# tud-amr/semantic_dsp_map

Hardware: AMD Instinct MI355X
Metric: Mvoxels updated/sec (256^3 grid, 2M particles, VKITTI2 camera; whole hot-path frame) (higher is better)
Workload: dtype f32

## Files before the change

### include/sdm.h

```cpp
#ifndef SDM_H_
#define SDM_H_

#include <stddef.h>
#include <stdint.h>

#ifdef __cplusplus
extern "C" {
#endif

typedef struct sdm_map sdm_map;

typedef enum {
  SDM_OK = 0,
  SDM_ERR_INVALID_ARGUMENT = 1,
  SDM_ERR_NO_DEVICE = 2,
  SDM_ERR_HIP = 3,
  SDM_ERR_CAPACITY = 4,
  SDM_ERR_NOT_CONVERGED = 5,
  SDM_ERR_COMM = 6
} sdm_status;

typedef struct {
  int32_t x_n, y_n, z_n;
  int32_t p_n;
// ... 305 lines not shown
  uint64_t cell_sum[3];
  float    box_min[3];
  float    box_max[3];
  float    centroid[3];
  uint32_t pad1;
} sdm_frontier_cluster;
sdm_status sdm_frontiers_update(sdm_map *m, uint32_t flags, int32_t min_cells, int64_t max_cells);
sdm_status sdm_get_frontier_clusters(sdm_map *m, sdm_frontier_cluster *out, int32_t cap, int32_t *n_out, float origin[3]);
sdm_status sdm_get_frontier_cells(sdm_map *m, uint32_t *cell, uint32_t *cluster, uint8_t *unknown_faces,
                                  int64_t cap, int64_t *n_out);

#define SDM_VIEW_MAX_RAYS 65536
typedef struct {
  float pos[3];
  float q[4];
  float range;
} sdm_view;
typedef struct {
  uint32_t n_unknown;
  uint32_t n_free;
  uint32_t n_occupied;
  uint32_t rays_hit;
  uint32_t rays_in_map;
  uint32_t pad;
  uint64_t ray_cells;
  uint64_t ray_unknown;
} sdm_view_gain;
sdm_status sdm_query_views(sdm_map *m, const sdm_view *views, int64_t n_views, const float *dirs, int32_t n_rays,
                           sdm_view_gain *out, sdm_segment_hit *rays_out, int32_t *ray_unknown_out, uint32_t flags);

#define SDM_REACH_FACE_CONNECTED  0x1u
#define SDM_REACH_THROUGH_UNKNOWN 0x2u
#define SDM_REACH_COST_PER_CELL   10
typedef struct {
  uint32_t n_starts_used;
  uint32_t n_traversable, n_reached, max_cost_reached;
  uint32_t rounds;
  uint32_t flags, min_d2, max_cost;
} sdm_reach_info;
typedef struct {
  uint32_t cost;
  float    metres;
  uint32_t cell;
  uint8_t  next;
  uint8_t  status;
  uint16_t pad;
} sdm_reach_result;
sdm_status sdm_reach_update(sdm_map *m, const float *start_xyz, const uint32_t *start_cells, int64_t n_starts,
                            uint32_t min_d2, uint32_t max_cost, uint32_t flags);
sdm_status sdm_get_reach(sdm_map *m, uint32_t *cost, sdm_reach_info *info, float origin[3]);
sdm_status sdm_query_reach(sdm_map *m, const float *xyz, const uint32_t *cells, int64_t n, sdm_reach_result *out, uint32_t flags);
sdm_status sdm_reach_paths(sdm_map *m, const float *xyz, const uint32_t *cells, int64_t n, int32_t max_len,
                           uint32_t *cells_out, int32_t *len_out, uint32_t flags);

sdm_status sdm_object_particle_count(sdm_map *m, int32_t track_id, int64_t *count);
sdm_status sdm_tracks_with_particles(sdm_map *m, int32_t *out, int32_t cap, int32_t *n_out);

sdm_status sdm_get_stats(sdm_map *m, sdm_stats *out, int32_t count_live);
sdm_status sdm_set_profiling(sdm_map *m, int32_t on);
sdm_status sdm_debug_force_generic_flood(sdm_map *m, int32_t on);
sdm_status sdm_get_ring_state(sdm_map *m, sdm_ring_state *out);
sdm_status sdm_set_ring_state(sdm_map *m, const sdm_ring_state *in);
sdm_status sdm_get_stamps(sdm_map *m, uint32_t *sx, uint32_t *sy, uint32_t *sz);
sdm_status sdm_set_stamps(sdm_map *m, const uint32_t *sx, const uint32_t *sy, const uint32_t *sz);
sdm_status sdm_dump_state(sdm_map *m, float *px, float *py, float *pz, float *w, uint16_t *ts,
                          uint16_t *track, uint8_t *label, uint8_t *status, uint8_t *forget,
                          uint16_t *owner);
sdm_status sdm_load_state(sdm_map *m, const float *px, const float *py, const float *pz,
                          const float *w, const uint16_t *ts, const uint16_t *track,
                          const uint8_t *label, const uint8_t *status, const uint8_t *forget,
                          const uint16_t *owner);
sdm_status sdm_get_ck_kappa(sdm_map *m, float *out);
sdm_status sdm_get_bin_counts(sdm_map *m, uint32_t *out);
sdm_status sdm_get_bins(sdm_map *m, uint32_t *out, int64_t cap, int64_t *n_out);
sdm_status sdm_get_extrinsic(sdm_map *m, float *out16);

sdm_status sdm_time_occupancy_sweep(sdm_map *m, int32_t iters, float *avg_ms);
sdm_status sdm_debug_fill_dense(sdm_map *m);
sdm_status sdm_debug_fill_dense_ex(sdm_map *m, int32_t mode);
sdm_status sdm_debug_hinted_groups(sdm_map *m, int64_t *n_out);
sdm_status sdm_debug_sweep_lists(sdm_map *m, int32_t mode);
sdm_status sdm_debug_sweep_mode(sdm_map *m, int32_t *mode_out);
sdm_status sdm_debug_alias_cap(sdm_map *m, int32_t cap);
sdm_status sdm_debug_reach_tiles(sdm_map *m, int64_t *tiles_out);
sdm_status sdm_debug_view_batch(sdm_map *m, int32_t max_views_in_flight);

sdm_status sdm_test_scan(const uint32_t *in, uint32_t *out, int64_t n);
sdm_status sdm_test_sort_pairs(const uint32_t *keys_in, const uint32_t *vals_in, uint32_t *keys_out,
                               uint32_t *vals_out, int64_t n, int32_t nbits);
#define SDM_TEST_IN_PLACE 1u
#define SDM_TEST_COUNT_ON_DEVICE 2u
#define SDM_TEST_GUARD_WORDS 64
sdm_status sdm_test_scratch_elems(int32_t sort, int64_t n, int64_t *elems);
sdm_status sdm_test_scan_seq(int32_t n_calls, const int64_t *capacity, const int64_t *count, uint32_t flags,
                             const uint32_t *in, uint32_t *out, int32_t *guard_ok, uint32_t *scratch_out);
sdm_status sdm_test_sort_pairs_seq(int32_t n_calls, const int64_t *capacity, const int64_t *count, const int32_t *nbits,
                                   uint32_t flags, const uint32_t *keys_in, const uint32_t *vals_in, uint32_t *keys_out,
                                   uint32_t *vals_out, int32_t *which, int32_t *guard_ok, uint32_t *scratch_out);

const char *sdm_last_error(void);
const char *sdm_version(void);

#ifdef __cplusplus
}
#endif
#endif
```

### semantic_dsp_map_amd/binding.py

```python
import ctypes as C
import os

import numpy as np

_HERE = os.path.dirname(os.path.abspath(__file__))
LIB_PATH = os.environ.get("SDM_LIB_PATH") or os.path.join(_HERE, "csrc", "libsdm_hip.so")

LABELED_POINT = np.dtype([("x", "<f4"), ("y", "<f4"), ("z", "<f4"), ("sigma", "<f4"),
                          ("track_id", "<u2"), ("label_id", "u1"), ("is_valid", "u1")])
OBJECT_MOVE = np.dtype([("track_id", "<i4"), ("T", "<f4", (16,))])
VOXEL_RESULT = np.dtype([("wsum", "<f4"), ("track", "<u2"), ("label", "u1"), ("occ", "i1")])
POINT = np.dtype([("x", "<f4"), ("y", "<f4"), ("z", "<f4"), ("track", "<u2"), ("label", "u1"), ("occ", "i1")])
POINT_XYZRGB = np.dtype([("x", "<f4"), ("y", "<f4"), ("z", "<f4"), ("one", "<f4"), ("b", "u1"), ("g", "u1"), ("r", "u1"), ("a", "u1"),
                         ("pad", "<u4", (3,))])
assert LABELED_POINT.itemsize == 20 and OBJECT_MOVE.itemsize == 68 and VOXEL_RESULT.itemsize == 8 and POINT.itemsize == 16
SEGMENT_HIT = np.dtype([("t", "<f4"), ("voxel", "<u4"), ("cells", "<i4"), ("track", "<u2"), ("label", "u1"), ("occ", "i1")])
BOX_RESULT = np.dtype([("n_occupied", "<i4"), ("n_free", "<i4"), ("n_unknown", "<i4"), ("first_occupied", "<u4"), ("clipped", "<i4")])
assert SEGMENT_HIT.itemsize == 16 and BOX_RESULT.itemsize == 20
QUERY_ON_DEVICE = 0x1
QUERY_UNKNOWN_BLOCKS = 0x2
DISTANCE_RESULT = np.dtype([("distance", "<f4"), ("gradient", "<f4", (3,)), ("nearest", "<f4", (3,)), ("d2", "<u4"), ("track", "<u2"),
                            ("label", "u1"), ("occ", "i1")])
assert DISTANCE_RESULT.itemsize == 36
ESDF_UNKNOWN_IS_OBSTACLE = 0x1
# ... 123 lines not shown
        "sdm_update": [vp, vp, vp, vp, vp, vp, i32, vp, i32, u32, i32],
        "sdm_update_raw": [vp, vp, vp, vp, vp, i32, vp, vp, vp, i32, vp, i32, u32, i32],
        "sdm_update_raw_ex": [vp, vp, vp, vp, vp, i32, vp, vp, vp, i32, vp, i32, u32, i32, vp],
        "sdm_get_labeled_cloud": [vp, vp],
        "sdm_host_alloc": [C.c_size_t, C.POINTER(vp)],
        "sdm_host_free": [vp],
        "sdm_update_begin": [vp, vp, vp, vp, vp, vp, i32, vp, i32, u32, i32, C.POINTER(vp)],
        "sdm_update_finish": [vp, vp, i32, u32, i32],
        "sdm_frame_start": [vp, vp, vp, vp, vp, vp, i32, vp, i32, u32, i32],
        "sdm_frame_moves": [vp],
        "sdm_frame_moves_pending": [vp, C.POINTER(C.c_int32)],
        "sdm_frame_predict": [vp, C.POINTER(vp)],
        "sdm_set_halo_buffers": [vp, vp, vp, vp, vp, i32],
        "sdm_comm_unique_id": [vp],
        "sdm_comm_init": [vp, vp, i32],
        "sdm_ipc_create": [vp, i32, vp],
        "sdm_ipc_connect": [vp, vp],
        "sdm_update_sharded": [vp, vp, vp, vp, vp, vp, i32, vp, i32, u32],
        "sdm_ck_chunk_elems": [vp, C.POINTER(i64)],
        "sdm_ck_reduce": [vp, vp, vp],
        "sdm_comm_timing": [vp, i32],
        "sdm_get_comm_times": [vp, vp],
        "sdm_device_alloc": [vp, C.c_size_t, C.POINTER(vp)],
        "sdm_device_free": [vp, vp],
        "sdm_device_upload": [vp, vp, vp, C.c_size_t],
        "sdm_device_download": [vp, vp, vp, C.c_size_t],
        "sdm_device_synchronize": [vp],
        "sdm_stream": [vp, C.POINTER(vp)],
        "sdm_set_stream": [vp, vp],
        "sdm_set_ck_buffer": [vp, vp],
        "sdm_synchronize": [vp],
        "sdm_get_voxels": [vp, vp],
        "sdm_get_occupied": [vp, vp, C.c_size_t, C.POINTER(C.c_size_t), i32],
        "sdm_get_occupied_rgb": [vp, vp, C.c_size_t, C.POINTER(C.c_size_t), i32],
        "sdm_get_freespace_rgb": [vp, vp, C.c_size_t, C.POINTER(C.c_size_t), i32],
        "sdm_set_colours": [vp, vp],
        "sdm_get_freespace": [vp, vp, C.c_size_t, C.POINTER(C.c_size_t), i32],
        "sdm_voxels_device_ptr": [vp, C.POINTER(vp)],
        "sdm_query_points": [vp, vp, i64, vp, vp, u32],
        "sdm_query_segments": [vp, vp, i64, vp, u32],
        "sdm_query_boxes": [vp, vp, i64, vp, u32],
        "sdm_esdf_update": [vp, u32],
        "sdm_get_esdf": [vp, vp, vp, vp],
        "sdm_query_distance": [vp, vp, i64, vp, u32],
        "sdm_instances_update": [vp, u32],
        "sdm_get_instances": [vp, vp, i32, C.POINTER(i32), vp],
        "sdm_get_label_cells": [vp, vp],
        "sdm_frontiers_update": [vp, u32, i32, i64],
        "sdm_get_frontier_clusters": [vp, vp, i32, C.POINTER(i32), vp],
        "sdm_get_frontier_cells": [vp, vp, vp, vp, i64, C.POINTER(i64)],
        "sdm_query_views": [vp, vp, i64, vp, i32, vp, vp, vp, u32],
        "sdm_debug_view_batch": [vp, i32],
        "sdm_reach_update": [vp, vp, vp, i64, u32, u32, u32],
        "sdm_get_reach": [vp, vp, vp, vp],
        "sdm_query_reach": [vp, vp, vp, i64, vp, u32],
        "sdm_reach_paths": [vp, vp, vp, i64, i32, vp, vp, u32],
        "sdm_debug_reach_tiles": [vp, C.POINTER(i64)],
        "sdm_object_particle_count": [vp, i32, C.POINTER(i64)],
        "sdm_tracks_with_particles": [vp, vp, i32, C.POINTER(i32)],
        "sdm_comm_set_options": [vp, i32, i32],
        "sdm_get_stats": [vp, C.POINTER(Stats), i32],
        "sdm_set_profiling": [vp, i32],
        "sdm_debug_force_generic_flood": [vp, i32],
        "sdm_get_ring_state": [vp, C.POINTER(RingState)],
        "sdm_set_ring_state": [vp, C.POINTER(RingState)],
        "sdm_get_stamps": [vp, vp, vp, vp],
        "sdm_set_stamps": [vp, vp, vp, vp],
        "sdm_dump_state": [vp] + [vp] * 10,
        "sdm_load_state": [vp] + [vp] * 10,
        "sdm_get_ck_kappa": [vp, vp],
        "sdm_get_bin_counts": [vp, vp],
        "sdm_get_bins": [vp, vp, i64, C.POINTER(i64)],
        "sdm_get_extrinsic": [vp, vp],
        "sdm_time_occupancy_sweep": [vp, i32, C.POINTER(C.c_float)],
        "sdm_set_issue_mode": [vp, i32],
        "sdm_bind_host_thread": [i32],
        "sdm_host_numa_node_early": [i32],
        "sdm_debug_fill_dense": [vp],
        "sdm_debug_fill_dense_ex": [vp, i32],
        "sdm_debug_hinted_groups": [vp, C.POINTER(C.c_int64)],
        "sdm_debug_sweep_lists": [vp, i32],
        "sdm_debug_sweep_mode": [vp, C.POINTER(i32)],
        "sdm_debug_alias_cap": [vp, i32],
        "sdm_test_scan": [vp, vp, i64],
        "sdm_test_sort_pairs": [vp, vp, vp, vp, i64, i32],
        "sdm_test_scratch_elems": [i32, i64, C.POINTER(i64)],
        "sdm_test_scan_seq": [i32, vp, vp, u32, vp, vp, C.POINTER(i32), vp],
        "sdm_test_sort_pairs_seq": [i32, vp, vp, vp, u32, vp, vp, vp, vp, vp, C.POINTER(i32), vp],
    }
    for name, argtypes in sig.items():
        fn = getattr(L, name)
        fn.argtypes = argtypes
        fn.restype = C.c_int
    L.sdm_last_error.restype = C.c_char_p
    L.sdm_version.restype = C.c_char_p
    global HOST_NUMA_NODE
    HOST_NUMA_NODE = L.sdm_bind_host_thread(int(os.environ.get("LOCAL_RANK", "0")))
    _lib = L
    return L


def _ptr(a):
    if a is None:
        return None
    if isinstance(a, int):
        return C.c_void_p(a)
    return a.ctypes.data_as(C.c_void_p)


def _check(L, rc, what):
    if rc != 0:
        raise SdmError("%s failed: %s (%s)" % (what, STATUS_NAMES.get(rc, rc), L.sdm_last_error().decode()))


class SdmMap:

    def __init__(self, cfg, params=None, noise_table=None, device=0, shard_rank=0, shard_count=1, max_visible=0):
        self.L = load_library()
        c = Config()
        for k, _ in Config._fields_:
            if k in cfg:
                setattr(c, k, cfg[k])
        c.device, c.shard_rank, c.shard_count, c.max_visible = device, shard_rank, shard_count, max_visible
        self.cfg = c
        h = C.c_void_p()
        _check(self.L, self.L.sdm_create(C.byref(c), C.byref(h)), "sdm_create")
        self.h = h
        self.V = 1 << (c.x_n + c.y_n + c.z_n)
        self.S = 1 << c.p_n
        self.v_count = self.V // shard_count
        self.W, self.H = c.width, c.height
        if params is not None:
            self.set_params(params)
        if noise_table is not None:
            self.upload_noise_table(noise_table)

    def close(self):
        if getattr(self, "h", None):
            self.L.sdm_destroy(self.h)
            self.h = None

    def __del__(self):
        try:
            self.close()
        except Exception:
            pass

    def clear(self):
        _check(self.L, self.L.sdm_clear(self.h), "sdm_clear")

    def set_params(self, params):
        p = Params()
        for k, _ in Params._fields_:
            setattr(p, k, params[k])
        _check(self.L, self.L.sdm_set_params(self.h, C.byref(p)), "sdm_set_params")

    def generate_noise_table(self, seed=20250217, n=1000000, stddev=0.05):
        _check(self.L, self.L.sdm_generate_noise_table(self.h, seed, n, stddev), "sdm_generate_noise_table")

    def upload_noise_table(self, table):
        t = np.ascontiguousarray(table, dtype=np.float32)
        _check(self.L, self.L.sdm_upload_noise_table(self.h, _ptr(t), t.size), "sdm_upload_noise_table")

    def download_noise_table(self, n=1000000):
        t = np.empty(n, np.float32)
        _check(self.L, self.L.sdm_download_noise_table(self.h, _ptr(t), n), "sdm_download_noise_table")
# ... 398 lines not shown

    def ring_state(self):
        r = RingState()
        _check(self.L, self.L.sdm_get_ring_state(self.h, C.byref(r)), "sdm_get_ring_state")
        return {"global_time_stamp": r.global_time_stamp, "moved_steps": list(r.moved_steps),
                "eq_steps": list(r.eq_steps), "map_center": list(r.map_center), "last_pos": list(r.last_pos),
                "birth_cursor": r.birth_cursor, "move_cursor": r.move_cursor}

    def set_ring_state(self, d):
        r = RingState()
        r.global_time_stamp = d["global_time_stamp"]
        for i in range(3):
            r.moved_steps[i] = d["moved_steps"][i]
            r.eq_steps[i] = d["eq_steps"][i]
            r.map_center[i] = d["map_center"][i]
            r.last_pos[i] = d["last_pos"][i]
        r.birth_cursor = d["birth_cursor"]
        r.move_cursor = d["move_cursor"]
        _check(self.L, self.L.sdm_set_ring_state(self.h, C.byref(r)), "sdm_set_ring_state")

    def stamps(self):
        c = self.cfg
        sx = np.empty(1 << c.x_n, np.uint32)
        sy = np.empty(1 << c.y_n, np.uint32)
        sz = np.empty(1 << c.z_n, np.uint32)
        _check(self.L, self.L.sdm_get_stamps(self.h, _ptr(sx), _ptr(sy), _ptr(sz)), "sdm_get_stamps")
        return sx, sy, sz

    def set_stamps(self, sx, sy, sz):
        sx, sy, sz = (np.ascontiguousarray(a, dtype=np.uint32) for a in (sx, sy, sz))
        _check(self.L, self.L.sdm_set_stamps(self.h, _ptr(sx), _ptr(sy), _ptr(sz)), "sdm_set_stamps")

    def dump_state(self):
        n = self.v_count * self.S
        st = {k: np.empty(n, dt) for k, dt in STATE_FIELDS}
        _check(self.L, self.L.sdm_dump_state(self.h, *[_ptr(st[k]) for k, _ in STATE_FIELDS]), "sdm_dump_state")
        return st

    def load_state(self, st):
        arrs = [np.ascontiguousarray(st[k], dtype=dt) for k, dt in STATE_FIELDS]
        _check(self.L, self.L.sdm_load_state(self.h, *[_ptr(a) for a in arrs]), "sdm_load_state")

    def ck_kappa(self):
        out = np.empty(self.W * self.H, np.float32)
        _check(self.L, self.L.sdm_get_ck_kappa(self.h, _ptr(out)), "sdm_get_ck_kappa")
        return out.reshape(self.H, self.W)

    def bin_counts(self):
        out = np.empty(self.W * self.H, np.uint32)
        _check(self.L, self.L.sdm_get_bin_counts(self.h, _ptr(out)), "sdm_get_bin_counts")
        return out.reshape(self.H, self.W)

    def bins(self):
        n = C.c_int64()
        _check(self.L, self.L.sdm_get_bins(self.h, None, 0, C.byref(n)), "sdm_get_bins")
        out = np.empty(max(n.value, 1), np.uint32)
        _check(self.L, self.L.sdm_get_bins(self.h, _ptr(out), n.value, C.byref(n)), "sdm_get_bins")
        return out[:n.value]

    def extrinsic(self):
        out = np.empty(16, np.float32)
        _check(self.L, self.L.sdm_get_extrinsic(self.h, _ptr(out)), "sdm_get_extrinsic")
        return out.reshape(4, 4)

    def fill_dense_ex(self, mode):
        _check(self.L, self.L.sdm_debug_fill_dense_ex(self.h, mode), "sdm_debug_fill_dense_ex")

    def hinted_groups(self):
        n = C.c_int64()
        _check(self.L, self.L.sdm_debug_hinted_groups(self.h, C.byref(n)), "sdm_debug_hinted_groups")
        return n.value

    def force_sweep_lists(self, mode):
        _check(self.L, self.L.sdm_debug_sweep_lists(self.h, int(mode)), "sdm_debug_sweep_lists")

    def sweep_mode(self):
        v = C.c_int32(0)
        _check(self.L, self.L.sdm_debug_sweep_mode(self.h, C.byref(v)), "sdm_debug_sweep_mode")
        return v.value

    def set_alias_cap(self, cap):
        _check(self.L, self.L.sdm_debug_alias_cap(self.h, int(cap)), "sdm_debug_alias_cap")

    def fill_dense(self):
        _check(self.L, self.L.sdm_debug_fill_dense(self.h), "sdm_debug_fill_dense")

    def time_occupancy_sweep(self, iters=20):
        ms = C.c_float()
        _check(self.L, self.L.sdm_time_occupancy_sweep(self.h, iters, C.byref(ms)), "sdm_time_occupancy_sweep")
        return ms.value


def pinhole_rays(cfg, stride=1):
    get = (lambda k: cfg[k]) if isinstance(cfg, dict) else (lambda k: getattr(cfg, k))
    u = np.arange(0, int(get("width")), int(stride), dtype=np.float32)
    v = np.arange(0, int(get("height")), int(stride), dtype=np.float32)
    x = (u - np.float32(get("cx"))) / np.float32(get("fx"))
    y = (v - np.float32(get("cy"))) / np.float32(get("fy"))
    out = np.empty((len(v), len(u), 3), np.float32)
    out[..., 0], out[..., 1], out[..., 2] = x[None, :], y[:, None], 1.0
    return out


def comm_unique_id():
    L = load_library()
    buf = np.zeros(128, np.uint8)
    _check(L, L.sdm_comm_unique_id(_ptr(buf)), "sdm_comm_unique_id")
    return buf.tobytes()


def test_scan(a):
    L = load_library()
    a = np.ascontiguousarray(a, dtype=np.uint32)
    out = np.empty_like(a)
    _check(L, L.sdm_test_scan(_ptr(a), _ptr(out), a.size), "sdm_test_scan")
    return out


def test_sort_pairs(keys, vals, nbits):
    L = load_library()
    keys = np.ascontiguousarray(keys, dtype=np.uint32)
    vals = np.ascontiguousarray(vals, dtype=np.uint32)
    ko, vo = np.empty_like(keys), np.empty_like(vals)
    _check(L, L.sdm_test_sort_pairs(_ptr(keys), _ptr(vals), _ptr(ko), _ptr(vo), keys.size, nbits), "sdm_test_sort_pairs")
    return ko, vo


TEST_IN_PLACE, TEST_COUNT_ON_DEVICE, TEST_GUARD_WORDS = 1, 2, 64


def test_scratch_elems(sort, n):
    L = load_library()
    v = C.c_int64(0)
    _check(L, L.sdm_test_scratch_elems(int(bool(sort)), int(n), C.byref(v)), "sdm_test_scratch_elems")
    return v.value


def _seq_args(capacity, count, arrays):
    capacity = np.ascontiguousarray(capacity, dtype=np.int64)
    count = capacity.copy() if count is None else np.ascontiguousarray(count, dtype=np.int64)
    if capacity.ndim != 1 or capacity.size == 0 or count.shape != capacity.shape:
        raise ValueError("one capacity and one count per call")
    arrays = [np.ascontiguousarray(a, dtype=np.uint32) for a in arrays]
    if any(a.shape != (int(capacity.sum()),) for a in arrays):
        raise ValueError("the arrays hold one slice of `capacity` words per call")
    return capacity, count, arrays


def test_scan_seq(capacity, a, out, count=None, in_place=False, count_on_device=False, want_scratch=False):
    L = load_library()
    capacity, count, (a, out) = _seq_args(capacity, count, [a, out])
    out = out.copy()
    flags = (TEST_IN_PLACE if in_place else 0) | (TEST_COUNT_ON_DEVICE if count_on_device else 0)
    scratch = np.empty(test_scratch_elems(False, capacity.max()), np.uint32) if want_scratch else None
    ok = C.c_int32(0)
    _check(L, L.sdm_test_scan_seq(capacity.size, _ptr(capacity), _ptr(count), flags, _ptr(a), _ptr(out), C.byref(ok), _ptr(scratch)),
           "sdm_test_scan_seq")
    return out, bool(ok.value), scratch


def test_sort_pairs_seq(capacity, nbits, keys, vals, keys_out, vals_out, count=None, count_on_device=False, want_scratch=False):
    L = load_library()
    capacity, count, (keys, vals, keys_out, vals_out) = _seq_args(capacity, count, [keys, vals, keys_out, vals_out])
    nbits = np.ascontiguousarray(np.broadcast_to(np.asarray(nbits, np.int32), capacity.shape))
    keys_out, vals_out = keys_out.copy(), vals_out.copy()
    which = np.zeros(capacity.size, np.int32)
# ... 7 lines not shown
```

### semantic_dsp_map_amd/csrc/frame.hip

```cpp
#include <chrono>

#include "sdm_map.h"

#pragma clang fp contract(off)

void sdm::drop_graphs(sdm_map *m) {
  if (m->graph_exec) (void)hipGraphExecDestroy(m->graph_exec);
  if (m->graph) (void)hipGraphDestroy(m->graph);
  m->graph_exec = nullptr;
  m->graph = nullptr;
  m->graph_set_node = nullptr;
  for (hipGraphExec_t &g : m->piece) {
    if (g) (void)hipGraphExecDestroy(g);
    g = nullptr;
  }
}

namespace {

inline void stage_mark(sdm_map *m, int stage) {
  if (m->profiling && !m->capturing) {
    (void)hipEventRecord(m->ev[stage], m->stream);
    m->stage_ran[stage] = true;
  }
}

sdm_status frame_host_prepare(sdm_map *m, const float cam_pos[3], const float cam_q[4], const sdm_object_move *moves, int32_t n_moves,
                              const int32_t *remove_tracks, int32_t n_remove, uint32_t flags, int32_t stop_after) {
  if ((n_moves > MAX_MOVE_OBJECTS || n_remove > MAX_REMOVE_TRACKS) && m->capturing) {
    set_error("sdm_update", __FILE__, __LINE__, "object lists beyond one frame block inside a graph capture");
    return SDM_ERR_INVALID_ARGUMENT;
  }
  m->moves_all.clear();
  m->removes_all.clear();
  m->mv_batch_next = n_moves > MAX_MOVE_OBJECTS ? (size_t)MAX_MOVE_OBJECTS : 0;
  m->mv_batch_ready = false;
  if (n_moves > MAX_MOVE_OBJECTS) m->moves_all.assign(moves, moves + n_moves);
  if (n_remove > MAX_REMOVE_TRACKS) m->removes_all.assign(remove_tracks, remove_tracks + n_remove);
  m->stop_after = stop_after;
  m->frame_flags = flags;
  for (int i = 0; i < 9; ++i) m->stage_ran[i] = false;
  m->global_time_stamp += 1;
  FrameArgs &fa = m->fa;
  fa.su.n = 0;
  fa.su.value = m->global_time_stamp;
  m->restamped[0] = m->restamped[1] = m->restamped[2] = 0;
  update_ego_center(m, cam_pos);
  sync_frame_scalars(m);
  if (m->stamps_dirty) {
    m->sweep_all = true;
    fa.su.n = 0;
  }
  refresh_filter(m);
  m->forgetting_initialized = true;
  compute_extrinsic(m, cam_pos, cam_q);
  compute_frustum_box(m);
  fa.f = m->f;
  memset(&fa.ms, 0, sizeof(fa.ms));
  const int n_first = n_moves < MAX_MOVE_OBJECTS ? n_moves : MAX_MOVE_OBJECTS;
  fa.ms.n = n_first;
  for (int k = 0; k < n_first; ++k) {
    fa.ms.track[k] = (uint16_t)moves[k].track_id;
    memcpy(fa.ms.T[k], moves[k].T, 12 * sizeof(float));
  }
  fa.n_obj = n_first;
  fa.mv_batch = 0;
  if (n_moves > 0 && !stage_done(stop_after, 1)) m->mv_seq++;
  fa.mv_seq = m->mv_seq;
  fa.n_remove = n_remove < MAX_REMOVE_TRACKS ? n_remove : MAX_REMOVE_TRACKS;
  for (int k = 0; k < fa.n_remove; ++k) fa.remove[k] = (uint16_t)remove_tracks[k];
  fa.force_generic = m->force_generic_flood;
  m->n_moves = n_moves;
  m->n_remove = n_remove;
  return SDM_OK;
}

sdm_status frame_enqueue_start(sdm_map *m) {
  hipStream_t s = m->stream;
  const Dims &d = m->d;
  const int32_t stop_after = m->stop_after;
  const bool whole = d.v_count == d.V;
  stage_mark(m, 0);
  if (m->stamps_dirty) SDM_TRY(upload_stamps(m));
  m->cur_depth = m->fa.depth;
  m->cur_cloud = m->fa.cloud;
  if (m->capturing) {
    m->fb.set(d, m->st, m->sc, m->fa, true, whole);
    launch_frame_begin(m->fb, s);
    HIP_TRY(hipEventRecord(m->cap_begin, s));
    HIP_TRY(hipStreamWaitEvent(m->s_frustum, m->cap_begin, 0));
    HIP_TRY(hipStreamWaitEvent(m->s_birth, m->cap_begin, 0));
  } else {
    const bool side_chain_now = m->n_moves > 0 && (!whole || ((m->comm || m->ipc) && m->sharded_frame));
    if (!m->state_event_valid && (!m->vis_event_valid || side_chain_now)) {
      HIP_TRY(hipEventRecord(m->ev_state, s));
      m->state_event_valid = true;
    }
    HIP_TRY(hipStreamWaitEvent(m->s_frustum, m->vis_event_valid ? m->ev_vis : m->ev_state, 0));
    launch_set_frame(m->d_fa[1], m->fa, m->s_frustum);
    HIP_TRY(hipEventRecord(m->ev_fa, m->s_frustum));
    if (whole && m->mv_pending) HIP_TRY(hipMemsetAsync(m->sc.mv_tot, 0, move_total_elems() * sizeof(uint32_t), s));
    m->fb.set(d, m->st, m->sc, m->fa, false, whole);
    launch_frame_begin(m->fb, s, !stage_done(stop_after, 5) ? m->ev_begin : nullptr);
    if (whole && m->n_moves > 0) m->mv_pending = true;
  }
  stage_mark(m, 1);
  if (stage_done(stop_after, 1)) return SDM_OK;

  const bool side_chain = !m->capturing && m->n_moves > 0 && (!whole || ((m->comm || m->ipc) && m->sharded_frame));
  if (m->capturing) {
    if (!whole) launch_moves_count(d, m->st, m->sc, m->d_counts_local, s);
  } else if (side_chain) {
    HIP_TRY(lazy_stream(m->device, &m->s_moves));
    HIP_TRY(hipStreamWaitEvent(m->s_moves, m->ev_state, 0));
    if (!whole) {
      if (m->mv_pending) HIP_TRY(hipMemsetAsync(m->sc.mv_tot, 0, move_total_elems() * sizeof(uint32_t), m->s_moves));
      launch_moves_count(d, m->st, m->sc, m->counts_local_user ? m->counts_local_user : m->d_counts_local, m->s_moves, &m->fa);
      m->mv_pending = true;
    }
    if ((m->comm || m->ipc) && m->sharded_frame) {
      if (m->comm_timing) HIP_TRY(hipEventRecord(m->ev_comm[0], m->s_moves));
      SDM_TRY(exchange_counts(m, m->s_moves));
      if (m->comm_timing) {
        HIP_TRY(hipEventRecord(m->ev_comm[1], m->s_moves));
        m->comm_timed[0] = true;
      }
    }
    HIP_TRY(hipEventRecord(m->ev_counts, m->s_moves));
  }
  if (!stage_done(stop_after, 3)) {
    launch_frustum(d, m->sc, m->s_frustum);
    HIP_TRY(hipGetLastError());
    HIP_TRY(hipEventRecord(m->capturing ? m->cap_frustum : m->ev_frustum, m->s_frustum));
  } else if (!m->capturing) {
    HIP_TRY(hipStreamWaitEvent(s, m->ev_fa, 0));
  }
  if (!stage_done(stop_after, 5)) {
    if (!m->capturing) HIP_TRY(hipStreamWaitEvent(m->s_birth, m->ev_begin, 0));
    m->birth_which = launch_birth_prepare(d, m->flt, m->bo, m->st, m->sc, m->s_birth);
    HIP_TRY(hipEventRecord(m->capturing ? m->cap_birth : m->ev_birth, m->s_birth));
  }
  if (side_chain) HIP_TRY(hipStreamWaitEvent(s, m->ev_counts, 0));
  m->state_event_valid = false;
  m->vis_event_valid = false;
  return SDM_OK;
}

sdm_status check_frame_args(sdm_map *m, const float *depth, const sdm_labeled_point *cloud, const float cam_pos[3], const float cam_q[4],
                            const sdm_object_move *moves, int32_t n_moves, const int32_t *remove_tracks, int32_t n_remove) {
  if (!m || !depth || !cloud || !cam_pos || !cam_q || n_moves < 0 || n_remove < 0 || (n_moves && !moves) || (n_remove && !remove_tracks)) {
    set_error("sdm_update", __FILE__, __LINE__, "null pointer or negative count");
    return SDM_ERR_INVALID_ARGUMENT;
  }
  return SDM_OK;
}

sdm_status stage_inputs(sdm_map *m, const float *depth, const sdm_labeled_point *cloud, uint32_t flags) {
  const size_t hw = (size_t)m->d.W * m->d.H;
  if (flags & SDM_INPUT_ON_DEVICE) {
    m->fa.depth = depth;
    m->fa.cloud = cloud;
  } else {
    HIP_TRY(hipMemcpyAsync(m->d_depth, depth, hw * sizeof(float), hipMemcpyHostToDevice, m->stream));
    HIP_TRY(hipMemcpyAsync(m->d_cloud, cloud, hw * sizeof(sdm_labeled_point), hipMemcpyHostToDevice, m->stream));
    m->fa.depth = m->d_depth;
    m->fa.cloud = m->d_cloud;
  }
  return SDM_OK;
}

}

extern "C" {

sdm_status sdm_frame_start(sdm_map *m, const float *depth, const sdm_labeled_point *cloud, const float cam_pos[3],
                           const float cam_q[4], const sdm_object_move *moves, int32_t n_moves,
                           const int32_t *remove_tracks, int32_t n_remove, uint32_t flags, int32_t stop_after) {
  sdm_status rc = check_frame_args(m, depth, cloud, cam_pos, cam_q, moves, n_moves, remove_tracks, n_remove);
  if (rc != SDM_OK) return rc;
  HIP_TRY(hipSetDevice(m->device));
  if ((rc = frame_host_prepare(m, cam_pos, cam_q, moves, n_moves, remove_tracks, n_remove, flags, stop_after)) != SDM_OK) return rc;
  if ((rc = stage_inputs(m, depth, cloud, flags)) != SDM_OK) return rc;
  m->n_direct_frames++;
  return frame_enqueue_start(m);
}

sdm_status sdm_frame_moves(sdm_map *m) {
  if (!m) return SDM_ERR_INVALID_ARGUMENT;
  if (stage_done(m->stop_after, SDM_STAGE_EGO)) return SDM_OK;
  if (!m->capturing) HIP_TRY(hipSetDevice(m->device));
  const int world = m->cfg.shard_count, rank = m->cfg.shard_rank;
  const int32_t *counts_all = m->counts_all_user;
  int w = world, r = rank;
  if (!counts_all) {
    counts_all = m->counts_local_user ? m->counts_local_user : m->d_counts_local;
    w = 1;
    r = 0;
  }
  if (m->capturing || m->n_moves > 0) {
    launch_moves_transform(m->d, m->flt, m->st, m->sc, counts_all, w, r, m->stream);
    m->mv_pending = false;
    m->mv_batch_ready = false;
    const bool shard = m->d.v_count != m->d.V;
    while (m->mv_batch_next && m->mv_batch_next < m->moves_all.size()) {
      const size_t k0 = m->mv_batch_next;
      const int nb = (int)std::min<size_t>(MAX_MOVE_OBJECTS, m->moves_all.size() - k0);
      FrameArgs &fa = m->fa;
      memset(&fa.ms, 0, sizeof(fa.ms));
      fa.ms.n = nb;
      for (int k = 0; k < nb; ++k) {
        fa.ms.track[k] = (uint16_t)m->moves_all[k0 + k].track_id;
        memcpy(fa.ms.T[k], m->moves_all[k0 + k].T, 12 * sizeof(float));
      }
      fa.n_obj = nb;
      fa.mv_seq = ++m->mv_seq;
      fa.mv_batch += 1;
      m->mv_batch_next = k0 + MAX_MOVE_OBJECTS;
      launch_moves_batch(m->d, m->st, m->sc, fa, m->counts_local_user ? m->counts_local_user : m->d_counts_local, m->stream);
      if (shard) {
        m->mv_batch_ready = true;
        return SDM_OK;
      }
      launch_moves_transform(m->d, m->flt, m->st, m->sc, counts_all, w, r, m->stream);
    }
    m->mv_batch_next = 0;
  }
  return SDM_OK;
}

sdm_status sdm_frame_moves_pending(sdm_map *m, int32_t *pending) {
  if (!m || !pending) return SDM_ERR_INVALID_ARGUMENT;
  *pending = m->mv_batch_ready ? 1 : 0;
  return SDM_OK;
}

sdm_status sdm_frame_predict(sdm_map *m, const float **ck_part_dev) {
  if (!m) return SDM_ERR_INVALID_ARGUMENT;
  if (m->mv_batch_ready) {
    set_error("sdm_frame_predict", __FILE__, __LINE__, "a batch of the frame's object list is still waiting for its counts: sdm_frame_moves_pending");
    return SDM_ERR_INVALID_ARGUMENT;
  }
  const int stop_after = m->stop_after;
  if (stage_done(stop_after, SDM_STAGE_EGO)) return SDM_OK;
  if (!m->capturing) HIP_TRY(hipSetDevice(m->device));
  hipStream_t s = m->stream;
  const Dims &d = m->d;
  if (m->capturing || m->n_moves > 0)
    launch_moves_finish(d, m->flt, m->st, m->sc, m->counts_all_user ? m->cfg.shard_count : 1, m->cfg.shard_rank, s);
  stage_mark(m, 2);
  if (stage_done(stop_after, 2)) return SDM_OK;

  if (m->capturing || m->n_remove > 0) launch_remove(d, m->st, m->sc, s);
  for (size_t k0 = MAX_REMOVE_TRACKS; k0 < m->removes_all.size(); k0 += MAX_REMOVE_TRACKS) {
    FrameArgs &fa = m->fa;
    fa.n_remove = (int)std::min<size_t>(MAX_REMOVE_TRACKS, m->removes_all.size() - k0);
    for (int k = 0; k < fa.n_remove; ++k) fa.remove[k] = (uint16_t)m->removes_all[k0 + k];
    launch_set_frame(m->d_fa[0], fa, s);
    launch_remove(d, m->st, m->sc, s);
  }
  stage_mark(m, 3);
  if (stage_done(stop_after, 3)) return SDM_OK;

  HIP_TRY(hipStreamWaitEvent(s, m->capturing ? m->cap_frustum : m->ev_frustum, 0));
  float *ck_dst = m->ck_user ? m->ck_user : m->d_ck_part;
  launch_visibility(d, m->flt, m->st, m->sc, ck_dst, m->fused_ck ? 1 : 0, s, m->capturing ? nullptr : m->ev_vis);
  if (!m->capturing) m->vis_event_valid = true;
  stage_mark(m, 4);
  if (stage_done(stop_after, 4)) return SDM_OK;

  launch_ck(d, m->flt, m->st, m->sc, ck_dst, m->fused_ck ? 1 : 0, s);
  if (ck_part_dev) *ck_part_dev = ck_dst;
  return SDM_OK;
}

sdm_status sdm_update_begin(sdm_map *m, const float *depth, const sdm_labeled_point *cloud, const float cam_pos[3],
                            const float cam_q[4], const sdm_object_move *moves, int32_t n_moves,
                            const int32_t *remove_tracks, int32_t n_remove, uint32_t flags, int32_t stop_after,
                            const float **ck_part_dev) {
  sdm_status rc = sdm_frame_start(m, depth, cloud, cam_pos, cam_q, moves, n_moves, remove_tracks, n_remove, flags, stop_after);
  if (rc != SDM_OK) return rc;
  const int32_t *keep_all = m->counts_all_user;
  m->counts_all_user = nullptr;
  rc = sdm_frame_moves(m);
  while (rc == SDM_OK && m->mv_batch_ready) rc = sdm_frame_moves(m);
  if (rc == SDM_OK) rc = sdm_frame_predict(m, ck_part_dev);
  m->counts_all_user = keep_all;
  return rc;
}

sdm_status sdm_set_halo_buffers(sdm_map *m, int32_t *counts_local, const int32_t *counts_all, void *send, const void *recv_all,
                                int32_t cap_records) {
  if (!m || cap_records < 0) return SDM_ERR_INVALID_ARGUMENT;
  m->counts_local_user = counts_local;
  m->counts_all_user = counts_all;
  m->sc.halo_send = (unsigned char *)send;
  m->sc.halo_recv = (const unsigned char *)recv_all;
  m->sc.halo_cap = (uint32_t)cap_records;
  m->sc.halo_world = (uint32_t)m->cfg.shard_count;
  return SDM_OK;
}

sdm_status sdm_update_finish(sdm_map *m, const float *ck_parts_dev, int32_t n_parts, uint32_t flags, int32_t stop_after) {
  if (!m || n_parts < 1) return SDM_ERR_INVALID_ARGUMENT;
  if (stage_done(stop_after, SDM_STAGE_VISIBILITY)) return SDM_OK;
  if (!m->capturing) HIP_TRY(hipSetDevice(m->device));
  hipStream_t s = m->stream;
  const Dims &d = m->d;
  const float *own = m->ck_user ? m->ck_user : m->d_ck_part;
  const float *ck_raw = nullptr;
  if (!m->fused_ck) {
    if (!ck_parts_dev || n_parts == 1) ck_raw = ck_parts_dev ? ck_parts_dev : own;
    else launch_ck_finish(d, m->flt, m->sc, ck_parts_dev, n_parts, m->ck_part_stride, s);
  }
  m->ck_raw_last = ck_raw;
  m->ck_part_stride = 0;
  launch_weight(d, m->flt, m->st, m->sc, s, ck_raw);
  stage_mark(m, 5);
  if (stage_done(stop_after, 5)) return SDM_OK;
  HIP_TRY(hipStreamWaitEvent(s, m->capturing ? m->cap_birth : m->ev_birth, 0));
  launch_birth_replay(d, m->flt, m->st, m->sc, m->birth_which, m->global_time_stamp > 65535u, s);
  if (!m->capturing) {
    if (d.v_count != d.V || m->comm || m->ipc) {
      HIP_TRY(hipEventRecord(m->ev_state, s));
      m->state_event_valid = true;
    } else {
      m->state_event_valid = false;
    }
  }
  stage_mark(m, 6);
  if (stage_done(stop_after, 6)) return SDM_OK;
  if (!(flags & SDM_SKIP_OCCUPANCY)) {
    launch_occupancy(d, m->flt, m->st, m->sc.cnt, m->sweep_all ? 1 : 0, m->sc.fa, next_epoch(m->f.epoch), s, sweep_mode(m));
    if (m->sweep_all) m->sweep_rec_pending = true;
    m->sweep_all = false;
    if (!m->capturing) m->sweep_epoch = next_epoch(m->f.epoch);
  }
  stage_mark(m, 7);
  return SDM_OK;
}

namespace {

sdm_status issue_frame(sdm_map *m, uint32_t flags, int32_t stop_after) {
  sdm_status rc = frame_enqueue_start(m);
  if (rc == SDM_OK) rc = sdm_frame_moves(m);
  if (rc == SDM_OK) rc = sdm_frame_predict(m, nullptr);
  if (rc == SDM_OK) rc = sdm_update_finish(m, nullptr, 1, flags, stop_after);
  return rc;
// ... 18 lines not shown
  sdm_status rc = SDM_OK;
  if (e == hipSuccess) {
    rc = issue_frame(m, m->frame_flags, 0);
    hipGraph_t g = nullptr;
    e = hipStreamEndCapture(m->stream, &g);
    m->graph = g;
  }
  m->s_frustum = side[0];
  m->s_birth = side[1];
  m->s_moves = side[2];
  m->capturing = false;
  if (e != hipSuccess || rc != SDM_OK || !m->graph) {
    set_error("hipStreamCapture", __FILE__, __LINE__, e != hipSuccess ? hipGetErrorString(e) : "frame enqueue failed under capture");
    (void)hipGetLastError();
    return rc != SDM_OK ? rc : SDM_ERR_HIP;
  }
  size_t n_nodes = 0;
  HIP_TRY(hipGraphGetNodes(m->graph, nullptr, &n_nodes));
  std::vector<hipGraphNode_t> nodes(n_nodes);
  HIP_TRY(hipGraphGetNodes(m->graph, nodes.data(), &n_nodes));
  for (hipGraphNode_t nd : nodes) {
    hipGraphNodeType t;
    if (hipGraphNodeGetType(nd, &t) != hipSuccess || t != hipGraphNodeTypeKernel) continue;
    hipKernelNodeParams kp;
    if (hipGraphKernelNodeGetParams(nd, &kp) == hipSuccess && kp.func == FrameBeginLaunch::kernel()) m->graph_set_node = nd;
  }
  if (!m->graph_set_node) {
    set_error("graph_capture", __FILE__, __LINE__, "frame-block node not found in the captured graph");
    return SDM_ERR_HIP;
  }
  HIP_TRY(hipGraphInstantiate(&m->graph_exec, m->graph, nullptr, nullptr, 0));
  m->graph_flt = m->flt;
  return SDM_OK;
}

sdm_status graph_launch(sdm_map *m) {
  m->fb.set(m->d, m->st, m->sc, m->fa, true, m->d.v_count == m->d.V);
  hipKernelNodeParams kp;
  memset(&kp, 0, sizeof(kp));
  kp.func = const_cast<void *>(FrameBeginLaunch::kernel());
  kp.gridDim = dim3(FrameBeginLaunch::GRID);
  kp.blockDim = dim3(FrameBeginLaunch::BLOCK);
  kp.sharedMemBytes = 0;
  kp.kernelParams = m->fb.argv;
  kp.extra = nullptr;
  const auto t0 = std::chrono::steady_clock::now();
  HIP_TRY(hipGraphExecKernelNodeSetParams(m->graph_exec, m->graph_set_node, &kp));
  const auto t1 = std::chrono::steady_clock::now();
  HIP_TRY(hipGraphLaunch(m->graph_exec, m->stream));
  if (m->host_timing) {
    m->t_setparams_us += std::chrono::duration<double, std::micro>(t1 - t0).count();
    m->t_launch_us += std::chrono::duration<double, std::micro>(std::chrono::steady_clock::now() - t1).count();
  }
  return SDM_OK;
}

sdm_status pieces_capture(sdm_map *m) {
  SDM_TRY(capture_prepare(m));
  const Dims &d = m->d;
  auto capture = [&](hipStream_t st, int which, auto &&body) -> sdm_status {
    HIP_TRY(hipStreamBeginCapture(st, hipStreamCaptureModeThreadLocal));
    body(st);
    hipGraph_t g = nullptr;
    hipError_t e = hipStreamEndCapture(st, &g);
    if (e != hipSuccess || !g) {
      set_error("hipStreamEndCapture", __FILE__, __LINE__, e != hipSuccess ? hipGetErrorString(e) : "no graph");
      (void)hipGetLastError();
      return SDM_ERR_HIP;
    }
    e = hipGraphInstantiate(&m->piece[which], g, nullptr, nullptr, 0);
    (void)hipGraphDestroy(g);
    if (e != hipSuccess) {
      set_error("hipGraphInstantiate", __FILE__, __LINE__, hipGetErrorString(e));
      return SDM_ERR_HIP;
    }
    return SDM_OK;
  };
  sdm_status rc = capture(m->s_frustum, 0, [&](hipStream_t st) { launch_frustum(d, m->sc, st); });
  if (rc == SDM_OK)
    rc = capture(m->s_birth, 1, [&](hipStream_t st) { m->birth_which = launch_birth_prepare(d, m->flt, m->bo, m->st, m->sc, st); });
  if (rc == SDM_OK)
    rc = capture(m->stream, 2, [&](hipStream_t st) {
      if (d.v_count != d.V) launch_moves_count(d, m->st, m->sc, m->d_counts_local, st);
      launch_moves_transform(d, m->flt, m->st, m->sc, m->d_counts_local, 1, 0, st);
      launch_moves_finish(d, m->flt, m->st, m->sc, 1, m->cfg.shard_rank, st);
      launch_remove(d, m->st, m->sc, st);
    });
  if (rc == SDM_OK)
    rc = capture(m->stream, 3, [&](hipStream_t st) {
      launch_visibility(d, m->flt, m->st, m->sc, m->d_ck_part, 1, st);
      launch_ck(d, m->flt, m->st, m->sc, m->d_ck_part, 1, st);
      launch_weight(d, m->flt, m->st, m->sc, st);
    });
  if (rc == SDM_OK)
    rc = capture(m->stream, 4, [&](hipStream_t st) {
      launch_birth_replay(d, m->flt, m->st, m->sc, m->birth_which, false, st);
      launch_occupancy(d, m->flt, m->st, m->sc.cnt, 0, m->sc.fa, 0, st);
    });
  m->graph_flt = m->flt;
  return rc;
}

sdm_status pieces_launch(sdm_map *m) {
  hipStream_t s = m->stream;
  const auto t0 = std::chrono::steady_clock::now();
  m->fb.set(m->d, m->st, m->sc, m->fa, true, m->d.v_count == m->d.V);
  launch_frame_begin(m->fb, s);
  HIP_TRY(hipEventRecord(m->ev_begin, s));
  HIP_TRY(hipStreamWaitEvent(m->s_frustum, m->ev_begin, 0));
  HIP_TRY(hipGraphLaunch(m->piece[0], m->s_frustum));
  HIP_TRY(hipEventRecord(m->ev_frustum, m->s_frustum));
  HIP_TRY(hipStreamWaitEvent(m->s_birth, m->ev_begin, 0));
  HIP_TRY(hipGraphLaunch(m->piece[1], m->s_birth));
  HIP_TRY(hipEventRecord(m->ev_birth, m->s_birth));
  HIP_TRY(hipGraphLaunch(m->piece[2], s));
  HIP_TRY(hipStreamWaitEvent(s, m->ev_frustum, 0));
  HIP_TRY(hipGraphLaunch(m->piece[3], s));
  HIP_TRY(hipStreamWaitEvent(s, m->ev_birth, 0));
  HIP_TRY(hipGraphLaunch(m->piece[4], s));
  if (m->host_timing) m->t_launch_us += std::chrono::duration<double, std::micro>(std::chrono::steady_clock::now() - t0).count();
  return SDM_OK;
}

}

sdm_status sdm_set_issue_mode(sdm_map *m, int32_t mode) {
  if (!m || mode < 0 || mode > 4) return SDM_ERR_INVALID_ARGUMENT;
  HIP_TRY(hipSetDevice(m->device));
  bool use;
  int shape;
  issue_mode_for(m, mode, &use, &shape);
  if (shape != m->graph_shape) {
    HIP_TRY(hipStreamSynchronize(m->stream));
    drop_graphs(m);
  }
  m->graph_mode = mode;
  m->use_graph = use;
  m->graph_shape = shape;
  return SDM_OK;
}

sdm_status sdm_update(sdm_map *m, const float *depth, const sdm_labeled_point *cloud, const float cam_pos[3],
                      const float cam_q[4], const sdm_object_move *moves, int32_t n_moves, const int32_t *remove_tracks,
                      int32_t n_remove, uint32_t flags, int32_t stop_after) {
  sdm_status rc = check_frame_args(m, depth, cloud, cam_pos, cam_q, moves, n_moves, remove_tracks, n_remove);
  if (rc != SDM_OK) return rc;
  HIP_TRY(hipSetDevice(m->device));
  m->fused_ck = true;
  const auto tp0 = std::chrono::steady_clock::now();
  rc = frame_host_prepare(m, cam_pos, cam_q, moves, n_moves, remove_tracks, n_remove, flags, stop_after);
  if (rc == SDM_OK) rc = stage_inputs(m, depth, cloud, flags);
  if (m->host_timing) m->t_prepare_us += std::chrono::duration<double, std::micro>(std::chrono::steady_clock::now() - tp0).count();
  if (rc != SDM_OK) {
    m->fused_ck = false;
    return rc;
  }
  const bool would_be_plain = stop_after == 0 && (flags & ~(uint32_t)SDM_INPUT_ON_DEVICE) == 0 && !m->profiling &&
                              m->cfg.shard_count == 1 && !m->comm && !m->ck_user && !m->counts_local_user &&
                              m->stream == m->own_stream && !m->sweep_all && !m->stamps_dirty &&
                              n_moves <= MAX_MOVE_OBJECTS && n_remove <= MAX_REMOVE_TRACKS &&
                              m->global_time_stamp <= 65535u;
  const bool plain = m->use_graph && would_be_plain;
  if (plain) {
    const bool pieces = m->graph_shape == GRAPH_PIECES;
    bool have = pieces ? m->piece[4] != nullptr : m->graph_exec != nullptr;
    if (have && memcmp(&m->graph_flt, &m->flt, sizeof(Filter)) != 0) have = false;
    if (!have) {
      const auto tc = std::chrono::steady_clock::now();
      rc = pieces ? pieces_capture(m) : graph_capture(m);
      if (m->host_timing)
        fprintf(stderr, "sdm host timing: graph capture + instantiate %.0f us (%s)\n",
                std::chrono::duration<double, std::micro>(std::chrono::steady_clock::now() - tc).count(),
                pieces ? "pieces" : (m->graph_shape == GRAPH_CHAIN ? "chain" : "branched"));
    }
    bool direct = false;
    if (rc != SDM_OK) {
      m->use_graph = false;
      direct = true;
      rc = SDM_OK;
    } else {
      rc = pieces ? pieces_launch(m) : graph_launch(m);
      if (rc != SDM_OK) {
        m->use_graph = false;
        m->stamps_dirty = true;
        m->sweep_all = true;
      } else {
        m->cur_depth = m->fa.depth;
        m->cur_cloud = m->fa.cloud;
        m->state_event_valid = false;
        m->vis_event_valid = false;
// ... 191 lines not shown
```

### semantic_dsp_map_amd/csrc/kernels.hip

```cpp
#include <algorithm>

#include <type_traits>

#include <hip/hip_ext.h>
#include "sdm_internal.h"
#include "sdm_scratch.h"

#pragma clang fp contract(off)

namespace sdm {

namespace {

constexpr int TPB = 256;

#ifdef SDM_AB_TIMERS
}
__device__ unsigned long long g_dbg[6][8192 * 4];
namespace {
#define DBG_T() wall_clock64()
#define DBG_PUTK(k, i, v) do { if (blockIdx.x < 8192) g_dbg[k][blockIdx.x * 4 + (i)] = (unsigned long long)(v); } while (0)
#define DBG_PUT(i, v) DBG_PUTK(0, i, v)
#define DBG_LANE0(k, i) do { if (threadIdx.x == 0 && threadIdx.y == 0) DBG_PUTK(k, i, DBG_T()); } while (0)
#else
#define DBG_T() 0ull
#define DBG_PUT(i, v)
#define DBG_LANE0(k, i)
#endif

typedef uint32_t v4u __attribute__((ext_vector_type(4)));
typedef uint32_t v2u __attribute__((ext_vector_type(2)));
template <typename T>
using gptr = const __attribute__((address_space(1))) T *;
template <typename T>
__device__ __forceinline__ gptr<T> as_global(const T *p) {
  return (gptr<T>)p;
}
__device__ __forceinline__ sdm_labeled_point load_point(const sdm_labeled_point *cloud, size_t i) {
  static_assert(sizeof(sdm_labeled_point) == 20, "five words");
  gptr<uint32_t> w = (gptr<uint32_t>)(cloud + i);
  uint32_t t[5];
#pragma unroll
  for (int k = 0; k < 5; ++k) t[k] = w[k];
  sdm_labeled_point o;
  __builtin_memcpy(&o, t, sizeof(o));
  return o;
}
template <int A = 16, typename T, int N>
__device__ __forceinline__ void load_vec(T (&dst)[N], const T *src) {
  constexpr int B = (int)sizeof(T) * N;
  if constexpr (A < (B > 16 ? 16 : B)) {
    __builtin_memcpy(dst, __builtin_assume_aligned(src, A), B);
  } else if constexpr (B >= 16) {
    const v4u *p = reinterpret_cast<const v4u *>(src);
    v4u tmp[B / 16];
#pragma unroll
    for (int i = 0; i < B / 16; ++i) tmp[i] = __builtin_nontemporal_load(p + i);
    __builtin_memcpy(dst, tmp, B);
  } else if constexpr (B == 8) {
    v2u tmp = __builtin_nontemporal_load(reinterpret_cast<const v2u *>(src));
    __builtin_memcpy(dst, &tmp, 8);
  } else if constexpr (B == 4) {
    uint32_t tmp = __builtin_nontemporal_load(reinterpret_cast<const uint32_t *>(src));
    __builtin_memcpy(dst, &tmp, 4);
  } else {
    uint16_t tmp = __builtin_nontemporal_load(reinterpret_cast<const uint16_t *>(src));
    __builtin_memcpy(dst, &tmp, 2);
  }
}
template <int A = 16, typename T, int N>
__device__ __forceinline__ void store_vec(T *dst, const T (&src)[N]) {
  constexpr int B = (int)sizeof(T) * N;
  constexpr int AL = A < (B > 16 ? 16 : B) ? A : (B > 16 ? 16 : B);
  __builtin_memcpy(__builtin_assume_aligned(dst, AL), src, B);
}

template <int S>
struct RecRaw {
  static constexpr int L = S - 1, BYTES = 10 * L, N8 = (BYTES + 7) / 8;
  uint32_t d[2 * N8];
};
template <int S, bool NT = true>
__device__ __forceinline__ void rec_fetch(RecRaw<S> &raw, const unsigned char *r) {
  constexpr int N8 = RecRaw<S>::N8;
#pragma unroll
  for (int j = 0; j < N8 / 2; ++j) {
    const rec_v4u *q = reinterpret_cast<const rec_v4u *>(r + 16 * j);
    const rec_v4u t = NT ? __builtin_nontemporal_load(q) : *q;
    raw.d[4 * j + 0] = t.x;
    raw.d[4 * j + 1] = t.y;
    raw.d[4 * j + 2] = t.z;
    raw.d[4 * j + 3] = t.w;
  }
  if constexpr (N8 & 1) {
    const rec_v2u *q = reinterpret_cast<const rec_v2u *>(r + 16 * (N8 / 2));
    const rec_v2u t = NT ? __builtin_nontemporal_load(q) : *q;
    raw.d[2 * N8 - 2] = t.x;
    raw.d[2 * N8 - 1] = t.y;
  }
}
__device__ __forceinline__ uint32_t raw_u16(const uint32_t *d, int off) { return (d[off >> 2] >> ((off & 3) * 8)) & 0xffffu; }
__device__ __forceinline__ uint32_t raw_u8(const uint32_t *d, int off) { return (d[off >> 2] >> ((off & 3) * 8)) & 0xffu; }
template <int S>
__device__ __forceinline__ void rec_unpack(const RecRaw<S> &raw, float (&wv)[S], uint16_t (&ts)[S], uint16_t (&trk)[S], uint8_t (&lab)[S],
                                           uint8_t (&stv)[S]) {
  constexpr int L = S - 1;
  wv[0] = 0.f;
  ts[0] = 0;
  trk[0] = 0;
  lab[0] = 0;
// ... 1375 lines not shown
  for (int i = 1; i < S; ++i) {
    live[i] = false;
    if (stv[i] == ST_INVALID) continue;
    if ((uint32_t)tsv[i] < smax) {
      stv[i] = ST_INVALID;
      dirty = true;
      continue;
    }
    valid_n++;
    live[i] = true;
  }
  int pixv[S], rowv[S];
  float camz[S], dptv[S];
#pragma unroll
  for (int i = 1; i < S; ++i) {
    pixv[i] = -1;
    rowv[i] = 0;
    if (!live[i]) continue;
    int row, col;
    if (project_to_image(d, f, pos[i].x, pos[i].y, pos[i].z, row, col, camz[i])) {
      pixv[i] = row * d.W + col;
      rowv[i] = row;
      dptv[i] = depth_img[pixv[i]];
    }
  }
  bool vis[S];
  uint32_t pib[S];
#pragma unroll
  for (int i = 1; i < S; ++i) {
    vis[i] = false;
    if (!live[i] || pixv[i] < 0) continue;
    const float dpt = dptv[i];
    if (dpt > d.dmax) {
      SlotRef{rec, S - 1, (uint32_t)i - 1u}.set_w(SDM_OCC_INIT_WEIGHT);
      wrote_free = true;
      observed = true;
      continue;
    }
    if (camz[i] > dpt * d.occl_coeff) continue;
    observed = true;
    vis[i] = true;
  }
  const uint32_t sub = (shard + (threadIdx.x & 63u)) & (ROW_SUBS - 1);
  uint32_t rq[S];
#pragma unroll
  for (int i = 1; i < S; ++i)
    if (vis[i]) {
      pib[i] = atomicAdd(&sc.bin_count[pixv[i]], 1u);
      rq[i] = atomicAdd(&sc.row_cnt[(size_t)(rowv[i] * ROW_SUBS + sub) * ROW_CNT_STRIDE], 1u);
    }
#pragma unroll
  for (int i = 1; i < S; ++i)
    if (vis[i]) {
      if (rq[i] < sc.row_cap && pib[i] < (1u << ROW_PIB_BITS)) {
        const uint32_t col = (uint32_t)(pixv[i] - rowv[i] * d.W);
        sc.row_list[(size_t)(rowv[i] * ROW_SUBS + sub) * sc.row_cap + rq[i]] =
            make_uint2((uint32_t)(((size_t)v << d.p_n) + i), col | pib[i] << ROW_COL_BITS);
      } else {
        sc.cnt->overflow = 1;
      }
    }
  if (dirty) rec_store_status<S>(rec, stv);
  if (dirty || wrote_free) st.vflag[lv] = VF_DIRTY;
  bool stamped = observed;
  if (!observed && valid_n == 0) stamped = im_ok && im_z <= im_depth;
  if (stamped) st.vts[lv] = (uint16_t)f.gts;
  if (dirty || wrote_free || stamped) mark_tile(st, lv, f.epoch);
}

constexpr int VIS_WORDS = 32;
constexpr int VIS_J = VIS_WORDS * 64 / TPB;

template <int S>
__global__ __launch_bounds__(TPB) void k_visibility(Dims d, State st, Scratch sc) {
  __shared__ unsigned long long wmask[VIS_WORDS];
  __shared__ uint32_t woff[VIS_WORDS + 1];
  __shared__ uint16_t full_list[VIS_WORDS * 64];
  __shared__ uint32_t n_full;
  DBG_LANE0(1, 0);
  const Frame f = sc.fa->f;
  const gptr<float> depth_img = as_global(sc.fa->depth);
  const uint32_t fgen = (uint32_t)sc.fa->force_generic, fcx = (uint32_t)sc.cnt->flood_complex;
  const bool generic = (fgen | fcx) != 0;
  if (blockIdx.x == 0 && threadIdx.x == 0) {
    sc.cnt->vis_flood_complex = fcx;
    sc.cnt->vis_flood_rounds = sc.cnt->flood_rounds;
    sc.cnt->vis_start_in_frustum = sc.cnt->start_in_frustum;
  }
  const int bx = f.bb1[0] - f.bb0[0], by = f.bb1[1] - f.bb0[1], bz = f.bb1[2] - f.bb0[2];
  if (bx <= 0 || by <= 0 || bz <= 0) return;
  const int wlo = f.bb0[0] >> 6, nwx = ((f.bb1[0] - 1) >> 6) - wlo + 1;
  const uint32_t n_words = (uint32_t)nwx * by * bz;
  for (uint32_t g0 = blockIdx.x * VIS_WORDS; g0 < n_words; g0 += gridDim.x * VIS_WORDS) {
  __syncthreads();
  if (threadIdx.x == 0) n_full = 0;
  if (threadIdx.x < VIS_WORDS) {
    const uint32_t g = g0 + threadIdx.x;
    unsigned long long m = 0;
    if (g < n_words) {
      const int wi = wlo + (int)(g % nwx);
      const int ay = f.bb0[1] + (int)((g / nwx) % by);
      const int az = f.bb0[2] + (int)(g / ((uint32_t)nwx * by));
      const uint32_t rz = axis_correct(az + f.eq[2], d.NZ);
      if (rz >= d.rz_begin && rz < d.rz_begin + d.rz_count) {
        const uint64_t *__restrict__ bits = generic ? sc.reach : sc.vmask;
        const int VY = d.NY + 1;
        unsigned long long w0[4], w1[4], lr[4];
        const int wi1 = wi + 1 < (int)sc.wpl ? wi + 1 : wi;
#pragma unroll
        for (int c = 0; c < 4; ++c) {
          const int y = ay + (c & 1), z = az + (c >> 1);
          const size_t lb = ((size_t)z * VY + y) * sc.wpl;
          lr[c] = sc.line_reach[(size_t)z * sc.wy + (y >> 6)];
          w0[c] = bits[lb + wi];
          w1[c] = bits[lb + wi1];
        }
        __builtin_amdgcn_sched_barrier(0);
#pragma unroll
        for (int c = 0; c < 4; ++c) {
          const int y = ay + (c & 1);
          const bool line_ok = generic || ((lr[c] >> (y & 63)) & 1ull);
          const unsigned long long w1m = wi + 1 < (int)sc.wpl ? w1[c] : 0ull;
          if (line_ok) m |= w0[c] | (w0[c] >> 1) | (w1m << 63);
        }
        const int x0 = wi << 6;
        const int lo = f.bb0[0] > x0 ? f.bb0[0] - x0 : 0;
        const int hi = f.bb1[0] - x0 < 64 ? f.bb1[0] - x0 : 64;
        unsigned long long keep = hi >= 64 ? ~0ull : ((1ull << hi) - 1ull);
        keep &= ~((1ull << lo) - 1ull);
        m &= keep;
      }
    }
    wmask[threadIdx.x] = m;
    const uint32_t c = (uint32_t)__popcll(m);
    uint32_t inc = c;
#pragma unroll
    for (int off = 1; off < VIS_WORDS; off <<= 1) {
      const uint32_t t = __shfl_up(inc, off, 64);
      if ((int)threadIdx.x >= off) inc += t;
    }
    woff[threadIdx.x] = inc - c;
    if (threadIdx.x == VIS_WORDS - 1) woff[VIS_WORDS] = inc;
  }
  __syncthreads();
  const uint32_t nl = woff[VIS_WORDS];
  DBG_LANE0(1, 1);
  if (threadIdx.x == 0 && nl) atomicAdd(&sc.cnt->shard[blockIdx.x & (VIS_SHARDS - 1)].fv, nl);
  if (nl == 0) continue;
  uint32_t code[VIS_J], lvv[VIS_J], flg[VIS_J];
#pragma unroll
  for (int j = 0; j < VIS_J; ++j) {
    const uint32_t li = threadIdx.x + (uint32_t)j * TPB;
    code[j] = 0xffffffffu;
    lvv[j] = 0;
    flg[j] = 0;
    if ((uint32_t)j * TPB >= nl) continue;
    const bool have = li < nl;
    int w = 0;
#pragma unroll
    for (int k = 1; k < VIS_WORDS; ++k) w += woff[k] <= li ? 1 : 0;
    const int bit = nth_set_bit(wmask[w], li - woff[w]) & 63;
    const uint32_t g = g0 + (uint32_t)w;
    const int ax = ((wlo + (int)(g % nwx)) << 6) + bit;
    const int ay = f.bb0[1] + (int)((g / nwx) % by);
    const int az = f.bb0[2] + (int)(g / ((uint32_t)nwx * by));
    const uint32_t rx = axis_correct(ax + f.eq[0], d.NX), ry = axis_correct(ay + f.eq[1], d.NY), rz = axis_correct(az + f.eq[2], d.NZ);
    code[j] = have ? (uint32_t)(w << 6 | bit) : 0xffffffffu;
    lvv[j] = have ? ring_to_voxel(d, rx, ry, rz) - d.v_begin : 0u;
    flg[j] = st.vflag[lvv[j]];
  }
  __builtin_amdgcn_sched_barrier(0);
#pragma unroll
  for (int j = 0; j < VIS_J; ++j) flg[j] = code[j] != 0xffffffffu ? flg[j] & VF_STATE : 0u;
  float imz[VIS_J], imd[VIS_J];
#pragma unroll
  for (int j = 0; j < VIS_J; ++j) {
    imz[j] = 1.f;
    imd[j] = 0.f;
    if (code[j] == 0xffffffffu) continue;
    if (flg[j]) {
      full_list[atomicAdd(&n_full, 1u)] = (uint16_t)code[j];
      continue;
    }
    const uint32_t g = g0 + (code[j] >> 6);
    const int ax = ((wlo + (int)(g % nwx)) << 6) + (int)(code[j] & 63u);
    const int ay = f.bb0[1] + (int)((g / nwx) % by);
    const int az = f.bb0[2] + (int)(g / ((uint32_t)nwx * by));
    const float ix = (float)(uint32_t)ax * d.voxel_size + d.pmin[0] + f.center[0];
    const float iy = (float)(uint32_t)ay * d.voxel_size + d.pmin[1] + f.center[1];
    const float iz = (float)(uint32_t)az * d.voxel_size + d.pmin[2] + f.center[2];
    int row, col;
    float z;
    if (project_to_image(d, f, ix, iy, iz, row, col, z)) {
      imz[j] = z;
      imd[j] = depth_img[(size_t)row * d.W + col];
    }
  }
#pragma unroll
  for (int j = 0; j < VIS_J; ++j) {
    if (code[j] == 0xffffffffu || flg[j]) continue;
    if (imz[j] <= imd[j]) {
      st.vts[lvv[j]] = (uint16_t)f.gts;
      mark_tile(st, lvv[j], f.epoch);
    }
  }
  __syncthreads();
  DBG_LANE0(1, 2);
  const uint32_t nf = n_full;
  for (uint32_t k = threadIdx.x; k < nf; k += TPB) {
    const uint32_t c = full_list[k];
    const uint32_t g = g0 + (c >> 6);
    const int ax = ((wlo + (int)(g % nwx)) << 6) + (int)(c & 63u);
    const int ay = f.bb0[1] + (int)((g / nwx) % by);
    const int az = f.bb0[2] + (int)(g / ((uint32_t)nwx * by));
    visibility_voxel<S>(d, f, st, sc, depth_img, ax, ay, az);
  }
  DBG_LANE0(1, 3);
  }
}

__device__ __forceinline__ void sift_down(uint32_t *a, uint32_t start, uint32_t end) {
  uint32_t root = start;
  while (2 * root + 1 <= end) {
    uint32_t child = 2 * root + 1, sw = root;
    if (a[sw] < a[child]) sw = child;
    if (child + 1 <= end && a[sw] < a[child + 1]) sw = child + 1;
    if (sw == root) return;
    uint32_t t = a[root];
    a[root] = a[sw];
    a[sw] = t;
    root = sw;
  }
}

constexpr int A7_ROWS = 16;
constexpr int A7_ITEMS = 16;
constexpr uint32_t CK_LIGHT_MAX = 4;
enum : uint8_t { CK_DONE = 0, CK_LIGHT = 1, CK_HEAVY = 2 };

__device__ __forceinline__ void ck_store(const Filter &flt, const Scratch &sc, float *__restrict__ ck_out, int finish, int p,
                                         const sdm_labeled_point &o, float ck) {
  if (finish) {
    const float ckk = ck * flt.p_detect + flt.noise_number;
    sc.ck_kappa[p] = ckk;
    sc.pix4[p] = make_float4(o.x, o.y, o.z, ckk);
    sc.pixt[p] = (uint32_t)o.track_id | (1u << 16);
  } else {
    ck_out[p] = ck;
  }
}

constexpr int BR_TPB = 640;
constexpr int BR_WAVES = BR_TPB / 64;
constexpr int BR_MAXW = 1 << ROW_COL_BITS;
template <int PPT>
__global__ __launch_bounds__(BR_TPB) __attribute__((amdgpu_waves_per_eu(PPT <= 4 ? 5 : 4, PPT <= 4 ? 5 : 4))) void k_bin_rows(Dims d, State st, Scratch sc) {
  static_assert(PPT == 2 || PPT == 4 || PPT * BR_TPB >= BR_MAXW, "eight pixels per thread cover the widest image");
  __shared__ uint32_t pre[BR_MAXW + 1];
  __shared__ uint32_t wave_tot[BR_WAVES];
  __shared__ uint32_t s_base;
  const int r = blockIdx.x;
  DBG_LANE0(2, 0);
  if (r == (int)gridDim.x - 1 && threadIdx.x < 64) alias_compact_wave(st);
  const bool overflow = sc.cnt->overflow != 0;
  const int lane = threadIdx.x & 63, wid = threadIdx.x >> 6;
  const int W = d.W;
  uint32_t c[PPT];
  const int j0 = PPT * (int)threadIdx.x;
#pragma unroll
  for (int u = 0; u < PPT; ++u) c[u] = (!overflow && j0 + u < W) ? sc.bin_count[r * W + j0 + u] : 0u;
  uint32_t sub_n = 0;
  if (threadIdx.x < ROW_SUBS && !overflow) {
    sub_n = sc.row_cnt[(size_t)(r * ROW_SUBS + threadIdx.x) * ROW_CNT_STRIDE];
    if (sub_n > sc.row_cap) sub_n = sc.row_cap;
  }
  uint32_t inc = 0;
#pragma unroll
  for (int u = 0; u < PPT; ++u) inc += c[u];
  const uint32_t mine = inc;
#pragma unroll
  for (int off = 1; off < 64; off <<= 1) {
    const uint32_t t = __shfl_up(inc, off, 64);
    if (lane >= off) inc += t;
  }
  if (lane == 63) wave_tot[wid] = inc;
  __syncthreads();
  uint32_t before = 0, total = 0;
#pragma unroll
  for (int w = 0; w < BR_WAVES; ++w) {
    if (w < wid) before += wave_tot[w];
    total += wave_tot[w];
  }
  {
    uint32_t run = before + inc - mine;
#pragma unroll
    for (int u = 0; u < PPT; ++u) {
      if (j0 + u < W) pre[j0 + u] = run;
      run += c[u];
    }
  }
  if (threadIdx.x == 0) {
// ... 1422 lines not shown
}

void launch_clear(const Dims &d, const State &st, hipStream_t s, bool fresh) {
  size_t n = (size_t)d.v_count * d.S;
  if (fresh) {
    hipMemsetAsync(st.pos4, 0, n * sizeof(float4), s);
    hipMemsetAsync(st.forget, 0, n, s);
    hipMemsetAsync(st.rec, 0, (size_t)d.v_count * rec_bytes(d.S), s);
    hipMemsetAsync(st.vts, 0, (size_t)d.v_count * sizeof(uint16_t), s);
    hipMemsetAsync(st.vflag, 0, (size_t)d.v_count, s);
    hipMemsetAsync(st.owner, 0xFF, n * sizeof(uint16_t), s);
    hipMemsetAsync(st.res, 0, (size_t)d.v_count * sizeof(sdm_voxel_result), s);
  } else {
    if (d.S == 8) hipLaunchKernelGGL(k_clear_map<8>, dim3(blocks_for(d.v_count, CLR_VOX)), dim3(TPB), 0, s, d, st);
    else if (d.S == 16) hipLaunchKernelGGL(k_clear_map<16>, dim3(blocks_for(d.v_count, CLR_VOX)), dim3(TPB), 0, s, d, st);
    else
      hipLaunchKernelGGL(k_clear_slots, dim3(blocks_for(n)), dim3(TPB), 0, s, d, st, n);
  }
  hipMemsetAsync(st.grp_hint, 0, grp_hint_bytes(d.v_count), s);
  hipMemsetAsync(st.alias, 0, 8, s);
  hipMemsetAsync(st.alias_filter, 0, ALIAS_FILTER_WORDS * 4, s);
  hipMemsetAsync(st.owner_flag, 0, owner_flag_bytes(n), s);
  hipMemsetAsync(st.owner_flag2, 0, owner_flag2_bytes(n), s);
}

#define SDM_DISPATCH_S(kernel, grid, s, ...)                                                      \
  switch (d.p_n) {                                                                                 \
    case 1: hipLaunchKernelGGL(kernel<2>, grid, dim3(TPB), 0, s, __VA_ARGS__); break;              \
    case 2: hipLaunchKernelGGL(kernel<4>, grid, dim3(TPB), 0, s, __VA_ARGS__); break;              \
    case 3: hipLaunchKernelGGL(kernel<8>, grid, dim3(TPB), 0, s, __VA_ARGS__); break;              \
    default: hipLaunchKernelGGL(kernel<16>, grid, dim3(TPB), 0, s, __VA_ARGS__); break;            \
  }

size_t tile_mark_bytes(const Dims &d) {
  const size_t n_tiles = blocks_for(d.v_count, OCC_TILE);
  return (std::max<size_t>(n_tiles, (size_t)TPB * OCC_SEG_MAX) + 16 + 15) / 16 * 16;
}
void launch_occupancy(const Dims &d, const Filter &flt, const State &st, Counters *cnt, int all_dirty, const FrameArgs *fa, uint32_t remark,
                      hipStream_t s, int mode) {
  dim3 grid(blocks_for(d.v_count, OCC_TILE));
  const int lists = mode & OCC_LISTS;
  if (all_dirty && (mode & OCC_SKIP_SCAN)) {
    SDM_DISPATCH_S(k_occupancy_dense, grid, s, d, flt.occ_threshold, st, cnt, st.occ_need, remark, grid.x | 0x80000000u);
  } else if (all_dirty) {
    const dim3 sgrid = grid;
    if (lists) {
      SDM_DISPATCH_S(k_occupancy_scan_lists, sgrid, s, d, flt.occ_threshold, st, cnt, st.occ_need, grid.x, remark);
      SDM_DISPATCH_S(k_occupancy_listed, dim3(OCC_LISTED_GRID), s, d, flt.occ_threshold, st, remark);
    } else {
      SDM_DISPATCH_S(k_occupancy_scan, sgrid, s, d, flt.occ_threshold, st, cnt, st.occ_need, grid.x, remark);
    }
    SDM_DISPATCH_S(k_occupancy_dense, grid, s, d, flt.occ_threshold, st, cnt, st.occ_need, remark, grid.x);
  } else {
    const uint32_t n_tiles = grid.x;
    const uint32_t seg = n_tiles <= TPB * OCC_SEG_MAX ? ((n_tiles + TPB - 1) / TPB + 15u) / 16u * 16u : 0u;
    if (seg) grid = dim3(std::min<uint32_t>(OCC_GRID, n_tiles));
    SDM_DISPATCH_S(k_occupancy, grid, s, d, flt.occ_threshold, st, cnt, fa, n_tiles, seg);
  }
}


void launch_set_frame(FrameArgs *fa_dev, const FrameArgs &fa, hipStream_t s) {
  hipLaunchKernelGGL(k_set_frame, dim3(1), dim3(TPB), 0, s, fa_dev, fa);
}
const void *set_frame_kernel() { return reinterpret_cast<const void *>(k_set_frame); }

void launch_frustum(const Dims &d, const Scratch &sc, hipStream_t s) {
  static bool lds_attr_set = false;
  if (!lds_attr_set) {
    (void)hipFuncSetAttribute(reinterpret_cast<const void *>(k_flood2d), hipFuncAttributeMaxDynamicSharedMemorySize, 152 * 1024);
    lds_attr_set = true;
  }
  const size_t max_words = (size_t)(d.NY + 1) * (d.NZ + 1) * sc.wpl;
  const unsigned g_mask = (unsigned)std::min<size_t>(blocks_for(max_words * 64), 4096);
  const unsigned g_line = (unsigned)std::min<size_t>(blocks_for((size_t)sc.wy * (d.NZ + 1) * 64), 256);
  hipLaunchKernelGGL(k_vertex_mask, dim3(g_mask), dim3(TPB), 0, s, d, sc.fa_side, sc.vmask, sc.wpl, sc.cnt);
  hipLaunchKernelGGL(k_line_info, dim3(g_line), dim3(TPB), 0, s, d, sc.fa_side, sc.vmask, sc.wpl, sc.wy, sc.line_ne, sc.line_ey, sc.line_ez,
                     sc.cnt);
  hipLaunchKernelGGL(k_flood2d, dim3(1), dim3(TPB), (size_t)(d.NZ + 1) * sc.wy * 8 * 4, s, d, sc.fa_side, sc.vmask, sc.wpl, sc.wy, sc.line_ey,
                     sc.line_ez, sc.line_reach, sc.cnt);
  hipLaunchKernelGGL(k_flood_generic, dim3(1), dim3(1024), 0, s, d, sc.fa_side, sc.vmask, sc.reach, sc.wpl, sc.cnt);
}

void launch_visibility(const Dims &d, const Filter &flt, const State &st, const Scratch &sc, float *ck_out, int finish, hipStream_t s,
                       hipEvent_t vis_done) {
  {
    const size_t max_words = (size_t)((d.NX + 63) / 64 + 1) * d.NY * d.NZ;
    dim3 grid((unsigned)std::min<size_t>(blocks_for(max_words, VIS_WORDS), 2048));
    if (vis_done) {
      switch (d.p_n) {
        case 1: hipExtLaunchKernelGGL(k_visibility<2>, grid, dim3(TPB), 0, s, nullptr, vis_done, 0, d, st, sc); break;
        case 2: hipExtLaunchKernelGGL(k_visibility<4>, grid, dim3(TPB), 0, s, nullptr, vis_done, 0, d, st, sc); break;
        case 3: hipExtLaunchKernelGGL(k_visibility<8>, grid, dim3(TPB), 0, s, nullptr, vis_done, 0, d, st, sc); break;
        default: hipExtLaunchKernelGGL(k_visibility<16>, grid, dim3(TPB), 0, s, nullptr, vis_done, 0, d, st, sc); break;
      }
    } else {
      SDM_DISPATCH_S(k_visibility, grid, s, d, st, sc);
    }
  }
  if (d.W <= 2 * BR_TPB) hipLaunchKernelGGL(k_bin_rows<2>, dim3((unsigned)d.H), dim3(BR_TPB), 0, s, d, st, sc);
  else if (d.W <= 4 * BR_TPB) hipLaunchKernelGGL(k_bin_rows<4>, dim3((unsigned)d.H), dim3(BR_TPB), 0, s, d, st, sc);
  else hipLaunchKernelGGL(k_bin_rows<8>, dim3((unsigned)d.H), dim3(BR_TPB), 0, s, d, st, sc);
  hipLaunchKernelGGL(k_ck_classify, dim3(blocks_for((size_t)d.W * d.H)), dim3(TPB), 0, s, d, flt, sc, ck_out, finish);
}

void launch_ck(const Dims &d, const Filter &flt, const State &st, const Scratch &sc, float *ck_out, int finish, hipStream_t s) {
  hipLaunchKernelGGL(k_ck, dim3(CK_HEAVY_BLOCKS + blocks_for((size_t)d.W * d.H, A7_ROWS * A7_ITEMS)), dim3(A7_ROWS, A7_ITEMS), 0, s, d, flt, st, sc,
                     ck_out, finish);
}
void launch_ck_finish(const Dims &d, const Filter &flt, const Scratch &sc, const float *parts, int n_parts, size_t part_stride, hipStream_t s) {
  hipLaunchKernelGGL(k_ck_finish, dim3(blocks_for((size_t)d.W * d.H)), dim3(TPB), 0, s, d, flt, sc, parts, n_parts,
                     part_stride ? part_stride : (size_t)d.W * d.H);
}
void launch_ck_reduce_chunk(const float *stage, const float *own_part, float *full, uint32_t chunk, int world, int rank, hipStream_t s) {
  hipLaunchKernelGGL(k_ck_reduce_chunk, dim3((chunk + TPB - 1) / TPB), dim3(TPB), 0, s, stage, own_part, full, chunk, world, rank);
}
void launch_weight(const Dims &d, const Filter &flt, const State &st, const Scratch &sc, hipStream_t s, const float *ck_raw) {
  const int side = 2 * d.window_half + 1;
#define SDM_WEIGHT(UU, RR)                                                                                              \
  if (ck_raw) hipLaunchKernelGGL((k_weight<UU, RR, true>), dim3(WT_GRID), dim3(64 * WT_WAVES), 0, s, d, flt, st, sc, ck_raw); \
  else hipLaunchKernelGGL((k_weight<UU, RR, false>), dim3(WT_GRID), dim3(64 * WT_WAVES), 0, s, d, flt, st, sc, ck_raw);
  if (side * side <= 64) {
    SDM_WEIGHT(4, 1)
  } else if (side * side <= 128) {
    SDM_WEIGHT(4, 2)
  } else {
    SDM_WEIGHT(2, 4)
  }
#undef SDM_WEIGHT
}

int launch_birth_prepare(const Dims &d, const Filter &flt, const BirthOrder &bo, const State &st,
                         const Scratch &sc, hipStream_t s) {
  const size_t hw = (size_t)d.W * d.H;
  const size_t total = hw * flt.nb;
  if (flt.use_rng) {
    hipLaunchKernelGGL(k_birth_flags, dim3(blocks_for(hw)), dim3(TPB), 0, s, d, bo, sc);
    exclusive_scan_u32(sc.b_valid, sc.b_rank, hw, sc.scan_scratch_b, s);
  }
  hipLaunchKernelGGL(k_birth_candidates, dim3(blocks_for(total)), dim3(TPB), 0, s, d, flt, bo, st, sc);
  if (flt.use_rng) hipLaunchKernelGGL(k_birth_cursor, dim3(1), dim3(64), 0, s, d, flt, sc);
  int nbits = d.x_n + d.y_n + d.z_n + 1;
  return radix_sort_pairs(sc.bkey_a, sc.bval_a, sc.bkey_b, sc.bval_b, total, nbits, sc.sort_scratch, s);
}

void launch_birth_replay(const Dims &d, const Filter &flt, const State &st, const Scratch &sc, int which, bool literal,
                         hipStream_t s) {
  const size_t total = (size_t)d.W * d.H * flt.nb;
  const uint32_t *skey = which ? sc.bkey_b : sc.bkey_a;
  const uint32_t *sval = which ? sc.bval_b : sc.bval_a;
  dim3 grid(blocks_for(total));
#define SDM_BIRTH(SS)                                                                                                  \
  if (literal) hipLaunchKernelGGL((k_birth_replay<SS, true>), grid, dim3(TPB), 0, s, d, flt, st, sc, skey, sval, (uint32_t)total); \
  else hipLaunchKernelGGL((k_birth_replay<SS, false>), grid, dim3(TPB), 0, s, d, flt, st, sc, skey, sval, (uint32_t)total);
  switch (d.p_n) {
    case 1: SDM_BIRTH(2) break;
    case 2: SDM_BIRTH(4) break;
    case 3: SDM_BIRTH(8) break;
    default: SDM_BIRTH(16) break;
  }
#undef SDM_BIRTH
}

void launch_labeled_cloud(const Dims &d, const CloudArgsHost &h, const float *depth, const uint8_t *static_mask,
                          const uint16_t *label_to_inst, const uint8_t *obj_masks, const double *bbox,
                          sdm_labeled_point *cloud, hipStream_t s) {
  CloudArgs a;
  static_assert(sizeof(CloudArgs) == sizeof(CloudArgsHost), "CloudArgs layout");
  __builtin_memcpy(&a, &h, sizeof(a));
  hipLaunchKernelGGL(k_labeled_cloud, dim3(blocks_for((size_t)d.W * d.H)), dim3(TPB), 0, s, d, a, depth, static_mask, label_to_inst,
                     obj_masks, bbox, cloud);
}

void launch_manual_resize(const Dims &d, const void *src, void *dst, int src_w, int src_h, float scale, int elem_bytes,
                          hipStream_t s) {
  const float scale_inv = 1.f / scale;
  dim3 grid(blocks_for((size_t)d.W * d.H));
  if (elem_bytes == 4)
    hipLaunchKernelGGL(k_manual_resize<float>, grid, dim3(TPB), 0, s, (const float *)src, (float *)dst, src_w, src_h, d.W, d.H, scale_inv);
  else
    hipLaunchKernelGGL(k_manual_resize<uint8_t>, grid, dim3(TPB), 0, s, (const uint8_t *)src, (uint8_t *)dst, src_w, src_h, d.W, d.H,
                       scale_inv);
// ... 143 lines not shown
```

### semantic_dsp_map_amd/csrc/lifecycle.hip

```cpp
#include <rocrand/rocrand.h>

#include <chrono>
#include <cmath>
#include <cstdlib>
#include <mutex>

#include "sdm_map.h"

#pragma clang fp contract(off)

namespace {

thread_local std::string g_last_error;

__attribute__((constructor(101))) void sdm_runtime_defaults() {
  setenv("HIP_FORCE_DEV_KERNARG", "1", 0);
}

constexpr double GRAPH_PIECES_US = 110.0, GRAPH_CHAIN_US = 170.0;
constexpr int LAUNCHES_PER_FRAME = 50;

__global__ void k_noop() {}

}
// ... 300 lines not shown
  }
  if (c.overflow && c.n_moved > m->sc.cap_move) {
    char buf[160];
    snprintf(buf, sizeof(buf), "moved-copy list overflowed: %u particles of moving objects in one frame, more than %u", c.n_moved,
             m->sc.cap_move);
    set_error("capacity", __FILE__, __LINE__, buf);
    return SDM_ERR_CAPACITY;
  }
  if (c.overflow) {
    set_error("capacity", __FILE__, __LINE__, "visible-particle or move list overflowed: more visible particles than sdm_config.max_visible, more in ONE image row than "
              "max(2 max_visible / height, 2 width slots) - raise max_visible -, or more than 2^20 in one pixel's bin");
    return SDM_ERR_CAPACITY;
  }
  if (c.vis_flood_rounds >= 256 && !c.vis_flood_complex) {
    set_error("flood", __FILE__, __LINE__, "frustum flood fill did not converge");
    return SDM_ERR_NOT_CONVERGED;
  }
  return SDM_OK;
}

}

extern "C" {

const char *sdm_last_error(void) { return g_last_error.c_str(); }
const char *sdm_version(void) { return "libsdm_hip 0.1 (gfx950)"; }

static sdm_status map_init(sdm_map *m, const sdm_config *cfg, int shard_count) {
  m->cfg = *cfg;
  m->cfg.shard_count = shard_count;
  m->device = cfg->device;
  Dims &d = m->d;
  d.x_n = cfg->x_n;
  d.y_n = cfg->y_n;
  d.z_n = cfg->z_n;
  d.p_n = cfg->p_n;
  d.NX = 1u << d.x_n;
  d.NY = 1u << d.y_n;
  d.NZ = 1u << d.z_n;
  d.S = 1u << d.p_n;
  d.V = d.NX * d.NY * d.NZ;
  d.rz_count = d.NZ / shard_count;
  d.rz_begin = d.rz_count * cfg->shard_rank;
  d.v_count = d.V / shard_count;
  d.v_begin = d.v_count * cfg->shard_rank;
  d.voxel_size = cfg->voxel_size;
  d.recip = 1.f / cfg->voxel_size;
  d.pmax[0] = (d.NX >> 1) * cfg->voxel_size;
  d.pmax[1] = (d.NY >> 1) * cfg->voxel_size;
  d.pmax[2] = (d.NZ >> 1) * cfg->voxel_size;
  for (int a = 0; a < 3; ++a) d.pmin[a] = -d.pmax[a];
  d.W = cfg->width;
  d.H = cfg->height;
  d.fx = cfg->fx;
  d.fy = cfg->fy;
  d.cx = cfg->cx;
  d.cy = cfg->cy;
  d.dmin = cfg->depth_min;
  d.dmax = cfg->depth_max;
  d.tanx = (float)tan(atan2(cfg->width / 2.0, (double)cfg->fx));
  d.tany = (float)tan(atan2(cfg->height / 2.0, (double)cfg->fy));
  d.occl_coeff = 0.1f + 1.f;
  d.window_half = cfg->window_half;
  d.max_movable = cfg->max_movable_track;
  m->stamps_x.assign(d.NX, 0);
  m->stamps_y.assign(d.NY, 0);
  m->stamps_z.assign(d.NZ, 0);
  m->prm.detection_probability = 0.95f;
  m->prm.noise_number = 0.1f;
  m->prm.nb_ptc_num_per_point = 3;
  m->prm.occupancy_threshold = 0.2f;
  m->prm.max_obersevation_lost_time = 5;
  m->prm.forgetting_rate = 1.0f;
  m->prm.max_forget_count = 5;
  m->prm.match_score_threshold = 0.3f;
  m->prm.id_transition_probability = 0.1f;
  m->prm.if_consider_depth_noise = 0;
  m->prm.if_use_independent_filter = 0;
  m->prm.depth_noise_first_order = 0.f;
  m->prm.depth_noise_zero_order = 0.1f;

  for (hipStream_t *s : {&m->own_stream, &m->s_frustum, &m->s_birth}) HIP_TRY(new_stream(cfg->device, s));
  m->stream = m->own_stream;
  for (hipEvent_t *e : {&m->ev_state, &m->ev_counts, &m->ev_begin, &m->ev_frustum, &m->ev_birth, &m->ev_fa, &m->ev_vis, &m->cap_begin,
                        &m->cap_frustum, &m->cap_birth, &m->ev_copy, &m->raw[0].ev_free, &m->raw[1].ev_free})
    SDM_TRY(new_event(m, e, hipEventDisableTiming));
  const size_t n_slots = (size_t)d.v_count * d.S;
  const size_t hw = (size_t)d.W * d.H;
#define A(ptr, n) SDM_TRY(alloc_tracked(m, &(ptr), (n)))
  A(m->st.pos4, n_slots);
  A(m->st.forget, n_slots);
  HIP_TRY(hipMemsetAsync(m->st.forget, 0, n_slots, m->stream));
  A(m->st.rec, rec_array_bytes(d.v_count, d.S));
  const size_t v_groups = ((size_t)d.v_count + 511) / 512 * 512;
  A(m->st.vts, v_groups + 64);
  A(m->st.vflag, v_groups + 64);
  m->st.tile_stride = (uint32_t)tile_mark_bytes(d);
  A(m->st.tile_dirty, 2 * (size_t)m->st.tile_stride);
  A(m->st.occ_need, ((size_t)d.v_count + 63) / 64 + 32);
  A(m->st.occ_list, occ_list_tiles(d.v_count) * OCC_LIST_CAP);
  A(m->st.occ_list_n, occ_list_tiles(d.v_count) + 64);
  m->st.occ_unit_cap = (uint32_t)((occ_list_tiles(d.v_count) + OCC_LIST_SHARDS - 1) / OCC_LIST_SHARDS * (OCC_LIST_CAP / OCC_LIST_UNIT));
  A(m->st.occ_unit, (size_t)OCC_LIST_SHARDS * m->st.occ_unit_cap);
  A(m->st.occ_shard, OCC_LIST_SHARDS + 1);
  HIP_TRY(hipMemsetAsync(m->st.occ_shard, 0, (OCC_LIST_SHARDS + 1) * sizeof(State::OccListShard), m->stream));
  A(m->st.grp_hint, grp_hint_bytes(d.v_count));
  HIP_TRY(hipMemsetAsync(m->st.grp_hint, 0, grp_hint_bytes(d.v_count), m->stream));
  A(m->st.owner, n_slots);
  A(m->st.owner_flag, owner_flag_bytes(n_slots));
  A(m->st.owner_flag2, owner_flag2_bytes(n_slots));
  A(m->st.alias, 2 + 2 * ALIAS_CAP);
  m->st.alias_cap = ALIAS_CAP;
  HIP_TRY(hipMemsetAsync(m->st.alias, 0, 8, m->stream));
  A(m->st.alias_filter, ALIAS_FILTER_WORDS);
  HIP_TRY(hipMemsetAsync(m->st.alias_filter, 0, ALIAS_FILTER_WORDS * 4, m->stream));
  A(m->st.res, d.v_count);
  A(m->st.stamps_x, d.NX);
  A(m->st.stamps_y, d.NY);
  A(m->st.stamps_z, d.NZ);
  A(m->st.pdf, PDF_NUM);
  m->noise_n = 1000000;
  A(m->st.noise, m->noise_n);
  HIP_TRY(hipMemsetAsync(m->st.noise, 0, (size_t)m->noise_n * 4, m->stream));
  {
    std::vector<float> pdf;
    build_pdf_table(pdf);
    HIP_TRY(hipMemcpyAsync(m->st.pdf, pdf.data(), PDF_NUM * 4, hipMemcpyHostToDevice, m->stream));
    HIP_TRY(hipStreamSynchronize(m->stream));
  }
  Scratch &sc = m->sc;
  sc.wpl = (int)((d.NX + 1 + 63) / 64);
  const size_t n_words = (size_t)(d.NZ + 1) * (d.NY + 1) * sc.wpl;
  A(sc.vmask, n_words);
  A(sc.reach, n_words);
  sc.wy = (int)((d.NY + 1 + 63) / 64);
  const size_t n_line_words = (size_t)(d.NZ + 1) * sc.wy;
  A(sc.line_ne, n_line_words);
  A(sc.line_ey, n_line_words);
  A(sc.line_ez, n_line_words);
  A(sc.line_reach, n_line_words);
  A(m->d_depth, hw);
  A(m->d_cloud, hw);
  A(sc.bin_count, hw + 1 + (size_t)d.H * ROW_SUBS * ROW_CNT_STRIDE);
  A(sc.row_win, hw);
  sc.row_cnt = sc.bin_count + hw + 1;
  A(sc.bin_start, (size_t)d.H * (d.W + 1));
  size_t cap_vis = cfg->max_visible > 0 ? (size_t)cfg->max_visible
                                        : std::min<size_t>(n_slots + (size_t)VIS_SHARDS * 256 * d.S, (size_t)16 << 20);
  cap_vis = (cap_vis + VIS_SHARDS - 1) / VIS_SHARDS * VIS_SHARDS;
  cap_vis = std::min<size_t>(cap_vis, 0xffffff00u);
  sc.cap_vis = (uint32_t)cap_vis;
  {
    const size_t row_total = std::min<size_t>(cap_vis, std::max<size_t>(2 * cap_vis / (size_t)d.H, (size_t)2 * d.W * d.S));
    sc.row_cap = (uint32_t)std::max<size_t>(64, (row_total + row_total / 4) / ROW_SUBS + 64);
  }
  A(sc.row_list, (size_t)d.H * ROW_SUBS * sc.row_cap);
  A(sc.bin_idx, cap_vis);
  A(sc.vpix, cap_vis);
  A(sc.vp4, cap_vis);
  A(sc.vtf, cap_vis);
  A(sc.pix4, hw);
  A(sc.pixt, hw);
  A(sc.ck_kappa, hw);
  sc.cap_heavy = (uint32_t)(((hw + 255) / 256 + VIS_SHARDS - 1) / VIS_SHARDS * 256);
  A(sc.ck_heavy, (size_t)sc.cap_heavy * VIS_SHARDS);
  A(sc.ck_class, hw);
  m->ck_chunk = (uint32_t)(((hw + shard_count - 1) / shard_count + 63) / 64 * 64);
  A(m->d_ck_part, (size_t)m->ck_chunk * shard_count);
  for (auto &r : m->raw) {
    A(r.depth, hw);
    A(r.static_mask, hw);
    A(r.label_to_inst, 256);
    A(r.bbox, 6 * MAX_CLOUD_OBJECTS);
  }
  A(sc.b_valid, hw + 1);
  A(sc.b_rank, hw + 1);
  sc.cap_move = (uint32_t)std::min<size_t>((size_t)d.V * d.S, (size_t)1 << 18);
  A(m->d_counts_local, HALO_OBJ);
  const size_t mv_cnt_n = move_count_elems();
  A(sc.mv_cnt, mv_cnt_n);
  A(sc.mv_list, 8192);
  A(sc.mv_nlist, 4);
  HIP_TRY(hipMemsetAsync(sc.mv_nlist, 0, 4 * sizeof(uint32_t), m->stream));
  A(sc.mv_nmem, 8192);
  A(sc.mv_mem, move_member_elems(n_slots));
  A(sc.mv_tot, move_total_elems());
  HIP_TRY(hipMemsetAsync(sc.mv_tot, 0, move_total_elems() * sizeof(uint32_t), m->stream));
  A(m->d_track_bits, 2048);
  A(sc.mv_copy, sc.cap_move);
  A(sc.track_to_obj, 65536);
  HIP_TRY(hipMemsetAsync(sc.track_to_obj, 0xFF, 65536, m->stream));
  size_t scan_need = scan_scratch_elems(hw + 1);
  A(sc.scan_scratch, scan_need + 16);
  A(sc.scan_scratch_b, scan_scratch_elems(hw + 1) + 16);
  HIP_TRY(hipMemsetAsync(sc.scan_scratch, 0, (scan_need + 16) * 4, m->stream));
  HIP_TRY(hipMemsetAsync(sc.scan_scratch_b, 0, (scan_scratch_elems(hw + 1) + 16) * 4, m->stream));
  A(sc.mv_row, (size_t)d.v_count * MV_ROW);
  HIP_TRY(hipMemsetAsync(sc.mv_row, 0xff, (size_t)d.v_count * MV_ROW * sizeof(uint32_t), m->stream));
  A(sc.mv_next, sc.cap_move);
  A(sc.cnt, 1);
  A(sc.cur, 1);
  HIP_TRY(hipMemsetAsync(sc.cnt, 0, sizeof(Counters), m->stream));
  HIP_TRY(hipMemsetAsync(sc.cur, 0, sizeof(Cursors), m->stream));
  A(m->d_fa[0], 1);
  A(m->d_fa[1], 1);
  A(m->d_fa[2], 1);
  for (FrameArgs *p : m->d_fa) HIP_TRY(hipMemsetAsync(p, 0, sizeof(FrameArgs), m->stream));
  m->sc.fa = m->d_fa[0];
  m->sc.fa_side = m->d_fa[1];
  m->sc.fa_moves = m->d_fa[2];
  A(m->d_u64, 1);
  A(m->emit.mask, emit_mask_bytes(d));
  A(m->emit.blk_cnt, emit_block_elems(d));
  A(m->emit.total, 4);
#undef A
  m->cur_depth = m->d_depth;
  m->cur_cloud = m->d_cloud;
  {
    const char *e = getenv("SDM_GRAPH");
    if (e && e[0] >= '0' && e[0] <= '4') m->graph_mode = e[0] - '0';
    if (const char *k = getenv("SDM_SWEEP_SKIP_SCAN")) m->sweep_skip_allowed = atoi(k) != 0;
    m->host_timing = getenv("SDM_HOST_TIMING") != nullptr;
  }
  {
    int lds_max = 0;
    if (hipDeviceGetAttribute(&lds_max, hipDeviceAttributeSharedMemPerBlockOptin, cfg->device) != hipSuccess || lds_max <= 0)
      (void)hipDeviceGetAttribute(&lds_max, hipDeviceAttributeMaxSharedMemoryPerBlock, cfg->device);
    (void)hipGetLastError();
    if ((size_t)(d.NZ + 1) * sc.wy * 32 > (size_t)std::min(lds_max, 152 * 1024)) m->force_generic_flood = 1;
  }
  refresh_filter(m);
  build_birth_order(m);
  SDM_TRY(ensure_birth_buffers(m));
  for (hipEvent_t &e : m->ev) SDM_TRY(new_event(m, &e, hipEventDefault));
  host_initialize(m);
  launch_clear(d, m->st, m->stream, true);
  SDM_TRY(upload_stamps(m));
  HIP_TRY(hipStreamSynchronize(m->stream));
  {
    hipLaunchKernelGGL(k_noop, dim3(1), dim3(1), 0, m->stream);
    HIP_TRY(hipStreamSynchronize(m->stream));
    double burst[5];
    for (int rep = 0; rep < 5; ++rep) {
      const auto t0 = std::chrono::steady_clock::now();
      for (int i = 0; i < 16; ++i) hipLaunchKernelGGL(k_noop, dim3(1), dim3(1), 0, m->stream);
      burst[rep] = std::chrono::duration<double, std::micro>(std::chrono::steady_clock::now() - t0).count();
      HIP_TRY(hipStreamSynchronize(m->stream));
    }
    std::sort(burst, burst + 5);
    static std::mutex best_mu;
    static double best_seen = 0.0;
    double best = burst[0];
    {
      std::lock_guard<std::mutex> g(best_mu);
      if (best_seen == 0.0 || best < best_seen) best_seen = best;
      best = best_seen;
    }
    m->enqueue_us = best / 16.0 * LAUNCHES_PER_FRAME;
    issue_mode_for(m, m->graph_mode, &m->use_graph, &m->graph_shape);
  }
  return SDM_OK;
}

sdm_status sdm_create(const sdm_config *cfg, sdm_map **out) {
  if (!cfg || !out) return SDM_ERR_INVALID_ARGUMENT;
  *out = nullptr;
  if (cfg->x_n + cfg->y_n + cfg->z_n + cfg->p_n > 31 || cfg->x_n < 2 || cfg->y_n < 2 || cfg->z_n < 2 || cfg->p_n < 1 ||
      cfg->p_n > 4 || cfg->x_n > 9 || cfg->y_n > 9 || cfg->z_n > 9 || cfg->width <= 0 || cfg->height <= 0 || !(cfg->voxel_size > 0.f) ||
      cfg->window_half < 0 || cfg->window_half > 7) {
    set_error("sdm_create", __FILE__, __LINE__, "invalid configuration");
    return SDM_ERR_INVALID_ARGUMENT;
  }
  int shard_count = cfg->shard_count > 0 ? cfg->shard_count : 1;
  if (cfg->shard_rank < 0 || cfg->shard_rank >= shard_count || ((1u << cfg->z_n) % (uint32_t)shard_count) != 0) {
    set_error("sdm_create", __FILE__, __LINE__, "invalid shard rank/count (count must divide the z axis)");
    return SDM_ERR_INVALID_ARGUMENT;
  }
  if (cfg->width >= (1 << ROW_COL_BITS)) {
    set_error("sdm_create", __FILE__, __LINE__, "image width above 4095 (the row kernel of the pixel bins holds one image row in LDS)");
    return SDM_ERR_INVALID_ARGUMENT;
  }
  int ndev = 0;
  if (hipGetDeviceCount(&ndev) != hipSuccess || ndev <= 0 || cfg->device < 0 || cfg->device >= ndev) {
    set_error("sdm_create", __FILE__, __LINE__, "no HIP device / bad device ordinal: libsdm_hip has no CPU path");
    return SDM_ERR_NO_DEVICE;
  }
  HIP_TRY(hipSetDevice(cfg->device));
  {
    const char *e = getenv("SDM_NUMA_BIND");
    if (!(e && e[0] == '0')) (void)bind_host_thread_to(cfg->device);
  }
  sdm_map *m = new sdm_map();
  const sdm_status rc = map_init(m, cfg, shard_count);
  if (rc == SDM_OK) *out = m;
  else (void)sdm_destroy(m);
  return rc;
}

sdm_status sdm_destroy(sdm_map *m) {
  if (!m) return SDM_ERR_INVALID_ARGUMENT;
  if (m->host_timing) {
    const double ng = m->n_graph_frames ? (double)m->n_graph_frames : 1.0, nd = m->n_direct_frames ? (double)m->n_direct_frames : 1.0;
    fprintf(stderr, "sdm host timing: prepare+inputs %.1f us/frame; graph frames %llu: set-params %.1f us, hipGraphLaunch %.1f us; direct frames %llu: %.1f us\n",
            m->t_prepare_us / (ng + nd - ((m->n_graph_frames && m->n_direct_frames) ? 0.0 : 1.0)), (unsigned long long)m->n_graph_frames,
// ... 96 lines not shown
```

### semantic_dsp_map_amd/csrc/moves.hip

```cpp
#include <hip/hip_ext.h>
#include "sdm_internal.h"
#include "sdm_scratch.h"

#pragma clang fp contract(off)

namespace sdm {

#ifdef SDM_AB_TIMERS
__device__ unsigned long long g_dbg_m[4][4096 * 4];
void debug_timers_moves(unsigned long long *out, int reset) {
  (void)hipMemcpyFromSymbol(out, HIP_SYMBOL(g_dbg_m), sizeof(g_dbg_m));
  if (reset) {
    static unsigned long long z[4][4096 * 4];
    (void)hipMemcpyToSymbol(HIP_SYMBOL(g_dbg_m), z, sizeof(z));
  }
}
#define DBGM(k, i, v) do { if (blockIdx.x < 4096 && threadIdx.x == 0) g_dbg_m[k][blockIdx.x * 4 + (i)] = (unsigned long long)(v); } while (0)
#define DBGM_T() wall_clock64()
#define DBGM_MAX(i, v) atomicMax(&g_dbg_m[1][2048 * 4 + (i)], (unsigned long long)(v))
#define DBGM_ADD(i, v) atomicAdd(&g_dbg_m[1][2048 * 4 + (i)], (unsigned long long)(v))
#else
#define DBGM(k, i, v)
#define DBGM_T() 0ull
#define DBGM_MAX(i, v)
// ... 209 lines not shown
    }
    __syncthreads();
    {
      uint32_t *mem = sc.mv_mem + (size_t)pos * MV_CHUNK;
#pragma unroll
      for (int r = 0; r < MV_ITEMS; ++r) {
        if (ent[r] == MV_COMPLEX) continue;
        const uint32_t o = (ent[r] >> 12) & 63u;
        const uint32_t rank = (ent[r] >> 18) + rank_cnt[r][wid][o];
        mem[all_cnt[r][wid] + pre[r]] = ((uint32_t)r * TPB + threadIdx.x) | o << 12 | rank << 18;
      }
    }
    DBGM(2, 2, DBGM_T());
  }
  DBGM(2, 3, DBGM_T());
}
__global__ __launch_bounds__(TPB) void k_move_members(State st, MembersArgs ma, const FrameArgs *__restrict__ fa) {
  const int n_obj = fa->n_obj;
  if (n_obj <= 0) return;
  move_members_body(st, ma, ma.n_flags, ma.n_slots, n_obj, fa->ms.track, fa->mv_seq);
}
__global__ __launch_bounds__(TPB) void k_move_members_v(State st, MembersArgs ma, const FrameArgs src, FrameArgs *__restrict__ dst) {
  if (blockIdx.x == 0) {
    const uint32_t *s4 = reinterpret_cast<const uint32_t *>(&src);
    uint32_t *d4 = reinterpret_cast<uint32_t *>(dst);
    for (uint32_t i = threadIdx.x; i < sizeof(FrameArgs) / 4; i += blockDim.x) d4[i] = s4[i];
  }
  if (src.n_obj <= 0) return;
  move_members_body(st, ma, ma.n_flags, ma.n_slots, src.n_obj, src.ms.track, src.mv_seq);
}

__global__ __launch_bounds__(TPB) void k_frame_begin(Counters *cnt, uint32_t *__restrict__ bin_count, uint32_t n_bins,
                                                      State st, const FrameArgs src, FrameArgs *__restrict__ dst_main,
                                                      FrameArgs *__restrict__ dst_side, Dims d, uint32_t slab_max, MembersArgs ma,
                                                      int with_members) {
  const StampUpdates &su = src.su;
  DBGM(3, 0, DBGM_T());
  if (blockIdx.x == gridDim.x - 1) {
    const uint32_t *s4 = reinterpret_cast<const uint32_t *>(&src);
    uint32_t *m4 = reinterpret_cast<uint32_t *>(dst_main), *e4 = reinterpret_cast<uint32_t *>(dst_side);
    for (uint32_t k = threadIdx.x; k < sizeof(FrameArgs) / 4; k += blockDim.x) {
      m4[k] = s4[k];
      if (e4) e4[k] = s4[k];
    }
  }
  uint32_t i = blockIdx.x * blockDim.x + threadIdx.x;
  for (uint32_t t = i; t < slab_max * (uint32_t)su.n; t += gridDim.x * blockDim.x) mark_slab_voxel_dirty(d, st, su, slab_max, t);
  if (i < offsetof(Counters, flood_complex) / 4) reinterpret_cast<uint32_t *>(cnt)[i] = 0;
  if (i < (uint32_t)su.n) {
    const uint32_t e = su.entry[i], axis = e >> 12, idx = e & 0xfffu;
    uint32_t *arr = axis == 0 ? st.stamps_x : (axis == 1 ? st.stamps_y : st.stamps_z);
    arr[idx] = su.value;
  }
  for (; i < n_bins; i += gridDim.x * blockDim.x) bin_count[i] = 0;
  DBGM(3, 1, DBGM_T());
  if (with_members && src.n_obj > 0) move_members_body(st, ma, ma.n_flags, ma.n_slots, src.n_obj, src.ms.track, src.mv_seq);
}

struct HaloRecord {
  float x, y, z;
  uint32_t forget_bits;
  float w;
  uint32_t voxel;
  uint32_t e;
  uint32_t ts_track;
  uint32_t owner_label_status;
};
static_assert(sizeof(HaloRecord) == HALO_RECORD_BYTES, "halo record layout");

__global__ void k_move_local_counts(int32_t *counts_local, Scratch sc, const FrameArgs *__restrict__ fa, int reset_export) {
  const int k = threadIdx.x;
  const int n_obj = fa->n_obj;
  const uint32_t world = sc.halo_world;
  if (sc.halo_send && reset_export)
    for (uint32_t dst = (uint32_t)k; dst < world; dst += blockDim.x)
      *reinterpret_cast<uint32_t *>(sc.halo_send + (size_t)dst * halo_segment_bytes(sc.halo_cap)) = 0;
  if (k >= HALO_OBJ) return;
  const uint32_t *tot = sc.mv_tot + (size_t)(fa->mv_seq & 1u) * MAX_MOVE_OBJECTS * MV_TOT_STRIDE;
  counts_local[k] = k < n_obj ? (int32_t)tot[k * MV_TOT_STRIDE] : 0;
}

constexpr uint32_t MV_NIL = 0xffffffffu;

__device__ __forceinline__ void move_link(const Dims &d, const Scratch &sc, uint32_t v, uint32_t e, uint32_t forget_bits) {
  const uint32_t lv = v - d.v_begin;
  uint32_t *row = sc.mv_row + (size_t)lv * MV_ROW;
  const uint32_t k = atomicAdd(&row[0], 1u) + 1u;
  if (k < (uint32_t)MV_DIRECT) {
    row[1 + k] = e;
    if (k == 0u) sc.mv_copy[e].forget_bits = forget_bits | MV_FIRST;
  } else {
    const uint32_t prev = atomicExch(&row[MV_ROW - 1], e);
    sc.mv_next[e] = prev;
  }
}

struct MoveLoaded {
  float4 p;
  float n[3];
  float w;
  uint16_t ts, track;
  uint8_t label, status;
};
__device__ __forceinline__ void move_load_particle(const Dims &d, const State &st, size_t li, bool copy_invalid, MoveLoaded &m) {
  m.p = st.pos4[li];
  m.p.w = __uint_as_float((uint32_t)st.forget[li]);
  const SlotRef sr = slot_ref_li(st, d.p_n, li);
  m.w = sr.w();
  m.ts = sr.ts();
  m.track = sr.track();
  m.label = sr.label();
  m.status = copy_invalid ? (uint8_t)ST_INVALID : sr.status();
}
__device__ __forceinline__ void move_load_noise(const Filter &flt, const State &st, long long cursor, uint32_t e, MoveLoaded &m) {
  const long long draw = cursor + 3ll * e;
  m.n[0] = st.noise[(draw + 1) % flt.noise_n];
  m.n[1] = st.noise[(draw + 2) % flt.noise_n];
  m.n[2] = st.noise[(draw + 3) % flt.noise_n];
}
__device__ __forceinline__ MoveLoaded move_load(const Dims &d, const Filter &flt, const State &st, long long cursor, uint32_t e,
                                                size_t li, bool copy_invalid) {
  MoveLoaded m;
  move_load_particle(d, st, li, copy_invalid, m);
  move_load_noise(flt, st, cursor, e, m);
  return m;
}
__device__ __forceinline__ void move_store(const Dims &d, const Frame &f, const MoveSet &ms, const State &st, const Scratch &sc,
                                           const MoveLoaded &m, int obj, uint32_t e, size_t li, bool alias) {
  const float4 p = m.p;
  const float *T = ms.T[obj];
  float nx = row4(T + 0, p.x, p.y, p.z);
  float ny = row4(T + 4, p.x, p.y, p.z);
  float nz = row4(T + 8, p.x, p.y, p.z);
  nx = nx + m.n[0];
  ny = ny + m.n[1];
  nz = nz + m.n[2];
  const float pw = m.w;
  const uint16_t pts = m.ts, ptrack = m.track;
  const uint8_t plabel = m.label, pstatus = m.status;
  const uint16_t powner = ms.track[obj];
  slot_ref_li(st, d.p_n, li).set_status(ST_INVALID);
  st.vflag[li >> d.p_n] = VF_DIRTY;
  mark_tile(st, li >> d.p_n, f.epoch);
  if (!alias) st.owner[li] = OWNER_NONE;
  uint32_t rx, ry, rz;
  uint32_t v = global_pos_to_voxel(d, f, nx, ny, nz, rx, ry, rz);
  if (v == INVALID_INDEX) return;
  if (rz >= d.rz_begin && rz < d.rz_begin + d.rz_count) {
    if (e >= sc.cap_move) return;
    MoveCopy c;
    c.x = nx;
    c.y = ny;
    c.z = nz;
    c.forget_bits = __float_as_uint(p.w) & 0xffu;
    c.w = pw;
    c.ts = pts;
    c.track = ptrack;
    c.owner = powner;
    c.label = plabel;
    c.status = pstatus;
    c.voxel = v - d.v_begin;
    sc.mv_copy[e] = c;
    move_link(d, sc, v, e, c.forget_bits);
  } else if (sc.halo_send) {
    unsigned char *seg = sc.halo_send + (size_t)(rz / d.rz_count) * halo_segment_bytes(sc.halo_cap);
    uint32_t k = atomicAdd(reinterpret_cast<uint32_t *>(seg), 1u);
    if (k < sc.halo_cap) {
      HaloRecord r;
      r.x = nx;
      r.y = ny;
      r.z = nz;
      r.forget_bits = __float_as_uint(p.w);
      r.w = pw;
      r.voxel = v;
      r.e = e;
      r.ts_track = (uint32_t)pts | ((uint32_t)ptrack << 16);
      r.owner_label_status = (uint32_t)powner | ((uint32_t)plabel << 16) | ((uint32_t)pstatus << 24);
      reinterpret_cast<HaloRecord *>(seg + HALO_HEADER_BYTES)[k] = r;
    } else {
      sc.cnt->overflow = 1;
      atomicAdd(&sc.cnt->n_halo_dropped, 1u);
    }
  }
}
__device__ __forceinline__ void move_one(const Dims &d, const Frame &f, const Filter &flt, const MoveSet &ms, const State &st,
                                         const Scratch &sc, int obj, uint32_t e, size_t li, bool alias = false,
                                         bool copy_invalid = false) {
  const MoveLoaded m = move_load(d, flt, st, (long long)sc.cur->move_cursor, e, li, copy_invalid);
  move_store(d, f, ms, st, sc, m, obj, e, li, alias);
}

constexpr uint32_t CA_CAP = 512;
struct ChunkAliases {
  const uint32_t *idx;
  const uint32_t *ent;
  const uint8_t *obj;
  uint32_t n;
};
__device__ __forceinline__ uint32_t aliases_below(const ChunkAliases &ca, uint32_t o, uint32_t li) {
  uint32_t c = 0;
  for (uint32_t k = 0; k < ca.n; ++k) c += (ca.obj[k] == o && ca.idx[k] < li) ? 1u : 0u;
  return c;
}
__device__ __forceinline__ uint32_t primaries_below(const uint32_t *mem, uint32_t nm, uint32_t o, uint32_t s) {
  uint32_t c = 0;
  for (uint32_t i = 0; i < nm; ++i) {
    const uint32_t en = mem[i];
    if ((en & 4095u) >= s) break;
    c += ((en >> 12) & 63u) == o ? 1u : 0u;
  }
  return c;
}
__device__ __forceinline__ void move_slot_memberships(const Dims &d, const Frame &f, const Filter &flt, const MoveSet &ms, const State &st,
                                                      const Scratch &sc, const ChunkAliases &ca, const uint32_t *mem, uint32_t nm,
                                                      const uint32_t *obj_base, size_t li, uint32_t s, uint32_t prim_o, uint32_t prim_rank) {
  int last = -1;
  bool first = true;
  for (;;) {
    uint32_t ob = 0xFFu, entry = 0;
    bool is_alias = false;
    if (prim_o != 0xFFu && (int)prim_o > last) ob = prim_o;
    for (uint32_t k = 0; k < ca.n; ++k)
      if (ca.idx[k] == (uint32_t)li && (int)ca.obj[k] > last && ca.obj[k] < ob) {
        ob = ca.obj[k];
        entry = ca.ent[k];
        is_alias = true;
      }
    if (ob == 0xFFu) break;
    const uint32_t below = (!is_alias ? prim_rank : primaries_below(mem, nm, ob, s)) + aliases_below(ca, ob, (uint32_t)li);
    move_one(d, f, flt, ms, st, sc, (int)ob, obj_base[ob] + below, li, is_alias, !first);
    if (is_alias) st.alias[3 + 2 * entry] = OWNER_NONE;
    last = (int)ob;
    first = false;
  }
}

__global__ __launch_bounds__(TPB) void k_move_apply(Dims d, Filter flt, State st, Scratch sc, const int32_t *__restrict__ counts_all,
                                                    int world, int rank) {
  uint32_t pos = blockIdx.x;
  uint32_t nm = sc.mv_nmem[pos], listed = sc.mv_list[pos];
  uint32_t first_entry = sc.mv_mem[(size_t)pos * MV_CHUNK + threadIdx.x];
  uint32_t my_c = threadIdx.x < MAX_MOVE_OBJECTS ? sc.mv_cnt[(size_t)threadIdx.x * MV_LIST_CAP + pos] : 0u;
  uint32_t tot2[2] = {0u, 0u};
  if (threadIdx.x < MAX_MOVE_OBJECTS) {
    tot2[0] = sc.mv_tot[(size_t)threadIdx.x * MV_TOT_STRIDE];
    tot2[1] = sc.mv_tot[((size_t)MAX_MOVE_OBJECTS + threadIdx.x) * MV_TOT_STRIDE];
  }
  const long long cursor = (long long)sc.cur->move_cursor;
  const uint32_t n = *sc.mv_nlist;
  const uint32_t na_raw = st.alias[0];
  const int n_obj = sc.fa->n_obj;
  if (n_obj <= 0) return;
  DBGM(0, 0, DBGM_T());
  const Frame f = sc.fa->f;
  const MoveSet &ms = sc.fa->ms;
  const uint32_t par = sc.fa->mv_seq & 1u;
  const uint32_t batch = sc.fa->mv_batch;
  const uint32_t e_base = batch ? sc.cnt->n_moved_b[(batch - 1u) & 1u] : 0u;
  __shared__ uint32_t obj_base[MAX_MOVE_OBJECTS];
  __shared__ uint32_t obj_first[MAX_MOVE_OBJECTS];
  __shared__ uint32_t c_here[MAX_MOVE_OBJECTS];
  __shared__ uint32_t tot_l[MAX_MOVE_OBJECTS];
  __shared__ uint16_t tracks[MAX_MOVE_OBJECTS];
  __shared__ uint32_t ca_idx[CA_CAP], ca_ent[CA_CAP], ca_n;
  __shared__ uint8_t ca_obj[CA_CAP];
  __shared__ uint32_t cm_mem[MV_CHUNK];
  const int lane = threadIdx.x & 63, wid = threadIdx.x >> 6;
  const size_t n_slots = (size_t)d.v_count * d.S;
  if (threadIdx.x < MAX_MOVE_OBJECTS) {
    tracks[threadIdx.x] = (int)threadIdx.x < n_obj ? ms.track[threadIdx.x] : OWNER_NONE;
    tot_l[threadIdx.x] = (int)threadIdx.x < n_obj ? tot2[par] : 0u;
  }
  __syncthreads();
  if ((int)threadIdx.x < n_obj) {
    uint32_t run = 0;
    if (counts_all) {
      for (int k = 0; k < (int)threadIdx.x; ++k)
        for (int r = 0; r < world; ++r) run += (uint32_t)counts_all[r * HALO_OBJ + k];
      for (int r = 0; r < rank; ++r) run += (uint32_t)counts_all[r * HALO_OBJ + threadIdx.x];
    } else {
      for (int k = 0; k < (int)threadIdx.x; ++k) run += tot_l[k];
    }
    obj_first[threadIdx.x] = e_base + run;
  }
  if (blockIdx.x == 0) {
    if (threadIdx.x == 0) {
      uint32_t total = 0;
      if (counts_all) {
        for (int k = 0; k < n_obj; ++k)
          for (int r = 0; r < world; ++r) total += (uint32_t)counts_all[r * HALO_OBJ + k];
      } else {
        for (int k = 0; k < n_obj; ++k) total += tot_l[k];
      }
      sc.cnt->n_moved = e_base + total;
      sc.cnt->n_moved_b[batch & 1u] = e_base + total;
      if (e_base + total > sc.cap_move || sc.cur->move_list_overflow) sc.cnt->overflow = 1;
    }
    if (threadIdx.x < MAX_MOVE_OBJECTS) sc.mv_tot[((size_t)(par ^ 1u) * MAX_MOVE_OBJECTS + threadIdx.x) * MV_TOT_STRIDE] = 0;
  }
  const uint64_t lt_mask = (lane == 0) ? 0ull : (~0ull >> (64 - lane));
  const uint32_t na_total = na_raw < st.alias_cap ? na_raw : st.alias_cap;
  while (pos < n) {
    const uint32_t chunk = listed & ~MV_CLEAR_FLAG;
    const size_t base = (size_t)chunk * MV_CHUNK;
    __syncthreads();
    if ((int)threadIdx.x < n_obj) c_here[threadIdx.x] = my_c;
    if (threadIdx.x == 0 && (listed & MV_CLEAR_FLAG)) st.owner_flag[chunk] = 0;
    MoveLoaded ml;
    const bool simple = (nm & MV_COMPLEX_BIT) == 0u;
    const uint32_t nm_raw = nm;
    nm &= ~MV_COMPLEX_BIT;
    const bool mine = threadIdx.x < nm;
    if (mine) move_load_particle(d, st, base + (first_entry & 4095u), false, ml);
    __syncthreads();
    if (nm_raw != 0) {
      for (int k = wid; k < n_obj; k += MV_WAVES) {
        if (c_here[k] == 0) continue;
        uint32_t sum = 0;
        const uint32_t *row = sc.mv_cnt + (size_t)k * MV_LIST_CAP;
        for (uint32_t p = (uint32_t)lane; p < pos; p += 64) sum += row[p];
#pragma unroll
        for (int off = 32; off >= 1; off >>= 1) sum += __shfl_xor(sum, off, 64);
        if (lane == 0) obj_base[k] = obj_first[k] + sum;
      }
      __syncthreads();
      DBGM(0, 1, DBGM_T());
      if (simple) {
        if (mine) {
          const uint32_t o = (first_entry >> 12) & 63u;
          const uint32_t e = obj_base[o] + (first_entry >> 18);
          move_load_noise(flt, st, cursor, e, ml);
          move_store(d, f, ms, st, sc, ml, (int)o, e, base + (first_entry & 4095u), false);
        }
        for (uint32_t i = TPB + threadIdx.x; i < nm; i += TPB) {
          const uint32_t en = sc.mv_mem[(size_t)pos * MV_CHUNK + i];
          const uint32_t o = (en >> 12) & 63u;
          move_one(d, f, flt, ms, st, sc, (int)o, obj_base[o] + (en >> 18), base + (en & 4095u));
        }
        DBGM(0, 2, DBGM_T());
      } else {
        if (threadIdx.x == 0) ca_n = 0;
        for (uint32_t i = threadIdx.x; i < nm; i += TPB) cm_mem[i] = i == threadIdx.x ? first_entry : sc.mv_mem[(size_t)pos * MV_CHUNK + i];
        __syncthreads();
        for (uint32_t k = threadIdx.x; k < na_total; k += blockDim.x) {
          const uint32_t idx = st.alias[2 + 2 * k], trk = st.alias[3 + 2 * k];
          if (trk == OWNER_NONE || idx / MV_CHUNK != chunk) continue;
          const uint8_t o = obj_of((uint16_t)trk, tracks, n_obj);
          if (o == 0xFF) continue;
          const uint32_t c = atomicAdd(&ca_n, 1u);
          if (c < CA_CAP) {
            ca_idx[c] = idx;
            ca_obj[c] = o;
            ca_ent[c] = k;
          }
        }
        __syncthreads();
        ChunkAliases ca;
        ca.idx = ca_idx;
        ca.ent = ca_ent;
        ca.obj = ca_obj;
        ca.n = ca_n < CA_CAP ? ca_n : CA_CAP;
        if (threadIdx.x == 0 && ca_n > CA_CAP) sc.cnt->overflow = 1;
        for (uint32_t i = threadIdx.x; i < nm; i += TPB) {
          const uint32_t en = cm_mem[i], sl = en & 4095u, o = (en >> 12) & 63u;
          const size_t li = base + sl;
          bool shared_slot = false;
          for (uint32_t k = 0; k < ca.n; ++k) shared_slot = shared_slot || ca.idx[k] == (uint32_t)li;
          if (!shared_slot) {
            const uint32_t e = obj_base[o] + (en >> 18) + aliases_below(ca, o, (uint32_t)li);
            if (i == threadIdx.x) {
              move_load_noise(flt, st, cursor, e, ml);
              move_store(d, f, ms, st, sc, ml, (int)o, e, li, false);
            } else {
              move_one(d, f, flt, ms, st, sc, (int)o, e, li);
            }
          } else {
            move_slot_memberships(d, f, flt, ms, st, sc, ca, cm_mem, nm, obj_base, li, sl, o, en >> 18);
          }
        }
        for (uint32_t c = threadIdx.x; c < ca.n; c += TPB) {
          const uint32_t li = ca.idx[c], sl = li - (uint32_t)base;
          bool other = false;
          for (uint32_t k = 0; k < c; ++k) other = other || ca.idx[k] == li;
          for (uint32_t i = 0; i < nm && !other; ++i) {
            const uint32_t s2 = cm_mem[i] & 4095u;
            if (s2 >= sl) {
              other = s2 == sl;
              break;
            }
          }
          if (!other) move_slot_memberships(d, f, flt, ms, st, sc, ca, cm_mem, nm, obj_base, li, sl, 0xFFu, 0u);
        }
      }
    }
    pos += gridDim.x;
    if (pos < n) {
      nm = sc.mv_nmem[pos];
      listed = sc.mv_list[pos];
      first_entry = sc.mv_mem[(size_t)pos * MV_CHUNK + threadIdx.x];
      my_c = threadIdx.x < MAX_MOVE_OBJECTS ? sc.mv_cnt[(size_t)threadIdx.x * MV_LIST_CAP + pos] : 0u;
    }
  }
  DBGM(0, 3, DBGM_T());
}

__global__ __launch_bounds__(TPB) void k_move_import(Dims d, Scratch sc, int world, int rank) {
  if (sc.fa->n_obj <= 0) return;
  const int src = blockIdx.y;
  if (src == rank || src >= world) return;
  const unsigned char *buf = sc.halo_recv + (size_t)src * halo_segment_bytes(sc.halo_cap);
  uint32_t n = *reinterpret_cast<const uint32_t *>(buf);
  if (n > sc.halo_cap) n = sc.halo_cap;
  const HaloRecord *rec = reinterpret_cast<const HaloRecord *>(buf + HALO_HEADER_BYTES);
  uint32_t stride = gridDim.x * blockDim.x;
  for (uint32_t k = blockIdx.x * blockDim.x + threadIdx.x; k < n; k += stride) {
    const HaloRecord r = rec[k];
    uint32_t rz = (r.voxel >> (d.x_n + d.y_n)) & (d.NZ - 1);
    if (rz < d.rz_begin || rz >= d.rz_begin + d.rz_count) continue;
    const uint32_t e = r.e;
    if (e >= sc.cap_move) continue;
    MoveCopy c;
    c.x = r.x;
    c.y = r.y;
    c.z = r.z;
    c.forget_bits = r.forget_bits & 0xffu;
    c.w = r.w;
    c.ts = (uint16_t)(r.ts_track & 0xffffu);
    c.track = (uint16_t)(r.ts_track >> 16);
    c.owner = (uint16_t)(r.owner_label_status & 0xffffu);
    c.label = (uint8_t)((r.owner_label_status >> 16) & 0xffu);
    c.status = (uint8_t)(r.owner_label_status >> 24);
    c.voxel = r.voxel - d.v_begin;
    sc.mv_copy[e] = c;
    move_link(d, sc, r.voxel, e, c.forget_bits);
  }
}

constexpr int RP_TPB = 64;
constexpr int RP_GRID = 1024;
constexpr int RP_KEEP = 96;
constexpr uint8_t RP_SORT16[63][2] = {
    {0, 1}, {2, 3}, {0, 2}, {1, 3}, {1, 2}, {4, 5}, {6, 7}, {4, 6}, {5, 7}, {5, 6}, {0, 4}, {2, 6}, {2, 4}, {1, 5}, {3, 7}, {3, 5},
    {1, 2}, {3, 4}, {5, 6}, {8, 9}, {10, 11}, {8, 10}, {9, 11}, {9, 10}, {12, 13}, {14, 15}, {12, 14}, {13, 15}, {13, 14}, {8, 12},
    {10, 14}, {10, 12}, {9, 13}, {11, 15}, {11, 13}, {9, 10}, {11, 12}, {13, 14}, {0, 8}, {4, 12}, {4, 8}, {2, 10}, {6, 14}, {6, 10},
    {2, 4}, {6, 8}, {10, 12}, {1, 9}, {5, 13}, {5, 9}, {3, 11}, {7, 15}, {7, 11}, {3, 5}, {7, 9}, {11, 13}, {1, 2}, {3, 4}, {5, 6},
    {7, 8}, {9, 10}, {11, 12}, {13, 14}};
static_assert(MV_ROW == 16, "the row's ranks are sorted by a 16-key network");
template <int S>
__global__ __launch_bounds__(RP_TPB) void k_move_replay(Dims d, Filter flt, State st, Scratch sc) {
  uint32_t t = blockIdx.x * blockDim.x + threadIdx.x;
  MoveCopy c0;
  c0.voxel = MV_NIL;
  if (t < sc.cap_move) c0 = sc.mv_copy[t];
  const uint32_t n_alias = st.alias[0];
  if (sc.fa->n_obj <= 0) return;
  const uint32_t n_moved = sc.cnt->n_moved;
  if (blockIdx.x == 0 && threadIdx.x == 0) {
    long long c = (long long)sc.cur->move_cursor + 3ll * (long long)n_moved;
    sc.cur->move_cursor = (int32_t)(c % flt.noise_n);
  }
  const uint32_t n_copies = n_moved < sc.cap_move ? n_moved : sc.cap_move;
  const uint32_t epoch = sc.fa->f.epoch;
  const uint32_t stride = gridDim.x * blockDim.x;
  const bool overflow = sc.cnt->overflow != 0;
  bool first_round = true;
  __shared__ uint32_t n_ok_block;
  __shared__ uint32_t kept[RP_KEEP][RP_TPB];
  if (threadIdx.x == 0) n_ok_block = 0;
  __syncthreads();
  for (; t < n_copies; t += stride) {
    if (first_round) {
      first_round = false;
    } else {
      c0 = sc.mv_copy[t];
    }
    DBGM(1, 0, DBGM_T());
    [[maybe_unused]] const unsigned long long dbg_t0 = DBGM_T();
    const uint32_t lv = c0.voxel;
    if (lv >= d.v_count || !(c0.forget_bits & MV_FIRST)) continue;
    uint32_t *const row = sc.mv_row + (size_t)lv * MV_ROW;
    uint32_t rk[MV_ROW];
    {
      const uint4 *rp = reinterpret_cast<const uint4 *>(row);
#pragma unroll
      for (int q = 0; q < MV_ROW / 4; ++q) {
        const uint4 x = rp[q];
        rk[4 * q] = x.x;
        rk[4 * q + 1] = x.y;
        rk[4 * q + 2] = x.z;
        rk[4 * q + 3] = x.w;
      }
    }
    const uint32_t v = d.v_begin + lv;
    uint32_t rx, ry, rz;
    voxel_to_ring(d, v, rx, ry, rz);
    uint32_t a = st.stamps_x[rx], b = st.stamps_y[ry], c = st.stamps_z[rz];
    const size_t base = (size_t)lv * S;
    uint8_t stv[S];
    uint16_t tsv[S];
    unsigned char *const rec = rec_ptr(st, S, lv);
    float wv[S];
    uint16_t trk[S];
    uint8_t lab[S], fg[S];
    {
      stv[0] = ST_TIMEPTC;
      tsv[0] = 0;
      wv[0] = 0.f;
      trk[0] = 0;
      lab[0] = 0;
      __builtin_memcpy(&wv[1], __builtin_assume_aligned(rec, 2), 4 * (S - 1));
      __builtin_memcpy(&tsv[1], rec + 4 * (S - 1), 2 * (S - 1));
      __builtin_memcpy(&trk[1], rec + 6 * (S - 1), 2 * (S - 1));
      __builtin_memcpy(&lab[1], rec + 8 * (S - 1), S - 1);
      __builtin_memcpy(&stv[1], rec + 9 * (S - 1), S - 1);
      __builtin_memcpy(fg, st.forget + base, S);
    }
    float px[S], py[S], pz[S];
// ... 286 lines not shown
inline unsigned blocks_for(size_t n, int tpb = TPB) { return (unsigned)((n + tpb - 1) / tpb); }

}

void launch_owner_flags(const Dims &d, const State &st, hipStream_t s) {
  const size_t n_slots = (size_t)d.v_count * d.S;
  hipMemsetAsync(st.owner_flag2, 0, owner_flag2_bytes(n_slots), s);
  hipLaunchKernelGGL(k_owner_flags, dim3((unsigned)((n_slots + OWNER_CHUNK - 1) / OWNER_CHUNK)), dim3(TPB), 0, s, st.owner, n_slots,
                     st.owner_flag, st.owner_flag2);
}

void launch_tracks_with_particles(const Dims &d, const State &st, uint32_t *bitmap, hipStream_t s) {
  const size_t n_slots = (size_t)d.v_count * d.S;
  hipMemsetAsync(bitmap, 0, 2048 * sizeof(uint32_t), s);
  const size_t n_chunks = (n_slots + OWNER_CHUNK - 1) / OWNER_CHUNK;
  hipLaunchKernelGGL(k_tracks_with_particles, dim3((unsigned)((n_chunks + OWNER_GROUP - 1) / OWNER_GROUP)), dim3(TPB), 0, s, st, n_slots, bitmap);
}

size_t move_blocks(const Dims &d) { return ((size_t)d.v_count * d.S + MV_CHUNK - 1) / MV_CHUNK; }
size_t move_count_elems() { return (size_t)MAX_MOVE_OBJECTS * MV_LIST_CAP + 1; }
size_t move_member_elems(size_t n_slots) {
  const size_t n_chunks = (n_slots + MV_CHUNK - 1) / MV_CHUNK;
  return std::min<size_t>(MV_LIST_CAP, std::max<size_t>(n_chunks, 1024)) * MV_CHUNK;
}
size_t move_total_elems() { return (size_t)2 * MAX_MOVE_OBJECTS * MV_TOT_STRIDE; }

static MembersArgs members_args(const Dims &d, const Scratch &sc) {
  MembersArgs ma;
  ma.mv_cnt = sc.mv_cnt;
  ma.mv_list = sc.mv_list;
  ma.mv_nlist = sc.mv_nlist;
  ma.mv_nmem = sc.mv_nmem;
  ma.mv_mem = sc.mv_mem;
  ma.mv_tot = sc.mv_tot;
  ma.cur = sc.cur;
  ma.n_flags = (uint32_t)move_blocks(d);
  ma.n_slots = (size_t)d.v_count * d.S;
  return ma;
}
void launch_moves_count(const Dims &d, const State &st, const Scratch &sc, int32_t *counts_local, hipStream_t s, const FrameArgs *by_value) {
  const FrameArgs *fa = by_value ? sc.fa_moves : sc.fa_side;
  const MembersArgs ma = members_args(d, sc);
  if (by_value)
    hipLaunchKernelGGL(k_move_members_v, dim3(MV_GRID), dim3(TPB), 0, s, st, ma, *by_value, const_cast<FrameArgs *>(sc.fa_moves));
  else
    hipLaunchKernelGGL(k_move_members, dim3(MV_GRID), dim3(TPB), 0, s, st, ma, fa);
  if (d.v_count != d.V) hipLaunchKernelGGL(k_move_local_counts, dim3(1), dim3(HALO_OBJ), 0, s, counts_local, sc, fa, 1);
}

void launch_moves_batch(const Dims &d, const State &st, const Scratch &sc, const FrameArgs &fa_batch, int32_t *counts_local, hipStream_t s) {
  const MembersArgs ma = members_args(d, sc);
  hipLaunchKernelGGL(k_move_members_v, dim3(MV_GRID), dim3(TPB), 0, s, st, ma, fa_batch, const_cast<FrameArgs *>(sc.fa));
  if (d.v_count != d.V) hipLaunchKernelGGL(k_move_local_counts, dim3(1), dim3(HALO_OBJ), 0, s, counts_local, sc, sc.fa, 0);
}

void FrameBeginLaunch::set(const Dims &d_, const State &st_, const Scratch &sc, const FrameArgs &fa_, bool with_side, bool with_members_) {
  cnt = sc.cnt;
  bin_count = sc.bin_count;
  n_bins = (uint32_t)(d_.W * d_.H + 1 + d_.H * (int)(ROW_SUBS * ROW_CNT_STRIDE));
  st = st_;
  fa = fa_;
  dst_main = const_cast<FrameArgs *>(sc.fa);
  dst_side = with_side ? const_cast<FrameArgs *>(sc.fa_side) : nullptr;
  d = d_;
  slab_max = d_.NY * d_.NZ;
  if (d_.NX * d_.NZ > slab_max) slab_max = d_.NX * d_.NZ;
  if (d_.NX * d_.NY > slab_max) slab_max = d_.NX * d_.NY;
  ma = members_args(d_, sc);
  with_members = with_members_ ? 1 : 0;
  argv[0] = &cnt;
  argv[1] = &bin_count;
  argv[2] = &n_bins;
  argv[3] = &st;
  argv[4] = &fa;
  argv[5] = &dst_main;
  argv[6] = &dst_side;
  argv[7] = &d;
  argv[8] = &slab_max;
  argv[9] = &ma;
  argv[10] = &with_members;
}
const void *FrameBeginLaunch::kernel() { return reinterpret_cast<const void *>(k_frame_begin); }

void launch_frame_begin(FrameBeginLaunch &a, hipStream_t s, hipEvent_t done) {
  if (done) (void)hipExtLaunchKernel(FrameBeginLaunch::kernel(), dim3(FrameBeginLaunch::GRID), dim3(FrameBeginLaunch::BLOCK), a.argv, 0, s, nullptr, done, 0);
  else (void)hipLaunchKernel(FrameBeginLaunch::kernel(), dim3(FrameBeginLaunch::GRID), dim3(FrameBeginLaunch::BLOCK), a.argv, 0, s);
}

void launch_moves_transform(const Dims &d, const Filter &flt, const State &st, const Scratch &sc, const int32_t *counts_all, int world,
                            int rank, hipStream_t s) {
  hipLaunchKernelGGL(k_move_apply, dim3(1024), dim3(TPB), 0, s, d, flt, st, sc, d.v_count != d.V ? counts_all : nullptr, world, rank);
}

void launch_moves_finish(const Dims &d, const Filter &flt, const State &st, const Scratch &sc, int world, int rank, hipStream_t s) {
  if (world > 1 && sc.halo_recv) hipLaunchKernelGGL(k_move_import, dim3(64, world), dim3(TPB), 0, s, d, sc, world, rank);
  dim3 grid(RP_GRID);
  switch (d.p_n) {
    case 1: hipLaunchKernelGGL(k_move_replay<2>, grid, dim3(RP_TPB), 0, s, d, flt, st, sc); break;
    case 2: hipLaunchKernelGGL(k_move_replay<4>, grid, dim3(RP_TPB), 0, s, d, flt, st, sc); break;
    case 3: hipLaunchKernelGGL(k_move_replay<8>, grid, dim3(RP_TPB), 0, s, d, flt, st, sc); break;
    default: hipLaunchKernelGGL(k_move_replay<16>, grid, dim3(RP_TPB), 0, s, d, flt, st, sc); break;
  }
}

void launch_remove(const Dims &d, const State &st, const Scratch &sc, hipStream_t s) {
  const size_t n_slots = (size_t)d.v_count * d.S;
  const size_t n_chunks = (n_slots + OWNER_CHUNK - 1) / OWNER_CHUNK;
  hipLaunchKernelGGL(k_remove, dim3((unsigned)(n_chunks < 1024 ? n_chunks : 1024)), dim3(TPB), 0, s, st, n_slots, sc.fa, d.p_n);
}

}
```

### semantic_dsp_map_amd/csrc/readback.hip

```cpp
#include <cmath>

#include "sdm_map.h"

extern "C" {

sdm_status sdm_get_labeled_cloud(sdm_map *m, sdm_labeled_point *out) {
  if (!m || !out) return SDM_ERR_INVALID_ARGUMENT;
  HIP_TRY(hipSetDevice(m->device));
  HIP_TRY(hipMemcpyAsync(out, m->cur_cloud, (size_t)m->d.W * m->d.H * sizeof(sdm_labeled_point), hipMemcpyDeviceToHost, m->stream));
  HIP_TRY(hipStreamSynchronize(m->stream));
  return SDM_OK;
}

sdm_status sdm_device_alloc(sdm_map *m, size_t bytes, void **out) {
  if (!m || !out) return SDM_ERR_INVALID_ARGUMENT;
  HIP_TRY(hipSetDevice(m->device));
  HIP_TRY(hipMalloc(out, bytes ? bytes : 1));
  return SDM_OK;
}
sdm_status sdm_device_free(sdm_map *m, void *p) {
  if (!m) return SDM_ERR_INVALID_ARGUMENT;
  HIP_TRY(hipSetDevice(m->device));
  HIP_TRY(hipFree(p));
  return SDM_OK;
// ... 63 lines not shown
    for (int a = 0; a < 3; ++a) sub[a] = m->cam_p[a];
  uint32_t cap32 = (uint32_t)std::min<size_t>(cap, 0xffffffffu);
  launch_emit_points(m->d, m->f, m->st, m->emit, m->d_points, cap32, want_free, sub, (flags & SDM_POINTS_MARK_FOV) ? 1 : 0, m->stream);
  return fetch_points(m, m->d_points, out, sizeof(sdm_point), cap, n_out);
}
sdm_status sdm_get_occupied(sdm_map *m, sdm_point *out, size_t cap, size_t *n_out, int32_t flags) {
  return get_points(m, out, cap, n_out, flags, 0);
}
sdm_status sdm_get_freespace(sdm_map *m, sdm_point *out, size_t cap, size_t *n_out, int32_t flags) {
  return get_points(m, out, cap, n_out, flags, 1);
}
sdm_status sdm_set_colours(sdm_map *m, const sdm_colour_config *c) {
  if (!m || !c) return SDM_ERR_INVALID_ARGUMENT;
  HIP_TRY(hipSetDevice(m->device));
  ColourTables t;
  memset(&t, 0, sizeof(t));
  t.cfg = *c;
  for (int i = 1; i < 256; ++i) {
    t.sdiv[i] = (int32_t)nearbyint((double)(255 << 12) / (1.0 * i));
    t.hdiv180[i] = (int32_t)nearbyint((double)(180 << 12) / (6.0 * i));
  }
  if (!m->d_colours) SDM_TRY(alloc_tracked(m, &m->d_colours, 1));
  HIP_TRY(hipMemcpyAsync(m->d_colours, &t, sizeof(t), hipMemcpyHostToDevice, m->stream));
  HIP_TRY(hipStreamSynchronize(m->stream));
  m->colours_set = true;
  return SDM_OK;
}

static sdm_status get_points_rgb(sdm_map *m, sdm_point_xyzrgb *out, size_t cap, size_t *n_out, int flags, int want_free) {
  if (!m || !n_out || (cap && !out)) return SDM_ERR_INVALID_ARGUMENT;
  if (!m->colours_set) {
    set_error("sdm_get_occupied_rgb", __FILE__, __LINE__, "call sdm_set_colours first");
    return SDM_ERR_INVALID_ARGUMENT;
  }
  HIP_TRY(hipSetDevice(m->device));
  if (cap > m->points_rgb_cap) SDM_TRY(regrow(m, &m->d_points_rgb, &m->points_rgb_cap, cap));
  float sub[3] = {0.f, 0.f, 0.f};
  if (flags & SDM_POINTS_ZERO_CENTER)
    for (int a = 0; a < 3; ++a) sub[a] = m->cam_p[a];
  uint32_t cap32 = (uint32_t)std::min<size_t>(cap, 0xffffffffu);
  launch_emit_points_rgb(m->d, m->f, m->st, m->d_colours, m->emit, m->d_points_rgb, cap32, want_free, sub, m->stream);
  return fetch_points(m, m->d_points_rgb, out, sizeof(sdm_point_xyzrgb), cap, n_out);
}
sdm_status sdm_get_occupied_rgb(sdm_map *m, sdm_point_xyzrgb *out, size_t cap, size_t *n_out, int32_t flags) {
  return get_points_rgb(m, out, cap, n_out, flags, 0);
}
sdm_status sdm_get_freespace_rgb(sdm_map *m, sdm_point_xyzrgb *out, size_t cap, size_t *n_out, int32_t flags) {
  return get_points_rgb(m, out, cap, n_out, flags, 1);
}

sdm_status sdm_voxels_device_ptr(sdm_map *m, const sdm_voxel_result **out) {
  if (!m || !out) return SDM_ERR_INVALID_ARGUMENT;
  *out = m->st.res;
  return SDM_OK;
}

sdm_status sdm_object_particle_count(sdm_map *m, int32_t track_id, int64_t *count) {
  if (!m || !count || track_id < 0 || track_id > 65535) return SDM_ERR_INVALID_ARGUMENT;
  HIP_TRY(hipSetDevice(m->device));
  launch_count_owner(m->d, m->st, (uint16_t)track_id, m->d_u64, m->stream);
  unsigned long long c = 0;
  HIP_TRY(hipMemcpyAsync(&c, m->d_u64, 8, hipMemcpyDeviceToHost, m->stream));
  HIP_TRY(hipStreamSynchronize(m->stream));
  *count = (int64_t)c;
  return SDM_OK;
}

sdm_status sdm_tracks_with_particles(sdm_map *m, int32_t *out, int32_t cap, int32_t *n_out) {
  if (!m || !n_out || cap < 0 || (cap > 0 && !out)) return SDM_ERR_INVALID_ARGUMENT;
  HIP_TRY(hipSetDevice(m->device));
  launch_tracks_with_particles(m->d, m->st, m->d_track_bits, m->stream);
  if (!m->h_track_bits) SDM_TRY(alloc_tracked(m, &m->h_track_bits, 2048, true));
  uint32_t *bits = m->h_track_bits;
  HIP_TRY(hipMemcpyAsync(bits, m->d_track_bits, 2048 * sizeof(uint32_t), hipMemcpyDeviceToHost, m->stream));
  HIP_TRY(hipStreamSynchronize(m->stream));
  int32_t n = 0;
  bits[2047] &= 0x7fffffffu;
  for (uint32_t w = 0; w < 2048u; ++w)
    for (uint32_t b = bits[w]; b; b &= b - 1u) {
      if (n < cap) out[n] = (int32_t)(w * 32u + (uint32_t)__builtin_ctz(b));
      ++n;
    }
  *n_out = n;
  return SDM_OK;
}

sdm_status sdm_get_stats(sdm_map *m, sdm_stats *out, int32_t count_live) {
  if (!m || !out) return SDM_ERR_INVALID_ARGUMENT;
  HIP_TRY(hipSetDevice(m->device));
  Counters c;
  sdm_status rc = check_counters(m, &c);
  memset(out, 0, sizeof(*out));
  out->n_visible = c.n_vis;
  out->n_birth_attempts = c.n_birth_attempts;
  out->n_birth_success = c.n_birth_success;
  out->n_resampled_voxels = c.n_resampled;
  for (uint32_t k = 0; k < VIS_SHARDS; ++k) {
    out->n_birth_success += c.shard[k].birth;
    out->n_resampled_voxels += c.shard[k].resample;
  }
  out->n_moved = c.n_moved;
  out->n_move_reinserted = c.n_move_reinserted;
  for (uint32_t k = 0; k < VIS_SHARDS; ++k) out->n_frustum_voxels += c.shard[k].fv;
  out->bfs_start_in_frustum = c.vis_start_in_frustum;
  for (uint32_t k = 0; k < VIS_SHARDS; ++k) {
    out->sweep_live_voxels += c.shard[k].sweep;
    out->sweep_tiles += c.shard[k].sweep_tiles;
  }
  out->flood_rounds = c.vis_flood_rounds;
  for (int a = 0; a < 3; ++a) out->restamped_slabs[a] = m->restamped[a];
  out->graph_frames = (int64_t)m->n_graph_frames;
  out->direct_frames = (int64_t)m->n_direct_frames;
  out->host_enqueue_us = m->enqueue_us;
  out->halo_dropped = c.n_halo_dropped;
  {
    uint32_t al[2] = {0, 0};
    HIP_TRY(hipMemcpyAsync(al, m->st.alias, 8, hipMemcpyDeviceToHost, m->stream));
    HIP_TRY(hipStreamSynchronize(m->stream));
    out->alias_entries = al[0] < m->st.alias_cap ? al[0] : m->st.alias_cap;
    out->alias_overflowed = (al[0] > m->st.alias_cap || al[1] != 0) ? 1 : 0;
  }
  if (m->profiling) {
    int prev = 0;
    for (int sidx = 1; sidx <= 7; ++sidx) {
      if (!m->stage_ran[sidx]) continue;
      float ms = 0.f;
      if (hipEventElapsedTime(&ms, m->ev[prev], m->ev[sidx]) == hipSuccess) out->stage_ms[sidx] = ms;
      prev = sidx;
    }
  }
  if (count_live) {
    launch_count_live(m->d, m->st, m->d_u64, m->stream);
    unsigned long long n = 0;
    HIP_TRY(hipMemcpyAsync(&n, m->d_u64, 8, hipMemcpyDeviceToHost, m->stream));
    HIP_TRY(hipStreamSynchronize(m->stream));
    out->live_particles = (int64_t)(n & ((1ull << 36) - 1));
    out->live_voxels = (int64_t)(n >> 36);
    size_t nocc = 0;
    launch_emit_count(m->d, m->st, m->emit, 0, m->stream);
    uint32_t total = 0;
    HIP_TRY(hipMemcpyAsync(&total, m->emit.total, 4, hipMemcpyDeviceToHost, m->stream));
    HIP_TRY(hipStreamSynchronize(m->stream));
    nocc = total;
    out->n_occupied = (int64_t)nocc;
  }
  return rc;
}

sdm_status sdm_set_profiling(sdm_map *m, int32_t on) {
  if (!m) return SDM_ERR_INVALID_ARGUMENT;
  m->profiling = on != 0;
  return SDM_OK;
}

sdm_status sdm_get_ring_state(sdm_map *m, sdm_ring_state *o) {
  if (!m || !o) return SDM_ERR_INVALID_ARGUMENT;
  HIP_TRY(hipSetDevice(m->device));
  Cursors c;
  HIP_TRY(hipMemcpyAsync(&c, m->sc.cur, sizeof(c), hipMemcpyDeviceToHost, m->stream));
  HIP_TRY(hipStreamSynchronize(m->stream));
  o->global_time_stamp = m->global_time_stamp;
  for (int a = 0; a < 3; ++a) {
    o->moved_steps[a] = m->moved_steps[a];
    o->eq_steps[a] = m->eq_steps[a];
    o->map_center[a] = m->map_center[a];
    o->last_pos[a] = m->last_pos[a];
// ... 204 lines not shown
```

### semantic_dsp_map_amd/csrc/sdm_internal.h

```cpp
#pragma once
#include <hip/hip_runtime.h>
#include <stdint.h>

#include "../../include/sdm.h"

#pragma clang fp contract(off)

namespace sdm {

constexpr uint32_t INVALID_INDEX = 0xffffffffu;
constexpr uint16_t OWNER_NONE = 0xFFFF;
constexpr int PDF_NUM = 20000;
#define SDM_OCC_INIT_WEIGHT 0.05f
#define SDM_MIN_RIGHT_PDF 0.1f

enum : uint8_t { ST_INVALID = 0, ST_UPDATED = 1, ST_REGULAR_BORN = 2, ST_GUESSED_BORN = 3, ST_COPIED = 4, ST_TIMEPTC = 5 };

struct Dims {
  int x_n, y_n, z_n, p_n;
  uint32_t NX, NY, NZ, S;
  uint32_t V;
  uint32_t v_begin;
  uint32_t v_count;
  uint32_t rz_begin, rz_count;
  float voxel_size, recip;
  float pmin[3], pmax[3];
  int W, H;
  float fx, fy, cx, cy;
  float dmin, dmax;
  float tanx, tany;
  float occl_coeff;
  int window_half;
  int max_movable;
};

struct Frame {
  int eq[3];
  float center[3];
  uint32_t gts;
  uint32_t epoch;
  float E[16];
  int bb0[3], bb1[3];
  int start_v[3];
  int start_ok;
};

struct Filter {
  float p_detect, noise_number, occ_threshold, id_transition;
  float forget[8];
  int independent;
  int consider_depth_noise;
  int nb;
  int use_rng;
  int noise_n;
};

struct Counters {
  uint32_t n_vis;
  uint32_t n_birth_success;
  uint32_t n_birth_attempts;
  uint32_t n_resampled;
  uint32_t n_moved;
  uint32_t n_move_reinserted;
  uint32_t n_frustum_voxels;
  uint32_t n_occupied;
  uint32_t n_free;
  uint32_t overflow;
  uint32_t n_valid_px;
  uint32_t n_halo_dropped;
  uint32_t vis_flood_complex, vis_flood_rounds, vis_start_in_frustum;
  uint32_t n_moved_b[2];
  uint32_t pad[2];
  struct alignas(128) ShardLine {
    uint32_t vis;
    uint32_t fv;
    uint32_t heavy;
    uint32_t birth;
    uint32_t resample;
    uint32_t sweep;
    uint32_t sweep_tiles;
    uint32_t heavy_ticket;
    uint32_t pad[24];
  };
  ShardLine shard[64];
  uint32_t flood_complex;
  uint32_t flood_rounds;
  uint32_t start_in_frustum;
  uint32_t flood_pad[29];
};
static_assert(sizeof(Counters::ShardLine) == 128, "one cache line per shard");
constexpr uint32_t VIS_SHARDS = 64;
constexpr uint32_t ROW_SUBS = 8;
constexpr int ROW_COL_BITS = 12, ROW_PIB_BITS = 32 - ROW_COL_BITS;
constexpr uint32_t ROW_CNT_STRIDE = 32;
constexpr uint32_t OWNER_CHUNK = 4096;
constexpr uint32_t OWNER_GROUP = 64;
__host__ __device__ constexpr size_t owner_flag_bytes(size_t n_slots) {
  return ((n_slots + OWNER_CHUNK - 1) / OWNER_CHUNK + OWNER_GROUP - 1) / OWNER_GROUP * OWNER_GROUP;
}
__host__ __device__ constexpr size_t owner_flag2_bytes(size_t n_slots) { return (owner_flag_bytes(n_slots) / OWNER_GROUP + 4095) / 4096 * 4096; }
constexpr int MAX_STAMP_UPDATES = 96;
struct StampUpdates {
  int n;
  uint32_t value;
  uint16_t entry[MAX_STAMP_UPDATES];
};
struct Cursors {
  int32_t birth_cursor;
  int32_t move_cursor;
  uint32_t move_list_overflow;
};

constexpr size_t REC_BYTES_PER_SLOT = 10;
__host__ __device__ constexpr uint32_t rec_bytes(uint32_t S) { return (uint32_t)REC_BYTES_PER_SLOT * (S - 1u); }
__host__ __device__ constexpr size_t rec_array_bytes(size_t v_count, uint32_t S) { return (v_count + 64) * rec_bytes(S) + 64; }
typedef float rec_f32 __attribute__((aligned(2)));
typedef uint32_t rec_v4u __attribute__((ext_vector_type(4), aligned(2)));
typedef uint32_t rec_v2u __attribute__((ext_vector_type(2), aligned(2)));

struct SlotRef {
  unsigned char *r;
  uint32_t L, k;
  __host__ __device__ __forceinline__ float w() const { return *reinterpret_cast<const rec_f32 *>(r + 4u * k); }
  __host__ __device__ __forceinline__ uint16_t ts() const { return *reinterpret_cast<const uint16_t *>(r + 4u * L + 2u * k); }
  __host__ __device__ __forceinline__ uint16_t track() const { return *reinterpret_cast<const uint16_t *>(r + 6u * L + 2u * k); }
  __host__ __device__ __forceinline__ uint8_t label() const { return r[8u * L + k]; }
  __host__ __device__ __forceinline__ uint8_t status() const { return r[9u * L + k]; }
  __host__ __device__ __forceinline__ void set_w(float v) const { *reinterpret_cast<rec_f32 *>(r + 4u * k) = v; }
  __host__ __device__ __forceinline__ void set_ts(uint16_t v) const { *reinterpret_cast<uint16_t *>(r + 4u * L + 2u * k) = v; }
  __host__ __device__ __forceinline__ void set_track(uint16_t v) const { *reinterpret_cast<uint16_t *>(r + 6u * L + 2u * k) = v; }
  __host__ __device__ __forceinline__ void set_label(uint8_t v) const { r[8u * L + k] = v; }
  __host__ __device__ __forceinline__ void set_status(uint8_t v) const { r[9u * L + k] = v; }
};

struct State {
  float4 *pos4 = nullptr;
  uint8_t *forget = nullptr;
  unsigned char *rec = nullptr;
  uint16_t *vts = nullptr;
  uint8_t *vflag = nullptr;
  uint8_t *tile_dirty = nullptr;
  uint32_t tile_stride = 0;
  unsigned long long *occ_need = nullptr;
  uint16_t *occ_list = nullptr;
  uint32_t *occ_list_n = nullptr;
  uint2 *occ_unit = nullptr;
  uint32_t occ_unit_cap = 0;
  struct alignas(128) OccListShard {
    unsigned long long word;
    uint32_t aux[30];
  };
  OccListShard *occ_shard = nullptr;
  uint8_t *grp_hint = nullptr;
  uint16_t *owner = nullptr;
  uint8_t *owner_flag = nullptr;
// ... 345 lines not shown
```

### semantic_dsp_map_amd/csrc/sdm_map.h

```cpp
#pragma once
#include <algorithm>
#include <cstdio>
#include <cstring>
#include <functional>
#include <string>
#include <vector>

#include "sdm_internal.h"
#include "sdm_scratch.h"

typedef struct ncclComm *ncclComm_t;

namespace sdm {
void set_error(const char *what, const char *file, int line, const char *detail);
}

#define HIP_TRY(expr)                                                        \
  do {                                                                       \
    hipError_t e_ = (expr);                                                  \
    if (e_ != hipSuccess) {                                                  \
      sdm::set_error(#expr, __FILE__, __LINE__, hipGetErrorString(e_));      \
      return SDM_ERR_HIP;                                                    \
    }                                                                        \
  } while (0)
#define NCCL_TRY(expr)                                                       \
  do {                                                                       \
    ncclResult_t r_ = (expr);                                                \
    if (r_ != ncclSuccess) {                                                 \
      sdm::set_error(#expr, __FILE__, __LINE__, ncclGetErrorString(r_));     \
      return SDM_ERR_COMM;                                                   \
    }                                                                        \
  } while (0)
#define SDM_TRY(expr) do { const sdm_status rc_ = (expr); if (rc_ != SDM_OK) return rc_; } while (0)

using namespace sdm;

struct Derived {
  Frame f{};
  uint32_t flags = 0;
  bool valid = false;
  void built(const Frame &from, uint32_t with) { f = from, flags = with, valid = true; }
};
struct QueryStage {
  unsigned char *d = nullptr, *h = nullptr;
  size_t bytes = 0;
};
struct EsdfLayer : Derived {
  uint32_t *site = nullptr, *snap = nullptr;
};
struct InstLayer : Derived {
  unsigned char *acc = nullptr;
  sdm_instance *out = nullptr;
  uint32_t *meta = nullptr;
};
struct FrontLayer : Derived {
  unsigned char *bits = nullptr, *cells = nullptr;
  uint32_t *meta = nullptr, *scan = nullptr;
  size_t alloc = 0;
  int64_t cap = 0;
};
struct ViewPool {
  uint32_t *pool = nullptr;
  uint32_t masks = 0;
  int32_t batch = 0;
  bool clear_rewalk = false;
};
struct ReachLayer : Derived {
  uint32_t *cost = nullptr, *trav = nullptr, *act = nullptr, *list = nullptr;
  uint32_t *meta = nullptr, *h_meta = nullptr;
  uint32_t min_d2 = 0, max_cost = 0;
};

struct sdm_map {
  sdm_config cfg{};
  sdm_params prm{};
  Dims d{};
  Frame f{};
  Filter flt{};
  BirthOrder bo{};
  State st{};
  Scratch sc{};
  hipStream_t stream = nullptr;
  hipStream_t own_stream = nullptr;
  hipStream_t s_frustum = nullptr, s_birth = nullptr, s_moves = nullptr;
  hipEvent_t ev_state = nullptr, ev_counts = nullptr;
  hipEvent_t ev_vis = nullptr;
  bool vis_event_valid = false;
  bool mv_pending = false;
  bool state_event_valid = false;
  hipEvent_t ev_begin = nullptr, ev_frustum = nullptr, ev_birth = nullptr;
  int birth_which = 0;
  float *ck_user = nullptr;
  bool fused_ck = false;
  const float *ck_raw_last = nullptr;
  int32_t stop_after = 0;
  uint32_t frame_flags = 0;
  int n_moves = 0, n_remove = 0;
  std::vector<sdm_object_move> moves_all;
  std::vector<int32_t> removes_all;
  size_t mv_batch_next = 0;
  bool mv_batch_ready = false;
  uint32_t mv_seq = 0;
  uint32_t *d_track_bits = nullptr;
  int32_t *d_counts_local = nullptr;
  ncclComm_t comm = nullptr;
  bool ipc = false;
  unsigned char *ipc_arena = nullptr;
  void *ipc_peer[16] = {};
  uint32_t ipc_seq[4] = {0, 0, 0, 0};
  size_t ipc_off_counts = 0, ipc_off_halo = 0, ipc_off_stage = 0, ipc_off_full = 0, ipc_bytes = 0;
  int ipc_fine_grained = 0;
  float *d_ck_full_local = nullptr;
  int32_t *d_counts_all_local = nullptr;
  uint32_t *d_ipc_sync = nullptr;
  int32_t *d_counts_all = nullptr;
  unsigned char *d_halo_send = nullptr, *d_halo_recv = nullptr;
  float *d_ck_stage = nullptr, *d_ck_full = nullptr;
  uint32_t halo_cap_own = 0;
  size_t ck_part_stride = 0;
  int ck_exchange = 0;
  float *d_ck_all = nullptr;
  int comm_timeout_ms = 30000;
  uint32_t ck_chunk = 0;
  hipEvent_t ev_comm[8]{};
  bool comm_timing = false, comm_timed[4]{};
  bool sharded_frame = false;
  int32_t *counts_local_user = nullptr;
  const int32_t *counts_all_user = nullptr;
  int device = 0;

  std::vector<uint32_t> stamps_x, stamps_y, stamps_z;
  int moved_steps[3]{}, eq_steps[3]{};
  float map_center[3]{}, ego_center[3]{}, last_pos[3]{};
  uint32_t global_time_stamp = 0;
  float forgetting_function[5]{};
  bool forgetting_initialized = false;
  float cam_R[9]{}, cam_p[3]{};
  FrameArgs fa{};
  FrameArgs *d_fa[3]{};
  FrameBeginLaunch fb{};
  hipEvent_t ev_fa = nullptr;
  const float *cur_depth = nullptr;
  const sdm_labeled_point *cur_cloud = nullptr;
  int graph_mode = 2;
  bool use_graph = false;
  int graph_shape = 0;
  hipGraphExec_t piece[5] = {};
  double enqueue_us = 0.0;
  double t_prepare_us = 0, t_setparams_us = 0, t_launch_us = 0, t_direct_us = 0;
  bool host_timing = false;
  bool capturing = false;
  hipGraph_t graph = nullptr;
  hipGraphExec_t graph_exec = nullptr;
  hipGraphNode_t graph_set_node = nullptr;
  Filter graph_flt{};
  hipEvent_t cap_begin = nullptr, cap_frustum = nullptr, cap_birth = nullptr;
  uint64_t n_graph_frames = 0, n_direct_frames = 0;
  int restamped[3]{};
  bool stamps_dirty = true;
  bool sweep_all = true;
  bool sweep_lists = true;
  bool sweep_skip_scan = false;
  bool sweep_skip_allowed = true;
  bool sweep_rec_pending = false;
  int sweep_lists_forced = -1;
  uint32_t sweep_epoch = 1;

  float *d_depth = nullptr;
  sdm_labeled_point *d_cloud = nullptr;
  float *d_ck_part = nullptr;
  struct RawInputs {
    float *depth = nullptr;
    uint8_t *static_mask = nullptr, *obj_masks = nullptr;
    uint16_t *label_to_inst = nullptr;
    uint16_t label_host[256];
    bool label_valid = false;
    double *bbox = nullptr;
    size_t obj_masks_cap = 0;
    hipEvent_t ev_free = nullptr;
  } raw[2];
  int raw_next = 0;
  hipStream_t s_copy = nullptr;
  hipEvent_t ev_copy = nullptr;
  unsigned char *d_src_stage = nullptr;
  size_t src_stage_bytes = 0;
// ... 104 lines not shown
```

### semantic_dsp_map_amd/csrc/sdm_scratch.h

```cpp
#pragma once
#include "sdm_internal.h"

namespace sdm {

struct BirthOrder {
  int off[10];
  int cols[9];
};

struct MoveCopy {
  float x, y, z;
  uint32_t forget_bits;
  float w;
  uint16_t ts, track, owner;
  uint8_t label, status;
  uint32_t voxel;
};
static_assert(sizeof(MoveCopy) == 32, "MoveCopy layout");

constexpr int MAX_MOVE_OBJECTS = 48;
constexpr int MAX_REMOVE_TRACKS = 128;
constexpr int HALO_OBJ = 64;
constexpr int HALO_RECORD_BYTES = 36;
constexpr int HALO_HEADER_BYTES = 16;
__host__ __device__ constexpr size_t halo_segment_bytes(uint32_t cap) { return HALO_HEADER_BYTES + (size_t)cap * HALO_RECORD_BYTES; }
struct MoveSet {
  int n;
  float T[MAX_MOVE_OBJECTS][12];
  uint16_t track[MAX_MOVE_OBJECTS];
};

struct FrameArgs {
  Frame f;
  StampUpdates su;
  MoveSet ms;
  int n_obj;
  int n_remove;
  uint32_t mv_seq;
  uint32_t mv_batch;
  int force_generic;
  const float *depth;
  const sdm_labeled_point *cloud;
  uint16_t remove[MAX_REMOVE_TRACKS];
};
static_assert(sizeof(FrameArgs) <= 3400, "FrameArgs travels as a kernel argument (4 KB limit, with the launch's other arguments)");

constexpr int MV_ROW = 16;
constexpr int MV_DIRECT = MV_ROW - 2;
constexpr uint32_t MV_FIRST = 0x100u;
struct Scratch {
  const FrameArgs *fa = nullptr;
  const FrameArgs *fa_side = nullptr;
  const FrameArgs *fa_moves = nullptr;
  uint64_t *vmask = nullptr, *reach = nullptr;
  int wpl = 0;
  uint64_t *line_ne = nullptr, *line_ey = nullptr, *line_ez = nullptr, *line_reach = nullptr;
  int wy = 0;
  uint32_t *bin_count = nullptr, *bin_start = nullptr;
  uint32_t *row_cnt = nullptr;
  uint8_t *row_win = nullptr;
  uint2 *row_list = nullptr;
  uint32_t row_cap = 0;
  uint32_t cap_vis = 0;
  uint32_t *bin_idx = nullptr, *vpix = nullptr;
  float4 *vp4 = nullptr;
  uint32_t *vtf = nullptr;
  float4 *pix4 = nullptr;
  uint32_t *pixt = nullptr;
  float *ck_kappa = nullptr;
  uint8_t *ck_class = nullptr;
  uint32_t *ck_heavy = nullptr;
  uint32_t cap_heavy = 0;
  uint32_t *b_valid = nullptr, *b_rank = nullptr;
  uint32_t *bkey_a = nullptr, *bval_a = nullptr, *bkey_b = nullptr, *bval_b = nullptr;
  float4 *bpos = nullptr;
  uint32_t *mv_cnt = nullptr;
  uint32_t *mv_list = nullptr, *mv_nlist = nullptr;
  uint32_t *mv_nmem = nullptr, *mv_mem = nullptr, *mv_tot = nullptr;
  MoveCopy *mv_copy = nullptr;
  uint32_t cap_move = 0;
  unsigned char *halo_send = nullptr;
  const unsigned char *halo_recv = nullptr;
  uint32_t halo_cap = 0;
  uint32_t halo_world = 1;
  uint8_t *track_to_obj = nullptr;
  uint32_t *scan_scratch = nullptr, *sort_scratch = nullptr;
  uint32_t *scan_scratch_b = nullptr;
  uint32_t *mv_row = nullptr, *mv_next = nullptr;
  Counters *cnt = nullptr;
  Cursors *cur = nullptr;
};

constexpr int MAX_CLOUD_OBJECTS = 64;
struct CloudArgsHost {
  double R[9], t[3];
  double ifx, icx, ify, icy;
  double dmin, dmax;
  float sigma0, sigma1;
  int consider_depth_noise, consider_instance, n_objects, has_static;
  int sky_instance, has_bbox;
  int track[MAX_CLOUD_OBJECTS], label[MAX_CLOUD_OBJECTS];
};
void launch_labeled_cloud(const Dims &d, const CloudArgsHost &h, const float *depth, const uint8_t *static_mask,
                          const uint16_t *label_to_inst, const uint8_t *obj_masks, const double *bbox,
                          sdm_labeled_point *cloud, hipStream_t s);
void launch_manual_resize(const Dims &d, const void *src, void *dst, int src_w, int src_h, float scale, int elem_bytes,
                          hipStream_t s);

void launch_set_frame(FrameArgs *fa_dev, const FrameArgs &fa, hipStream_t s);
const void *set_frame_kernel();
struct MembersArgs {
  uint32_t *mv_cnt, *mv_list, *mv_nlist, *mv_nmem, *mv_mem, *mv_tot;
  Cursors *cur;
  uint32_t n_flags;
  size_t n_slots;
};
struct FrameBeginLaunch {
#ifndef SDM_FB_GRID
#define SDM_FB_GRID 1024
#endif
  static constexpr unsigned GRID = SDM_FB_GRID, BLOCK = 256;
  Counters *cnt;
  uint32_t *bin_count;
  uint32_t n_bins;
  State st;
  FrameArgs fa;
  FrameArgs *dst_main, *dst_side;
  Dims d;
  uint32_t slab_max;
  MembersArgs ma;
  int with_members;
  void *argv[11];
  void set(const Dims &d, const State &st, const Scratch &sc, const FrameArgs &fa, bool with_side, bool with_members);
  static const void *kernel();
};
void launch_frame_begin(FrameBeginLaunch &a, hipStream_t s, hipEvent_t done = nullptr);
void launch_moves_batch(const Dims &d, const State &st, const Scratch &sc, const FrameArgs &fa_batch, int32_t *counts_local, hipStream_t s);
constexpr int OCC_LISTS = 1, OCC_SKIP_SCAN = 2;
void launch_occupancy(const Dims &d, const Filter &flt, const State &st, Counters *cnt, int all_dirty, const FrameArgs *fa, uint32_t remark,
                      hipStream_t s, int mode = 0);
size_t tile_mark_bytes(const Dims &d);
void launch_frustum(const Dims &d, const Scratch &sc, hipStream_t s);
void launch_visibility(const Dims &d, const Filter &flt, const State &st, const Scratch &sc, float *ck_out, int finish, hipStream_t s,
                       hipEvent_t vis_done = nullptr);
void launch_ck(const Dims &d, const Filter &flt, const State &st, const Scratch &sc, float *ck_out, int finish, hipStream_t s);
void launch_ck_finish(const Dims &d, const Filter &flt, const Scratch &sc, const float *parts, int n_parts, size_t part_stride, hipStream_t s);
void launch_ck_reduce_chunk(const float *stage, const float *own_part, float *full, uint32_t chunk, int world, int rank, hipStream_t s);
void launch_weight(const Dims &d, const Filter &flt, const State &st, const Scratch &sc, hipStream_t s, const float *ck_raw = nullptr);
int launch_birth_prepare(const Dims &d, const Filter &flt, const BirthOrder &bo, const State &st,
                         const Scratch &sc, hipStream_t s);
void launch_birth_replay(const Dims &d, const Filter &flt, const State &st, const Scratch &sc, int which, bool literal,
                         hipStream_t s);
void launch_count_live(const Dims &d, const State &st, unsigned long long *out, hipStream_t s);
void launch_count_owner(const Dims &d, const State &st, uint16_t track, unsigned long long *out, hipStream_t s);
void launch_pack_pos4(float4 *pos4, uint8_t *forget_plane, const float *px, const float *py, const float *pz, const uint8_t *forget, size_t n,
                      hipStream_t s);
void launch_unpack_pos4(const float4 *pos4, const uint8_t *forget_plane, float *px, float *py, float *pz, uint8_t *forget, size_t n, hipStream_t s);
void launch_rec_pack(const Dims &d, const State &st, const float *w, const uint16_t *ts, const uint16_t *track,
                     const uint8_t *label, const uint8_t *status, hipStream_t s);
void launch_rec_unpack(const Dims &d, const State &st, float *w, uint16_t *ts, uint16_t *track, uint8_t *label, uint8_t *status,
                       hipStream_t s);
void launch_fill_dense(const Dims &d, const State &st, uint32_t stamp, int mode, hipStream_t s);
void launch_vflag_from_records(const Dims &d, const State &st, hipStream_t s);
struct ColourTables {
  sdm_colour_config cfg;
  int32_t sdiv[256], hdiv180[256];
};
struct EmitScratch {
  uint8_t *mask = nullptr;
  uint32_t *blk_cnt = nullptr;
  uint32_t *total = nullptr;
};
size_t emit_mask_bytes(const Dims &d);
size_t emit_block_elems(const Dims &d);
void launch_emit_count(const Dims &d, const State &st, const EmitScratch &e, int want_free, hipStream_t s);
void launch_emit_points_rgb(const Dims &d, const Frame &f, const State &st, const ColourTables *ct, const EmitScratch &e,
                            sdm_point_xyzrgb *out, uint32_t cap, int want_free, const float sub[3], hipStream_t s);
void launch_emit_points(const Dims &d, const Frame &f, const State &st, const EmitScratch &e, sdm_point *out, uint32_t cap, int want_free,
                        const float sub[3], int mark_fov, hipStream_t s);

size_t move_blocks(const Dims &d);
size_t move_count_elems();
size_t move_member_elems(size_t n_slots);
size_t move_total_elems();
void launch_tracks_with_particles(const Dims &d, const State &st, uint32_t *bitmap, hipStream_t s);
void launch_owner_flags(const Dims &d, const State &st, hipStream_t s);
void launch_moves_count(const Dims &d, const State &st, const Scratch &sc, int32_t *counts_local, hipStream_t s,
                        const FrameArgs *by_value = nullptr);
void launch_moves_transform(const Dims &d, const Filter &flt, const State &st, const Scratch &sc, const int32_t *counts_all, int world,
                            int rank, hipStream_t s);
void launch_moves_finish(const Dims &d, const Filter &flt, const State &st, const Scratch &sc, int world, int rank, hipStream_t s);
void launch_remove(const Dims &d, const State &st, const Scratch &sc, hipStream_t s);

}
```

Baseline: 96010.

## Overlap move replay with visibility pass by deferring move-target voxels

When a frame has object moves and runs in the simple single-shard setting, the move replay kernel now runs on the frustum side stream while the visibility pass runs on the main stream. Voxels touched by moves are tagged with a per-frame sequence mark. The visibility pass skips them and appends them to a deferred list, which a small follow-up kernel processes once the replay has finished. This takes the replay off the critical path, at the cost of an extra mark read per voxel in visibility, atomics for the deferred list, and added stream and event synchronisation.

```diff
diff --git a/include/sdm.h b/include/sdm.h
--- a/include/sdm.h
+++ b/include/sdm.h
@@ -411,6 +411,7 @@
 sdm_status sdm_debug_sweep_lists(sdm_map *m, int32_t mode);
 sdm_status sdm_debug_sweep_mode(sdm_map *m, int32_t *mode_out);
 sdm_status sdm_debug_alias_cap(sdm_map *m, int32_t cap);
+sdm_status sdm_debug_move_overlap(sdm_map *m, int64_t *frames_overlapped, int64_t *deferred_last_frame);
 sdm_status sdm_debug_reach_tiles(sdm_map *m, int64_t *tiles_out);
 sdm_status sdm_debug_view_batch(sdm_map *m, int32_t max_views_in_flight);
 
diff --git a/semantic_dsp_map_amd/binding.py b/semantic_dsp_map_amd/binding.py
--- a/semantic_dsp_map_amd/binding.py
+++ b/semantic_dsp_map_amd/binding.py
@@ -229,6 +229,7 @@
         "sdm_debug_sweep_lists": [vp, i32],
         "sdm_debug_sweep_mode": [vp, C.POINTER(i32)],
         "sdm_debug_alias_cap": [vp, i32],
+        "sdm_debug_move_overlap": [vp, C.POINTER(C.c_int64), C.POINTER(C.c_int64)],
         "sdm_test_scan": [vp, vp, i64],
         "sdm_test_sort_pairs": [vp, vp, vp, vp, i64, i32],
         "sdm_test_scratch_elems": [i32, i64, C.POINTER(i64)],
@@ -793,6 +794,11 @@
     def set_alias_cap(self, cap):
         _check(self.L, self.L.sdm_debug_alias_cap(self.h, int(cap)), "sdm_debug_alias_cap")
 
+    def move_overlap(self):
+        a, b = C.c_int64(0), C.c_int64(0)
+        _check(self.L, self.L.sdm_debug_move_overlap(self.h, C.byref(a), C.byref(b)), "sdm_debug_move_overlap")
+        return a.value, b.value
+
     def fill_dense(self):
         _check(self.L, self.L.sdm_debug_fill_dense(self.h), "sdm_debug_fill_dense")
 
diff --git a/semantic_dsp_map_amd/csrc/frame.hip b/semantic_dsp_map_amd/csrc/frame.hip
--- a/semantic_dsp_map_amd/csrc/frame.hip
+++ b/semantic_dsp_map_amd/csrc/frame.hip
@@ -67,6 +67,8 @@
   fa.mv_batch = 0;
   if (n_moves > 0 && !stage_done(stop_after, 1)) m->mv_seq++;
   fa.mv_seq = m->mv_seq;
+  fa.mv_overlap = 0;
+  m->overlap_frame = false;
   fa.n_remove = n_remove < MAX_REMOVE_TRACKS ? n_remove : MAX_REMOVE_TRACKS;
   for (int k = 0; k < fa.n_remove; ++k) fa.remove[k] = (uint16_t)remove_tracks[k];
   fa.force_generic = m->force_generic_flood;
@@ -75,18 +77,35 @@
   return SDM_OK;
 }
 
+bool frame_overlaps(const sdm_map *m) {
+  const Dims &d = m->d;
+  return m->move_overlap && !m->capturing && !m->profiling && m->n_moves > 0 && m->n_moves <= MAX_MOVE_OBJECTS && m->n_remove == 0 &&
+         d.v_count == d.V && m->cfg.shard_count == 1 && !m->comm && !m->ipc && !m->sharded_frame && !m->sc.halo_send && !m->sc.halo_recv &&
+         !m->counts_local_user && !m->counts_all_user && !stage_done(m->stop_after, 4);
+}
+
 sdm_status frame_enqueue_start(sdm_map *m) {
   hipStream_t s = m->stream;
   const Dims &d = m->d;
   const int32_t stop_after = m->stop_after;
   const bool whole = d.v_count == d.V;
+  m->overlap_frame = frame_overlaps(m);
+  m->fa.mv_overlap = 0;
+  if (m->overlap_frame) {
+    if (++m->mv_overlap_seq == 0) {
+      HIP_TRY(hipMemsetAsync(m->sc.mv_mark, 0, (size_t)d.v_count * sizeof(uint32_t), s));
+      m->mv_overlap_seq = 1;
+    }
+    m->fa.mv_overlap = m->mv_overlap_seq;
+    m->n_overlap_frames++;
+  }
   stage_mark(m, 0);
   if (m->stamps_dirty) SDM_TRY(upload_stamps(m));
   m->cur_depth = m->fa.depth;
   m->cur_cloud = m->fa.cloud;
   if (m->capturing) {
     m->fb.set(d, m->st, m->sc, m->fa, true, whole);
-    launch_frame_begin(m->fb, s);
+    HIP_TRY(launch_frame_begin(m->fb, s));
     HIP_TRY(hipEventRecord(m->cap_begin, s));
     HIP_TRY(hipStreamWaitEvent(m->s_frustum, m->cap_begin, 0));
     HIP_TRY(hipStreamWaitEvent(m->s_birth, m->cap_begin, 0));
@@ -101,7 +120,7 @@
     HIP_TRY(hipEventRecord(m->ev_fa, m->s_frustum));
     if (whole && m->mv_pending) HIP_TRY(hipMemsetAsync(m->sc.mv_tot, 0, move_total_elems() * sizeof(uint32_t), s));
     m->fb.set(d, m->st, m->sc, m->fa, false, whole);
-    launch_frame_begin(m->fb, s, !stage_done(stop_after, 5) ? m->ev_begin : nullptr);
+    HIP_TRY(launch_frame_begin(m->fb, s, !stage_done(stop_after, 5) ? m->ev_begin : nullptr));
     if (whole && m->n_moves > 0) m->mv_pending = true;
   }
   stage_mark(m, 1);
@@ -198,7 +217,7 @@
     r = 0;
   }
   if (m->capturing || m->n_moves > 0) {
-    launch_moves_transform(m->d, m->flt, m->st, m->sc, counts_all, w, r, m->stream);
+    HIP_TRY(launch_moves_transform(m->d, m->flt, m->st, m->sc, counts_all, w, r, m->stream, m->overlap_frame ? m->ev_apply : nullptr));
     m->mv_pending = false;
     m->mv_batch_ready = false;
     const bool shard = m->d.v_count != m->d.V;
@@ -221,7 +240,7 @@
         m->mv_batch_ready = true;
         return SDM_OK;
       }
-      launch_moves_transform(m->d, m->flt, m->st, m->sc, counts_all, w, r, m->stream);
+      HIP_TRY(launch_moves_transform(m->d, m->flt, m->st, m->sc, counts_all, w, r, m->stream));
     }
     m->mv_batch_next = 0;
   }
@@ -245,8 +264,22 @@
   if (!m->capturing) HIP_TRY(hipSetDevice(m->device));
   hipStream_t s = m->stream;
   const Dims &d = m->d;
+  if (m->overlap_frame) {
+    HIP_TRY(hipStreamWaitEvent(m->s_frustum, m->ev_apply, 0));
+    HIP_TRY(launch_moves_finish(d, m->flt, m->st, m->sc, 1, m->cfg.shard_rank, m->s_frustum, m->ev_replay));
+    HIP_TRY(hipStreamWaitEvent(s, m->ev_frustum, 0));
+    float *ck_dst = m->ck_user ? m->ck_user : m->d_ck_part;
+    HIP_TRY(launch_visibility_pass(d, m->st, m->sc, s, m->ev_vis));
+    m->vis_event_valid = true;
+    HIP_TRY(hipStreamWaitEvent(s, m->ev_replay, 0));
+    launch_visibility_deferred(d, m->st, m->sc, s);
+    launch_visibility_bins(d, m->flt, m->st, m->sc, ck_dst, m->fused_ck ? 1 : 0, s);
+    launch_ck(d, m->flt, m->st, m->sc, ck_dst, m->fused_ck ? 1 : 0, s);
+    if (ck_part_dev) *ck_part_dev = ck_dst;
+    return SDM_OK;
+  }
   if (m->capturing || m->n_moves > 0)
-    launch_moves_finish(d, m->flt, m->st, m->sc, m->counts_all_user ? m->cfg.shard_count : 1, m->cfg.shard_rank, s);
+    HIP_TRY(launch_moves_finish(d, m->flt, m->st, m->sc, m->counts_all_user ? m->cfg.shard_count : 1, m->cfg.shard_rank, s));
   stage_mark(m, 2);
   if (stage_done(stop_after, 2)) return SDM_OK;
 
@@ -263,7 +296,7 @@
 
   HIP_TRY(hipStreamWaitEvent(s, m->capturing ? m->cap_frustum : m->ev_frustum, 0));
   float *ck_dst = m->ck_user ? m->ck_user : m->d_ck_part;
-  launch_visibility(d, m->flt, m->st, m->sc, ck_dst, m->fused_ck ? 1 : 0, s, m->capturing ? nullptr : m->ev_vis);
+  HIP_TRY(launch_visibility(d, m->flt, m->st, m->sc, ck_dst, m->fused_ck ? 1 : 0, s, m->capturing ? nullptr : m->ev_vis));
   if (!m->capturing) m->vis_event_valid = true;
   stage_mark(m, 4);
   if (stage_done(stop_after, 4)) return SDM_OK;
@@ -448,13 +481,13 @@
   if (rc == SDM_OK)
     rc = capture(m->stream, 2, [&](hipStream_t st) {
       if (d.v_count != d.V) launch_moves_count(d, m->st, m->sc, m->d_counts_local, st);
-      launch_moves_transform(d, m->flt, m->st, m->sc, m->d_counts_local, 1, 0, st);
-      launch_moves_finish(d, m->flt, m->st, m->sc, 1, m->cfg.shard_rank, st);
+      (void)launch_moves_transform(d, m->flt, m->st, m->sc, m->d_counts_local, 1, 0, st);
+      (void)launch_moves_finish(d, m->flt, m->st, m->sc, 1, m->cfg.shard_rank, st);
       launch_remove(d, m->st, m->sc, st);
     });
   if (rc == SDM_OK)
     rc = capture(m->stream, 3, [&](hipStream_t st) {
-      launch_visibility(d, m->flt, m->st, m->sc, m->d_ck_part, 1, st);
+      (void)launch_visibility(d, m->flt, m->st, m->sc, m->d_ck_part, 1, st);
       launch_ck(d, m->flt, m->st, m->sc, m->d_ck_part, 1, st);
       launch_weight(d, m->flt, m->st, m->sc, st);
     });
@@ -471,7 +504,7 @@
   hipStream_t s = m->stream;
   const auto t0 = std::chrono::steady_clock::now();
   m->fb.set(m->d, m->st, m->sc, m->fa, true, m->d.v_count == m->d.V);
-  launch_frame_begin(m->fb, s);
+  HIP_TRY(launch_frame_begin(m->fb, s));
   HIP_TRY(hipEventRecord(m->ev_begin, s));
   HIP_TRY(hipStreamWaitEvent(m->s_frustum, m->ev_begin, 0));
   HIP_TRY(hipGraphLaunch(m->piece[0], m->s_frustum));
diff --git a/semantic_dsp_map_amd/csrc/kernels.hip b/semantic_dsp_map_amd/csrc/kernels.hip
--- a/semantic_dsp_map_amd/csrc/kernels.hip
+++ b/semantic_dsp_map_amd/csrc/kernels.hip
@@ -22,10 +22,12 @@
 #define DBG_PUTK(k, i, v) do { if (blockIdx.x < 8192) g_dbg[k][blockIdx.x * 4 + (i)] = (unsigned long long)(v); } while (0)
 #define DBG_PUT(i, v) DBG_PUTK(0, i, v)
 #define DBG_LANE0(k, i) do { if (threadIdx.x == 0 && threadIdx.y == 0) DBG_PUTK(k, i, DBG_T()); } while (0)
+#define DBG_DEFERRED(i) do { if (threadIdx.x == 0) DBG_PUTK(1, 4096 * 4 + (i), DBG_T()); } while (0)
 #else
 #define DBG_T() 0ull
 #define DBG_PUT(i, v)
 #define DBG_LANE0(k, i)
+#define DBG_DEFERRED(i)
 #endif
 
 typedef uint32_t v4u __attribute__((ext_vector_type(4)));
@@ -1567,6 +1569,7 @@
   const gptr<float> depth_img = as_global(sc.fa->depth);
   const uint32_t fgen = (uint32_t)sc.fa->force_generic, fcx = (uint32_t)sc.cnt->flood_complex;
   const bool generic = (fgen | fcx) != 0;
+  const uint32_t ovl = sc.fa->mv_overlap;
   if (blockIdx.x == 0 && threadIdx.x == 0) {
     sc.cnt->vis_flood_complex = fcx;
     sc.cnt->vis_flood_rounds = sc.cnt->flood_rounds;
@@ -1654,9 +1657,31 @@
     lvv[j] = have ? ring_to_voxel(d, rx, ry, rz) - d.v_begin : 0u;
     flg[j] = st.vflag[lvv[j]];
   }
+  uint32_t mk[VIS_J];
+#pragma unroll
+  for (int j = 0; j < VIS_J; ++j) mk[j] = 0;
+  if (ovl) {
+#pragma unroll
+    for (int j = 0; j < VIS_J; ++j)
+      if ((uint32_t)j * TPB < nl) mk[j] = sc.mv_mark[lvv[j]];
+  }
   __builtin_amdgcn_sched_barrier(0);
 #pragma unroll
   for (int j = 0; j < VIS_J; ++j) flg[j] = code[j] != 0xffffffffu ? flg[j] & VF_STATE : 0u;
+  if (ovl) {
+#pragma unroll
+    for (int j = 0; j < VIS_J; ++j) {
+      if (code[j] == 0xffffffffu || mk[j] != ovl) continue;
+      const uint32_t g = g0 + (code[j] >> 6);
+      const int ax = ((wlo + (int)(g % nwx)) << 6) + (int)(code[j] & 63u);
+      const int ay = f.bb0[1] + (int)((g / nwx) % by);
+      const int az = f.bb0[2] + (int)(g / ((uint32_t)nwx * by));
+      const uint32_t at = atomicAdd(&sc.cnt->n_vis_defer, 1u);
+      if (at < sc.cap_move) sc.vis_defer[at] = make_uint2((uint32_t)ax | (uint32_t)ay << 16, (uint32_t)az);
+      else sc.cnt->overflow = 1;
+      code[j] = 0xffffffffu;
+    }
+  }
   float imz[VIS_J], imd[VIS_J];
 #pragma unroll
   for (int j = 0; j < VIS_J; ++j) {
@@ -1702,6 +1727,37 @@
   }
   DBG_LANE0(1, 3);
   }
+}
+
+constexpr int VD_TPB = TPB, VD_GRID = 32;
+template <int S>
+__global__ __launch_bounds__(VD_TPB) void k_visibility_deferred(Dims d, State st, Scratch sc) {
+  DBG_DEFERRED(0);
+  const uint32_t n_raw = sc.cnt->n_vis_defer;
+  if (n_raw == 0) return;
+  const uint32_t n = n_raw < sc.cap_move ? n_raw : sc.cap_move;
+  const Frame f = sc.fa->f;
+  const gptr<float> depth_img = as_global(sc.fa->depth);
+  for (uint32_t t = blockIdx.x * VD_TPB + threadIdx.x; t < n; t += VD_GRID * VD_TPB) {
+    const uint2 en = sc.vis_defer[t];
+    const int ax = (int)(en.x & 0xffffu), ay = (int)(en.x >> 16), az = (int)en.y;
+    const uint32_t rx = axis_correct(ax + f.eq[0], d.NX), ry = axis_correct(ay + f.eq[1], d.NY), rz = axis_correct(az + f.eq[2], d.NZ);
+    const uint32_t lv = ring_to_voxel(d, rx, ry, rz) - d.v_begin;
+    if (st.vflag[lv] & VF_STATE) {
+      visibility_voxel<S>(d, f, st, sc, depth_img, ax, ay, az);
+      continue;
+    }
+    const float ix = (float)(uint32_t)ax * d.voxel_size + d.pmin[0] + f.center[0];
+    const float iy = (float)(uint32_t)ay * d.voxel_size + d.pmin[1] + f.center[1];
+    const float iz = (float)(uint32_t)az * d.voxel_size + d.pmin[2] + f.center[2];
+    int row, col;
+    float z;
+    if (project_to_image(d, f, ix, iy, iz, row, col, z) && z <= depth_img[(size_t)row * d.W + col]) {
+      st.vts[lv] = (uint16_t)f.gts;
+      mark_tile(st, lv, f.epoch);
+    }
+  }
+  DBG_DEFERRED(1);
 }
 
 __device__ __forceinline__ void sift_down(uint32_t *a, uint32_t start, uint32_t end) {
@@ -3290,22 +3346,34 @@
   hipLaunchKernelGGL(k_flood_generic, dim3(1), dim3(1024), 0, s, d, sc.fa_side, sc.vmask, sc.reach, sc.wpl, sc.cnt);
 }
 
-void launch_visibility(const Dims &d, const Filter &flt, const State &st, const Scratch &sc, float *ck_out, int finish, hipStream_t s,
-                       hipEvent_t vis_done) {
-  {
-    const size_t max_words = (size_t)((d.NX + 63) / 64 + 1) * d.NY * d.NZ;
-    dim3 grid((unsigned)std::min<size_t>(blocks_for(max_words, VIS_WORDS), 2048));
-    if (vis_done) {
-      switch (d.p_n) {
-        case 1: hipExtLaunchKernelGGL(k_visibility<2>, grid, dim3(TPB), 0, s, nullptr, vis_done, 0, d, st, sc); break;
-        case 2: hipExtLaunchKernelGGL(k_visibility<4>, grid, dim3(TPB), 0, s, nullptr, vis_done, 0, d, st, sc); break;
-        case 3: hipExtLaunchKernelGGL(k_visibility<8>, grid, dim3(TPB), 0, s, nullptr, vis_done, 0, d, st, sc); break;
-        default: hipExtLaunchKernelGGL(k_visibility<16>, grid, dim3(TPB), 0, s, nullptr, vis_done, 0, d, st, sc); break;
-      }
-    } else {
-      SDM_DISPATCH_S(k_visibility, grid, s, d, st, sc);
-    }
-  }
+hipError_t launch_visibility_pass(const Dims &d, const State &st, const Scratch &sc, hipStream_t s, hipEvent_t vis_done) {
+  const size_t max_words = (size_t)((d.NX + 63) / 64 + 1) * d.NY * d.NZ;
+  dim3 grid((unsigned)std::min<size_t>(blocks_for(max_words, VIS_WORDS), 2048));
+  if (vis_done) {
+    const void *k = d.p_n == 1   ? reinterpret_cast<const void *>(k_visibility<2>)
+                    : d.p_n == 2 ? reinterpret_cast<const void *>(k_visibility<4>)
+                    : d.p_n == 3 ? reinterpret_cast<const void *>(k_visibility<8>)
+                                 : reinterpret_cast<const void *>(k_visibility<16>);
+    void *argv[] = {(void *)&d, (void *)&st, (void *)&sc};
+    return hipExtLaunchKernel(k, grid, dim3(TPB), argv, 0, s, nullptr, vis_done, 0);
+  }
+  SDM_DISPATCH_S(k_visibility, grid, s, d, st, sc);
+  return hipSuccess;
+}
+
+void launch_visibility_deferred(const Dims &d, const State &st, const Scratch &sc, hipStream_t s) {
+  SDM_DISPATCH_S(k_visibility_deferred, dim3(VD_GRID), s, d, st, sc);
+}
+
+hipError_t launch_visibility(const Dims &d, const Filter &flt, const State &st, const Scratch &sc, float *ck_out, int finish, hipStream_t s,
+                             hipEvent_t vis_done) {
+  const hipError_t e = launch_visibility_pass(d, st, sc, s, vis_done);
+  if (e != hipSuccess) return e;
+  launch_visibility_bins(d, flt, st, sc, ck_out, finish, s);
+  return hipSuccess;
+}
+
+void launch_visibility_bins(const Dims &d, const Filter &flt, const State &st, const Scratch &sc, float *ck_out, int finish, hipStream_t s) {
   if (d.W <= 2 * BR_TPB) hipLaunchKernelGGL(k_bin_rows<2>, dim3((unsigned)d.H), dim3(BR_TPB), 0, s, d, st, sc);
   else if (d.W <= 4 * BR_TPB) hipLaunchKernelGGL(k_bin_rows<4>, dim3((unsigned)d.H), dim3(BR_TPB), 0, s, d, st, sc);
   else hipLaunchKernelGGL(k_bin_rows<8>, dim3((unsigned)d.H), dim3(BR_TPB), 0, s, d, st, sc);
diff --git a/semantic_dsp_map_amd/csrc/lifecycle.hip b/semantic_dsp_map_amd/csrc/lifecycle.hip
--- a/semantic_dsp_map_amd/csrc/lifecycle.hip
+++ b/semantic_dsp_map_amd/csrc/lifecycle.hip
@@ -406,7 +406,7 @@
 
   for (hipStream_t *s : {&m->own_stream, &m->s_frustum, &m->s_birth}) HIP_TRY(new_stream(cfg->device, s));
   m->stream = m->own_stream;
-  for (hipEvent_t *e : {&m->ev_state, &m->ev_counts, &m->ev_begin, &m->ev_frustum, &m->ev_birth, &m->ev_fa, &m->ev_vis, &m->cap_begin,
+  for (hipEvent_t *e : {&m->ev_state, &m->ev_counts, &m->ev_begin, &m->ev_frustum, &m->ev_birth, &m->ev_fa, &m->ev_vis, &m->ev_apply, &m->ev_replay, &m->cap_begin,
                         &m->cap_frustum, &m->cap_birth, &m->ev_copy, &m->raw[0].ev_free, &m->raw[1].ev_free})
     SDM_TRY(new_event(m, e, hipEventDisableTiming));
   const size_t n_slots = (size_t)d.v_count * d.S;
@@ -522,6 +522,9 @@
   A(sc.mv_row, (size_t)d.v_count * MV_ROW);
   HIP_TRY(hipMemsetAsync(sc.mv_row, 0xff, (size_t)d.v_count * MV_ROW * sizeof(uint32_t), m->stream));
   A(sc.mv_next, sc.cap_move);
+  A(sc.mv_mark, d.v_count);
+  HIP_TRY(hipMemsetAsync(sc.mv_mark, 0, (size_t)d.v_count * sizeof(uint32_t), m->stream));
+  A(sc.vis_defer, sc.cap_move);
   A(sc.cnt, 1);
   A(sc.cur, 1);
   HIP_TRY(hipMemsetAsync(sc.cnt, 0, sizeof(Counters), m->stream));
@@ -544,6 +547,7 @@
     const char *e = getenv("SDM_GRAPH");
     if (e && e[0] >= '0' && e[0] <= '4') m->graph_mode = e[0] - '0';
     if (const char *k = getenv("SDM_SWEEP_SKIP_SCAN")) m->sweep_skip_allowed = atoi(k) != 0;
+    if (const char *k = getenv("SDM_MOVE_OVERLAP")) m->move_overlap = atoi(k) != 0;
     m->host_timing = getenv("SDM_HOST_TIMING") != nullptr;
   }
   {
diff --git a/semantic_dsp_map_amd/csrc/moves.hip b/semantic_dsp_map_amd/csrc/moves.hip
--- a/semantic_dsp_map_amd/csrc/moves.hip
+++ b/semantic_dsp_map_amd/csrc/moves.hip
@@ -315,13 +315,16 @@
 
 constexpr uint32_t MV_NIL = 0xffffffffu;
 
-__device__ __forceinline__ void move_link(const Dims &d, const Scratch &sc, uint32_t v, uint32_t e, uint32_t forget_bits) {
+__device__ __forceinline__ void move_link(const Dims &d, const Scratch &sc, uint32_t v, uint32_t e, uint32_t forget_bits, uint32_t ovl) {
   const uint32_t lv = v - d.v_begin;
   uint32_t *row = sc.mv_row + (size_t)lv * MV_ROW;
   const uint32_t k = atomicAdd(&row[0], 1u) + 1u;
   if (k < (uint32_t)MV_DIRECT) {
     row[1 + k] = e;
-    if (k == 0u) sc.mv_copy[e].forget_bits = forget_bits | MV_FIRST;
+    if (k == 0u) {
+      sc.mv_copy[e].forget_bits = forget_bits | MV_FIRST;
+      if (ovl) sc.mv_mark[lv] = ovl;
+    }
   } else {
     const uint32_t prev = atomicExch(&row[MV_ROW - 1], e);
     sc.mv_next[e] = prev;
@@ -359,7 +362,7 @@
   return m;
 }
 __device__ __forceinline__ void move_store(const Dims &d, const Frame &f, const MoveSet &ms, const State &st, const Scratch &sc,
-                                           const MoveLoaded &m, int obj, uint32_t e, size_t li, bool alias) {
+                                           const MoveLoaded &m, int obj, uint32_t e, size_t li, bool alias, uint32_t ovl) {
   const float4 p = m.p;
   const float *T = ms.T[obj];
   float nx = row4(T + 0, p.x, p.y, p.z);
@@ -394,7 +397,7 @@
     c.status = pstatus;
     c.voxel = v - d.v_begin;
     sc.mv_copy[e] = c;
-    move_link(d, sc, v, e, c.forget_bits);
+    move_link(d, sc, v, e, c.forget_bits, ovl);
   } else if (sc.halo_send) {
     unsigned char *seg = sc.halo_send + (size_t)(rz / d.rz_count) * halo_segment_bytes(sc.halo_cap);
     uint32_t k = atomicAdd(reinterpret_cast<uint32_t *>(seg), 1u);
@@ -417,10 +420,10 @@
   }
 }
 __device__ __forceinline__ void move_one(const Dims &d, const Frame &f, const Filter &flt, const MoveSet &ms, const State &st,
-                                         const Scratch &sc, int obj, uint32_t e, size_t li, bool alias = false,
+                                         const Scratch &sc, uint32_t ovl, int obj, uint32_t e, size_t li, bool alias = false,
                                          bool copy_invalid = false) {
   const MoveLoaded m = move_load(d, flt, st, (long long)sc.cur->move_cursor, e, li, copy_invalid);
-  move_store(d, f, ms, st, sc, m, obj, e, li, alias);
+  move_store(d, f, ms, st, sc, m, obj, e, li, alias, ovl);
 }
 
 constexpr uint32_t CA_CAP = 512;
@@ -445,7 +448,7 @@
   return c;
 }
 __device__ __forceinline__ void move_slot_memberships(const Dims &d, const Frame &f, const Filter &flt, const MoveSet &ms, const State &st,
-                                                      const Scratch &sc, const ChunkAliases &ca, const uint32_t *mem, uint32_t nm,
+                                                      const Scratch &sc, uint32_t ovl, const ChunkAliases &ca, const uint32_t *mem, uint32_t nm,
                                                       const uint32_t *obj_base, size_t li, uint32_t s, uint32_t prim_o, uint32_t prim_rank) {
   int last = -1;
   bool first = true;
@@ -461,7 +464,7 @@
       }
     if (ob == 0xFFu) break;
     const uint32_t below = (!is_alias ? prim_rank : primaries_below(mem, nm, ob, s)) + aliases_below(ca, ob, (uint32_t)li);
-    move_one(d, f, flt, ms, st, sc, (int)ob, obj_base[ob] + below, li, is_alias, !first);
+    move_one(d, f, flt, ms, st, sc, ovl, (int)ob, obj_base[ob] + below, li, is_alias, !first);
     if (is_alias) st.alias[3 + 2 * entry] = OWNER_NONE;
     last = (int)ob;
     first = false;
@@ -488,6 +491,7 @@
   const Frame f = sc.fa->f;
   const MoveSet &ms = sc.fa->ms;
   const uint32_t par = sc.fa->mv_seq & 1u;
+  const uint32_t ovl = sc.fa->mv_overlap;
   const uint32_t batch = sc.fa->mv_batch;
   const uint32_t e_base = batch ? sc.cnt->n_moved_b[(batch - 1u) & 1u] : 0u;
   __shared__ uint32_t obj_base[MAX_MOVE_OBJECTS];
@@ -563,12 +567,12 @@
           const uint32_t o = (first_entry >> 12) & 63u;
           const uint32_t e = obj_base[o] + (first_entry >> 18);
           move_load_noise(flt, st, cursor, e, ml);
-          move_store(d, f, ms, st, sc, ml, (int)o, e, base + (first_entry & 4095u), false);
+          move_store(d, f, ms, st, sc, ml, (int)o, e, base + (first_entry & 4095u), false, ovl);
         }
         for (uint32_t i = TPB + threadIdx.x; i < nm; i += TPB) {
           const uint32_t en = sc.mv_mem[(size_t)pos * MV_CHUNK + i];
           const uint32_t o = (en >> 12) & 63u;
-          move_one(d, f, flt, ms, st, sc, (int)o, obj_base[o] + (en >> 18), base + (en & 4095u));
+          move_one(d, f, flt, ms, st, sc, ovl, (int)o, obj_base[o] + (en >> 18), base + (en & 4095u));
         }
         DBGM(0, 2, DBGM_T());
       } else {
@@ -603,12 +607,12 @@
             const uint32_t e = obj_base[o] + (en >> 18) + aliases_below(ca, o, (uint32_t)li);
             if (i == threadIdx.x) {
               move_load_noise(flt, st, cursor, e, ml);
-              move_store(d, f, ms, st, sc, ml, (int)o, e, li, false);
+              move_store(d, f, ms, st, sc, ml, (int)o, e, li, false, ovl);
             } else {
-              move_one(d, f, flt, ms, st, sc, (int)o, e, li);
+              move_one(d, f, flt, ms, st, sc, ovl, (int)o, e, li);
             }
           } else {
-            move_slot_memberships(d, f, flt, ms, st, sc, ca, cm_mem, nm, obj_base, li, sl, o, en >> 18);
+            move_slot_memberships(d, f, flt, ms, st, sc, ovl, ca, cm_mem, nm, obj_base, li, sl, o, en >> 18);
           }
         }
         for (uint32_t c = threadIdx.x; c < ca.n; c += TPB) {
@@ -622,7 +626,7 @@
               break;
             }
           }
-          if (!other) move_slot_memberships(d, f, flt, ms, st, sc, ca, cm_mem, nm, obj_base, li, sl, 0xFFu, 0u);
+          if (!other) move_slot_memberships(d, f, flt, ms, st, sc, ovl, ca, cm_mem, nm, obj_base, li, sl, 0xFFu, 0u);
         }
       }
     }
@@ -665,7 +669,7 @@
     c.status = (uint8_t)(r.owner_label_status >> 24);
     c.voxel = r.voxel - d.v_begin;
     sc.mv_copy[e] = c;
-    move_link(d, sc, r.voxel, e, c.forget_bits);
+    move_link(d, sc, r.voxel, e, c.forget_bits, 0u);
   }
 }
 
@@ -1118,25 +1122,41 @@
 }
 const void *FrameBeginLaunch::kernel() { return reinterpret_cast<const void *>(k_frame_begin); }
 
-void launch_frame_begin(FrameBeginLaunch &a, hipStream_t s, hipEvent_t done) {
-  if (done) (void)hipExtLaunchKernel(FrameBeginLaunch::kernel(), dim3(FrameBeginLaunch::GRID), dim3(FrameBeginLaunch::BLOCK), a.argv, 0, s, nullptr, done, 0);
-  else (void)hipLaunchKernel(FrameBeginLaunch::kernel(), dim3(FrameBeginLaunch::GRID), dim3(FrameBeginLaunch::BLOCK), a.argv, 0, s);
-}
-
-void launch_moves_transform(const Dims &d, const Filter &flt, const State &st, const Scratch &sc, const int32_t *counts_all, int world,
-                            int rank, hipStream_t s) {
-  hipLaunchKernelGGL(k_move_apply, dim3(1024), dim3(TPB), 0, s, d, flt, st, sc, d.v_count != d.V ? counts_all : nullptr, world, rank);
-}
-
-void launch_moves_finish(const Dims &d, const Filter &flt, const State &st, const Scratch &sc, int world, int rank, hipStream_t s) {
+hipError_t launch_frame_begin(FrameBeginLaunch &a, hipStream_t s, hipEvent_t done) {
+  if (done) return hipExtLaunchKernel(FrameBeginLaunch::kernel(), dim3(FrameBeginLaunch::GRID), dim3(FrameBeginLaunch::BLOCK), a.argv, 0, s, nullptr, done, 0);
+  return hipLaunchKernel(FrameBeginLaunch::kernel(), dim3(FrameBeginLaunch::GRID), dim3(FrameBeginLaunch::BLOCK), a.argv, 0, s);
+}
+
+hipError_t launch_moves_transform(const Dims &d, const Filter &flt, const State &st, const Scratch &sc, const int32_t *counts_all, int world,
+                                  int rank, hipStream_t s, hipEvent_t done) {
+  const int32_t *counts = d.v_count != d.V ? counts_all : nullptr;
+  if (!done) {
+    hipLaunchKernelGGL(k_move_apply, dim3(1024), dim3(TPB), 0, s, d, flt, st, sc, counts, world, rank);
+    return hipSuccess;
+  }
+  void *argv[] = {(void *)&d, (void *)&flt, (void *)&st, (void *)&sc, (void *)&counts, (void *)&world, (void *)&rank};
+  return hipExtLaunchKernel(reinterpret_cast<const void *>(k_move_apply), dim3(1024), dim3(TPB), argv, 0, s, nullptr, done, 0);
+}
+
+hipError_t launch_moves_finish(const Dims &d, const Filter &flt, const State &st, const Scratch &sc, int world, int rank, hipStream_t s,
+                               hipEvent_t done) {
   if (world > 1 && sc.halo_recv) hipLaunchKernelGGL(k_move_import, dim3(64, world), dim3(TPB), 0, s, d, sc, world, rank);
   dim3 grid(RP_GRID);
+  if (done) {
+    const void *k = d.p_n == 1   ? reinterpret_cast<const void *>(k_move_replay<2>)
+                    : d.p_n == 2 ? reinterpret_cast<const void *>(k_move_replay<4>)
+                    : d.p_n == 3 ? reinterpret_cast<const void *>(k_move_replay<8>)
+                                 : reinterpret_cast<const void *>(k_move_replay<16>);
+    void *argv[] = {(void *)&d, (void *)&flt, (void *)&st, (void *)&sc};
+    return hipExtLaunchKernel(k, grid, dim3(RP_TPB), argv, 0, s, nullptr, done, 0);
+  }
   switch (d.p_n) {
     case 1: hipLaunchKernelGGL(k_move_replay<2>, grid, dim3(RP_TPB), 0, s, d, flt, st, sc); break;
     case 2: hipLaunchKernelGGL(k_move_replay<4>, grid, dim3(RP_TPB), 0, s, d, flt, st, sc); break;
     case 3: hipLaunchKernelGGL(k_move_replay<8>, grid, dim3(RP_TPB), 0, s, d, flt, st, sc); break;
     default: hipLaunchKernelGGL(k_move_replay<16>, grid, dim3(RP_TPB), 0, s, d, flt, st, sc); break;
   }
+  return hipSuccess;
 }
 
 void launch_remove(const Dims &d, const State &st, const Scratch &sc, hipStream_t s) {
diff --git a/semantic_dsp_map_amd/csrc/readback.hip b/semantic_dsp_map_amd/csrc/readback.hip
--- a/semantic_dsp_map_amd/csrc/readback.hip
+++ b/semantic_dsp_map_amd/csrc/readback.hip
@@ -169,6 +169,19 @@
       ++n;
     }
   *n_out = n;
+  return SDM_OK;
+}
+
+sdm_status sdm_debug_move_overlap(sdm_map *m, int64_t *frames_overlapped, int64_t *deferred_last_frame) {
+  if (!m) return SDM_ERR_INVALID_ARGUMENT;
+  HIP_TRY(hipSetDevice(m->device));
+  if (frames_overlapped) *frames_overlapped = (int64_t)m->n_overlap_frames;
+  if (deferred_last_frame) {
+    uint32_t n = 0;
+    HIP_TRY(hipMemcpyAsync(&n, &m->sc.cnt->n_vis_defer, sizeof(n), hipMemcpyDeviceToHost, m->stream));
+    HIP_TRY(hipStreamSynchronize(m->stream));
+    *deferred_last_frame = (int64_t)n;
+  }
   return SDM_OK;
 }
 
diff --git a/semantic_dsp_map_amd/csrc/sdm_internal.h b/semantic_dsp_map_amd/csrc/sdm_internal.h
--- a/semantic_dsp_map_amd/csrc/sdm_internal.h
+++ b/semantic_dsp_map_amd/csrc/sdm_internal.h
@@ -70,7 +70,8 @@
   uint32_t n_halo_dropped;
   uint32_t vis_flood_complex, vis_flood_rounds, vis_start_in_frustum;
   uint32_t n_moved_b[2];
-  uint32_t pad[2];
+  uint32_t n_vis_defer;
+  uint32_t pad[1];
   struct alignas(128) ShardLine {
     uint32_t vis;
     uint32_t fv;
diff --git a/semantic_dsp_map_amd/csrc/sdm_map.h b/semantic_dsp_map_amd/csrc/sdm_map.h
--- a/semantic_dsp_map_amd/csrc/sdm_map.h
+++ b/semantic_dsp_map_amd/csrc/sdm_map.h
@@ -101,6 +101,11 @@
   size_t mv_batch_next = 0;
   bool mv_batch_ready = false;
   uint32_t mv_seq = 0;
+  bool move_overlap = true;
+  bool overlap_frame = false;
+  uint32_t mv_overlap_seq = 0;
+  uint64_t n_overlap_frames = 0;
+  hipEvent_t ev_apply = nullptr, ev_replay = nullptr;
   uint32_t *d_track_bits = nullptr;
   int32_t *d_counts_local = nullptr;
   ncclComm_t comm = nullptr;
diff --git a/semantic_dsp_map_amd/csrc/sdm_scratch.h b/semantic_dsp_map_amd/csrc/sdm_scratch.h
--- a/semantic_dsp_map_amd/csrc/sdm_scratch.h
+++ b/semantic_dsp_map_amd/csrc/sdm_scratch.h
@@ -38,6 +38,7 @@
   int n_remove;
   uint32_t mv_seq;
   uint32_t mv_batch;
+  uint32_t mv_overlap;
   int force_generic;
   const float *depth;
   const sdm_labeled_point *cloud;
@@ -87,6 +88,8 @@
   uint32_t *scan_scratch = nullptr, *sort_scratch = nullptr;
   uint32_t *scan_scratch_b = nullptr;
   uint32_t *mv_row = nullptr, *mv_next = nullptr;
+  uint32_t *mv_mark = nullptr;
+  uint2 *vis_defer = nullptr;
   Counters *cnt = nullptr;
   Cursors *cur = nullptr;
 };
@@ -134,15 +137,18 @@
   void set(const Dims &d, const State &st, const Scratch &sc, const FrameArgs &fa, bool with_side, bool with_members);
   static const void *kernel();
 };
-void launch_frame_begin(FrameBeginLaunch &a, hipStream_t s, hipEvent_t done = nullptr);
+hipError_t launch_frame_begin(FrameBeginLaunch &a, hipStream_t s, hipEvent_t done = nullptr);
 void launch_moves_batch(const Dims &d, const State &st, const Scratch &sc, const FrameArgs &fa_batch, int32_t *counts_local, hipStream_t s);
 constexpr int OCC_LISTS = 1, OCC_SKIP_SCAN = 2;
 void launch_occupancy(const Dims &d, const Filter &flt, const State &st, Counters *cnt, int all_dirty, const FrameArgs *fa, uint32_t remark,
                       hipStream_t s, int mode = 0);
 size_t tile_mark_bytes(const Dims &d);
 void launch_frustum(const Dims &d, const Scratch &sc, hipStream_t s);
-void launch_visibility(const Dims &d, const Filter &flt, const State &st, const Scratch &sc, float *ck_out, int finish, hipStream_t s,
-                       hipEvent_t vis_done = nullptr);
+hipError_t launch_visibility(const Dims &d, const Filter &flt, const State &st, const Scratch &sc, float *ck_out, int finish, hipStream_t s,
+                             hipEvent_t vis_done = nullptr);
+hipError_t launch_visibility_pass(const Dims &d, const State &st, const Scratch &sc, hipStream_t s, hipEvent_t vis_done);
+void launch_visibility_deferred(const Dims &d, const State &st, const Scratch &sc, hipStream_t s);
+void launch_visibility_bins(const Dims &d, const Filter &flt, const State &st, const Scratch &sc, float *ck_out, int finish, hipStream_t s);
 void launch_ck(const Dims &d, const Filter &flt, const State &st, const Scratch &sc, float *ck_out, int finish, hipStream_t s);
 void launch_ck_finish(const Dims &d, const Filter &flt, const Scratch &sc, const float *parts, int n_parts, size_t part_stride, hipStream_t s);
 void launch_ck_reduce_chunk(const float *stage, const float *own_part, float *full, uint32_t chunk, int world, int rank, hipStream_t s);
@@ -187,9 +193,10 @@
 void launch_owner_flags(const Dims &d, const State &st, hipStream_t s);
 void launch_moves_count(const Dims &d, const State &st, const Scratch &sc, int32_t *counts_local, hipStream_t s,
                         const FrameArgs *by_value = nullptr);
-void launch_moves_transform(const Dims &d, const Filter &flt, const State &st, const Scratch &sc, const int32_t *counts_all, int world,
-                            int rank, hipStream_t s);
-void launch_moves_finish(const Dims &d, const Filter &flt, const State &st, const Scratch &sc, int world, int rank, hipStream_t s);
+hipError_t launch_moves_transform(const Dims &d, const Filter &flt, const State &st, const Scratch &sc, const int32_t *counts_all, int world,
+                                  int rank, hipStream_t s, hipEvent_t done = nullptr);
+hipError_t launch_moves_finish(const Dims &d, const Filter &flt, const State &st, const Scratch &sc, int world, int rank, hipStream_t s,
+                               hipEvent_t done = nullptr);
 void launch_remove(const Dims &d, const State &st, const Scratch &sc, hipStream_t s);
 
 }
```

Result: slower. 92370 (-3.8%).
